# manuelbb-upb/Morbit.jl

Hardware: AMD Instinct MI355X
Metric: RBF build+solve+eval cycles/sec (higher is better)
Workload: dtype f64

## Files before the change

### include/mrbf.h

```cpp
#ifndef MRBF_H
#define MRBF_H

#include <stdint.h>

#ifdef __cplusplus
extern "C" {
#endif

typedef struct mrbf_ctx mrbf_ctx;
typedef struct mrbf_model mrbf_model;

enum {
    MRBF_CUBIC = 0,
    MRBF_INV_MULTIQUADRIC = 1,
    MRBF_MULTIQUADRIC = 2,
    MRBF_THIN_PLATE_SPLINE = 3,
    MRBF_GAUSSIAN = 4
};

enum {
    MRBF_OK = 0,
    MRBF_ENOTPD = 1,
    MRBF_ESINGULAR = 2,
    MRBF_EHIP = 3,
    MRBF_EBLAS = 4,
    MRBF_ENOMEM = 5,
    MRBF_ENODEVICE = 6,
    MRBF_ENCCL = 7
};

enum {
    MRBF_PATH_CHOL = 1,
    MRBF_PATH_PROJ_CHOL = 2,
    MRBF_PATH_LU = 3,
    MRBF_PATH_MINNORM = 4,
    MRBF_PATH_ROUND4 = 5
};

enum {
    MRBF_OPT_GRAM_MODE = 1,
    MRBF_OPT_RESIDUAL = 2,
    MRBF_OPT_FORCE_PATH = 3,
    MRBF_OPT_CHOL_IMPL = 4,
    MRBF_OPT_EVAL_IMPL = 5,
    MRBF_OPT_TIMING = 6,
    MRBF_OPT_DIAG_IMPL = 7,
    MRBF_OPT_CHOL_WINDOW = 8,
    MRBF_OPT_SPIN_MS = 9,
    MRBF_OPT_LAST_DEVICE_MS = 11,
    MRBF_OPT_SLOW_LAUNCHES = 12,
    MRBF_OPT_ARENA_BYTES = 13,
    MRBF_OPT_LIVE_HANDLES = 14,
    MRBF_OPT_SMALL_FIT_MAX_N = 15,
    MRBF_OPT_SMALL_LU = 16,
    MRBF_OPT_DEBUG_FAULT = 10
};

enum {
    MRBF_FB_CHOL_HOST_DRIVEN = 1,
    MRBF_FB_BACKSOLVE_BLOCKED = 2,
    MRBF_FB_LU = 4
};

typedef struct {
    int32_t path;
    int32_t factor_info;
    int32_t n, q;
    double rel_residual;
    double max_pitw;
    double mu;
    float ms_gram, ms_project, ms_factor, ms_solve, ms_check, ms_total;
    int32_t fallbacks;
    int32_t giveup_code;
    float ms_factor_device;
    int32_t slow_launches;
} mrbf_fit_info;

typedef struct {
    float ms_total;
    float ms_dist, ms_kernel, ms_contract;
} mrbf_eval_info;

int32_t mrbf_init(int32_t device_id, mrbf_ctx **ctx);
int32_t mrbf_shutdown(mrbf_ctx *ctx);
const char *mrbf_last_error(const mrbf_ctx *ctx);
const char *mrbf_version(void);
int32_t mrbf_set_option(mrbf_ctx *ctx, int32_t key, double value);
int32_t mrbf_get_option(const mrbf_ctx *ctx, int32_t key, double *value);
int32_t mrbf_set_stream(mrbf_ctx *ctx, void *hip_stream);
int32_t mrbf_sync(mrbf_ctx *ctx);

int32_t mrbf_gram(mrbf_ctx *ctx, int64_t n, int32_t d, const double *centres, int32_t kernel_id, double a, double b,
                  int32_t poly_deg, double *Phi_out, double *Pi_out, float *ms);

int32_t mrbf_cross_gram(mrbf_ctx *ctx, int64_t m, int64_t n, int32_t d, const double *X, const double *centres, int32_t kernel_id,
                        double a, double b, double *K_out);

int32_t mrbf_fit(mrbf_ctx *ctx, int64_t n, int32_t d, int32_t k, const double *centres, const double *values,
                 int32_t kernel_id, double a, double b, int32_t poly_deg, mrbf_model **model, double *weights_out,
                 double *poly_out, mrbf_fit_info *info);

int32_t mrbf_model_from_coeffs(mrbf_ctx *ctx, int64_t n, int32_t d, int32_t k, const double *centres,
                               const double *weights, const double *poly, int32_t kernel_id, double a, double b,
                               int32_t poly_deg, mrbf_model **model);

int32_t mrbf_eval(mrbf_ctx *ctx, const mrbf_model *model, int64_t m, const double *X, double *vals_out,
                  double *jac_out, mrbf_eval_info *info);

typedef struct {
    float ms_total;
    int32_t nsplit;
    int32_t chunks;
    int32_t reserved;
} mrbf_hess_info;
int32_t mrbf_eval_hessian(mrbf_ctx *ctx, const mrbf_model *model, int64_t m, const double *X, int32_t n_rows, const int32_t *rows,
                          double *hess_out, mrbf_hess_info *info);
int32_t mrbf_eval_hessian_limited(mrbf_ctx *ctx, const mrbf_model *model, int64_t m, const double *X, int32_t n_rows,
                                  const int32_t *rows, double *hess_out, mrbf_hess_info *info, int64_t stage_bytes);

int32_t mrbf_backtrack(mrbf_ctx *ctx, const mrbf_model *model, const double *x, const double *dir, double step0,
                       double omega, int32_t strict, double const_rhs, double shrink, double min_stepsize,
                       int32_t max_loops, double *x_plus, double *mx_plus, double *step, int32_t *n_loops);

int32_t mrbf_affine_scores(mrbf_ctx *ctx, int64_t mc, int32_t d, int32_t dz, const double *shifted, const double *Z, int32_t p_is_inf,
                           double *vals_out, int64_t *argmax, double *maxval);
int32_t mrbf_affine_select(mrbf_ctx *ctx, int64_t mc, int32_t d, const double *shifted, int32_t j0, const double *Q0, int32_t max_picks,
                           double pivot_val, int32_t p_is_inf, int64_t *picked_out, int32_t *n_picked, double *Z_out);

typedef struct {
    int64_t mc;
    int32_t j0;
    int32_t max_picks;
    double pivot_val;
    const double *shifted;
    const double *Q0;
    int64_t *picked_out;
    double *Z_out;
    int32_t n_picked;
    int32_t reserved;
} mrbf_affine_job;
int32_t mrbf_affine_select_batch(mrbf_ctx *ctx, int64_t n_starts, int32_t d, int32_t p_is_inf, mrbf_affine_job *jobs,
                                 float *ms_total);

typedef struct mrbf_round4_state mrbf_round4_state;
int32_t mrbf_round4(mrbf_ctx *ctx, int64_t n0, int32_t d, const double *start_sites, int64_t mc, const double *cand_sites,
                    int32_t kernel_id, double a, double b, int32_t poly_deg, int32_t max_points, double theta_pivot_cholesky,
                    int32_t *accepted_out, int32_t *n_accepted, mrbf_round4_state **state);
int32_t mrbf_fit_from_round4(mrbf_ctx *ctx, const mrbf_round4_state *state, int32_t k, const double *values, mrbf_model **model,
                             double *weights_out, double *poly_out, mrbf_fit_info *info);
int32_t mrbf_round4_sites(const mrbf_round4_state *state, int64_t *n0, int64_t *n_candidates, int32_t *n_accepted);
int32_t mrbf_free_round4(mrbf_ctx *ctx, mrbf_round4_state *state);

typedef struct {
    int64_t n0, mc;
    const double *start_sites;
    const double *cand_sites;
    int32_t kernel_id, poly_deg;
    double a, b;
    int32_t max_points;
    double theta_pivot_cholesky;
    int32_t *accepted_out;
    int32_t n_accepted;
    int32_t rc;
} mrbf_round4_job;
int32_t mrbf_round4_batch(mrbf_ctx *ctx, int64_t n_starts, int32_t d, mrbf_round4_job *jobs, float *ms_total);

int32_t mrbf_model_dims(const mrbf_model *model, int64_t *n, int32_t *d, int32_t *k, int32_t *q);
int32_t mrbf_free_model(mrbf_ctx *ctx, mrbf_model *model);

typedef struct {
    int64_t n, m;
    int32_t d, k, kernel_id, poly_deg;
    double a, b;
    const double *centres;
    const double *values;
    const double *X;
    double *weights_out;
    double *poly_out;
    double *vals_out;
    double *jac_out;
} mrbf_problem;

typedef struct {
    int32_t status;
    int32_t device;
    mrbf_fit_info fit;
    float ms_eval;
    double checksum_w;
    double checksum_vals;
} mrbf_result;

int32_t mrbf_batch_run(int32_t n_dev, const int32_t *device_ids, int64_t n_problems, const mrbf_problem *problems,
                       mrbf_result *results);

typedef struct {
    int64_t n;
    int32_t d, k, kernel_id, poly_deg;
    double a, b;
    const double *centres, *values;
    double *weights_out, *poly_out;
    mrbf_model *model;
    int32_t status;
    int32_t reserved;
    mrbf_fit_info info;
} mrbf_fit_job;
int32_t mrbf_fit_batch(mrbf_ctx *ctx, int64_t n_starts, mrbf_fit_job *jobs, float *ms_total);

typedef struct {
    const mrbf_model *model;
    int64_t m;
    const double *X;
    double *vals_out;
    double *jac_out;
    int32_t status;
    int32_t reserved;
} mrbf_eval_job;
int32_t mrbf_eval_batch(mrbf_ctx *ctx, int64_t n_jobs, mrbf_eval_job *jobs, float *ms_total);
int32_t mrbf_eval_batch_limited(mrbf_ctx *ctx, int64_t n_jobs, mrbf_eval_job *jobs, float *ms_total, int64_t arena_limit_bytes);

typedef struct mrbf_db mrbf_db;
int32_t mrbf_db_create(mrbf_ctx *ctx, int32_t d, int32_t k, int64_t capacity_hint, mrbf_db **db);
int32_t mrbf_db_append(mrbf_ctx *ctx, mrbf_db *db, int64_t m, const double *sites, const double *values, int64_t *first_index);
int32_t mrbf_db_set_values(mrbf_ctx *ctx, mrbf_db *db, int64_t m, const int64_t *indices, const double *values);
int32_t mrbf_db_read(mrbf_ctx *ctx, const mrbf_db *db, int64_t first, int64_t m, double *sites_out, double *values_out);
int32_t mrbf_db_dims(const mrbf_db *db, int64_t *n_sites, int32_t *d, int32_t *k);
int32_t mrbf_db_free(mrbf_ctx *ctx, mrbf_db *db);

typedef struct {
    mrbf_db *db;
    const double *lb, *ub, *x0;
    int64_t n_exclude;
    const int64_t *exclude;
    int32_t zero_first_pick;
    int32_t rc;
    int64_t *indices_out;
    double *sites_out, *shifted_out;
    double *first_row;
    int64_t mc;
    int64_t first_pick;
    const double *cand_sites_dev;
    const double *shifted_dev;
} mrbf_db_box_job;
int32_t mrbf_db_box_batch(mrbf_ctx *ctx, int64_t n_starts, int32_t d, int32_t p_is_inf, mrbf_db_box_job *jobs, float *ms_total);

typedef struct {
    mrbf_db *db;
    int64_t n_idx;
    const int64_t *indices;
    double *sites_out, *values_out;
    const double *sites_dev;
    const double *values_dev;
    int32_t rc;
    int32_t reserved;
} mrbf_db_gather_job;
int32_t mrbf_db_gather_batch(mrbf_ctx *ctx, int64_t n_starts, int32_t d, mrbf_db_gather_job *jobs, float *ms_total);

typedef struct {
    mrbf_db *db;
    int64_t m;
    const double *sites;
    const double *values;
    int64_t first_index;
    int32_t rc;
    int32_t reserved;
} mrbf_db_append_job;
int32_t mrbf_db_append_batch(mrbf_ctx *ctx, int64_t n_starts, mrbf_db_append_job *jobs, float *ms_total);
typedef struct {
    mrbf_db *db;
    int64_t m;
    const int64_t *indices;
    const double *values;
    int32_t rc;
    int32_t reserved;
} mrbf_db_set_values_job;
int32_t mrbf_db_set_values_batch(mrbf_ctx *ctx, int64_t n_starts, mrbf_db_set_values_job *jobs, float *ms_total);

enum { MRBF_R3_UPDATE = 0, MRBF_R3_IMPROVE = 1 };
enum { MRBF_R3_DONE = 0, MRBF_R3_REBUILT = 1 };
typedef struct {
    mrbf_db *db;
    const double *x, *lb, *ub;
    double pivot_val;
    const double *dirs;
    int32_t n_dirs, reversed;
    int32_t n_missing, max_new;
    int32_t ensure_fully_linear, force_rebuild, mode;
    int32_t rc;
    double *new_sites_out;
    int64_t first_index;
    int32_t n_new, fully_linear, status, n_dirs_used;
} mrbf_round3_job;
int32_t mrbf_db_round3_batch(mrbf_ctx *ctx, int64_t n_starts, int32_t d, mrbf_round3_job *jobs, float *ms_total);

int32_t mrbf_debug_env(const char *name);
int32_t mrbf_debug_mfma_layout(mrbf_ctx *ctx, double *out16x16_a_times_b, const double *A16x4, const double *B4x16);
int32_t mrbf_debug_potrf(mrbf_ctx *ctx, int64_t n, double *A_colmajor_inout, int32_t impl, int32_t *info, float *ms);
int32_t mrbf_debug_diag(mrbf_ctx *ctx, const double *A128, int32_t reps, float *ms_per_call, double *shader_cycles,
                        double *realtime_us);
int32_t mrbf_debug_mfma_peak(mrbf_ctx *ctx, int32_t blocks_per_cu, int32_t threads, int32_t iters, float *ms, double *tflops);
int32_t mrbf_debug_mfma_asm(mrbf_ctx *ctx, int32_t variant, int32_t blocks_per_cu, int32_t iters, float *ms, double *tflops,
                            double *cycles_per_mfma);
int32_t mrbf_debug_dgemm(mrbf_ctx *ctx, int32_t m, int32_t n, int32_t k, float *ms, double *tflops);
int32_t mrbf_debug_mega_tables(int32_t nt, int32_t mt, int32_t slack, int32_t slack_chain, int32_t first, int32_t win, int32_t srows,
                               int32_t half_cols, int64_t *out6);
int32_t mrbf_debug_mega_tables2(int32_t nt, int32_t mt, int32_t slack, int32_t slack_chain, int32_t first, int32_t win, int32_t srows,
                                int32_t half_cols, const int32_t *opt5, int64_t *out6);
int32_t mrbf_debug_mega_plan(int32_t nt, int32_t mt, int32_t xreal, int64_t *out39);

enum { MRBF_PS_OK = 0, MRBF_PS_CRITICAL = 1, MRBF_PS_FAILURE = 2 };
typedef struct {
    int32_t max_ideal_evals;
    int32_t max_ps_evals;
    int32_t max_polish_evals;
    int32_t reserved;
    uint64_t seed;
    double t0;
    double xtol_rel;
} mrbf_ps_options;
typedef struct {
    int32_t status;
    int32_t generations;
    int32_t evals_ideal, evals_ps, evals_polish;
    float ms_total;
    double tau;
} mrbf_ps_info;
int32_t mrbf_ps_step(mrbf_ctx *ctx, const mrbf_model *model, const double *x_n, const double *lb_eff, const double *ub_eff,
                     const double *fx_n, const double *r_or_null, const mrbf_ps_options *opts, double *x_trial, double *mx_trial,
                     double *r_out, mrbf_ps_info *info);

enum { MRBF_ROLE_NONE = -1, MRBF_ROLE_EQ = -2, MRBF_ROLE_INEQ = -3 };
typedef struct {
    int32_t n_models, n_objectives;
    const mrbf_model *const *models;
    const int32_t *roles;
    int32_t n_lin_eq, n_lin_ineq;
    const double *A_eq, *b_eq, *A_ineq, *b_ineq;
    double eq_tol;
} mrbf_ps_problem;
int32_t mrbf_ps_step_problem(mrbf_ctx *ctx, const mrbf_ps_problem *problem, const double *x_n, const double *lb_eff,
                             const double *ub_eff, const double *fx_n, const double *r_or_null, const mrbf_ps_options *opts,
                             double *x_trial, double *mx_trial, double *r_out, mrbf_ps_info *info);
int32_t mrbf_debug_ps_rank(mrbf_ctx *ctx, int32_t lam, const double *f, const double *phi, uint64_t seed, int32_t gen, int32_t impl,
                           int32_t *order_out, int32_t *gave_up);

enum { MRBF_SD_OK = 0, MRBF_SD_NO_OBJECTIVE = 1, MRBF_SD_INFEASIBLE = 2, MRBF_SD_GAVE_UP = 3 };
int32_t mrbf_sd_direction(mrbf_ctx *ctx, int64_t n_lp, int32_t d, int32_t k, int32_t m_eq, int32_t m_ineq, const double *G,
                          const double *x, const double *lb, const double *ub, const double *A_eq, const double *b_eq,
                          const double *A_ineq, const double *b_ineq, int32_t normalize, double *d_out, double *omega_out,
                          double *dual_out, int32_t *status_out, int32_t *iters_out);
typedef struct {
    int32_t status;
    int32_t iterations;
    int32_t bound_flips;
    float ms_total;
    double omega;
} mrbf_sd_info;
int32_t mrbf_sd_criticality(mrbf_ctx *ctx, const mrbf_ps_problem *problem, const double *x, const double *x_n, const double *lb,
                            const double *ub, int32_t normalize, double *d_out, double *dual_out, mrbf_sd_info *info);

enum { MRBF_NS_OK = 0, MRBF_NS_INFEASIBLE = 1, MRBF_NS_GAVE_UP = 2 };
int32_t mrbf_normal_direction(mrbf_ctx *ctx, int64_t n_lp, int32_t d, int32_t m_eq, int32_t m_ineq, const double *x, const double *lb,
                              const double *ub, const double *A_eq, const double *b_eq, const double *A_ineq, const double *b_ineq,
                              double *n_out, double *alpha_out, double *dual_out, int32_t *status_out, int32_t *iters_out);
typedef struct {
    int32_t status;
    int32_t iterations;
    int32_t bound_flips;
    float ms_total;
    double alpha;
    double delta;
} mrbf_normal_info;
int32_t mrbf_normal_step(mrbf_ctx *ctx, const mrbf_ps_problem *problem, int32_t d, const double *x, const double *lb, const double *ub,
                         double delta, double kappa_delta, double delta_max, int32_t variable_radius, double *n_out, double *dual_out,
                         mrbf_normal_info *info);

typedef struct {
    int32_t strict;
    int32_t max_loops;
    double const_rhs;
    double shrink;
    double min_stepsize;
} mrbf_sd_step_options;
typedef struct {
    int32_t branch;
    int32_t loops;
    float ms_total;
    double sigma;
    double omega;
    double step_norm;
} mrbf_sd_step_info;
int32_t mrbf_sd_step(mrbf_ctx *ctx, const mrbf_ps_problem *problem, const double *x, const double *x_n, double delta, const double *lb,
                     const double *ub, double omega, const double *d, const mrbf_sd_step_options *opts, double *x_plus, double *mx_plus,
                     mrbf_sd_step_info *info);

typedef struct {
    int32_t sd_status;
    int32_t iterations, bound_flips;
    int32_t branch, loops;
    int32_t reserved;
    double omega;
    double omega_step;
    double sigma, step_norm;
} mrbf_sd_batch_record;
int32_t mrbf_sd_iterate_batch(mrbf_ctx *ctx, int64_t n_starts, const mrbf_ps_problem *shape, const mrbf_model *const *models,
                              const double *x, const double *x_n, const double *delta, const double *lb, const double *ub,
                              int32_t normalize, const mrbf_sd_step_options *opts, double *d_out, double *x_plus, double *mx_plus,
                              mrbf_sd_batch_record *records, float *ms_total);

typedef struct {
    int32_t status;
    int32_t iterations, bound_flips;
    int32_t reserved;
    double alpha;
    double delta;
} mrbf_normal_batch_record;
int32_t mrbf_normal_step_batch(mrbf_ctx *ctx, int64_t n_starts, const mrbf_ps_problem *shape, const mrbf_model *const *models, int32_t d,
                               const double *x, const double *lb, const double *ub, const double *delta, double kappa_delta,
                               double delta_max, int32_t variable_radius, double *n_out, double *x_n_out, double *dual_out,
                               mrbf_normal_batch_record *records, float *ms_total);

int32_t mrbf_ps_step_batch(mrbf_ctx *ctx, int64_t n_starts, const mrbf_ps_problem *shape, const mrbf_model *const *models,
                           const double *x_n, const double *lb_eff, const double *ub_eff, const double *fx_n, const double *r_or_null,
                           const mrbf_ps_options *opts, const uint64_t *seeds_or_null, double *x_trial, double *mx_trial, double *r_out,
                           mrbf_ps_info *infos, float *ms_total);

enum { MRBF_DISPATCH_REFERENCE = 0, MRBF_DISPATCH_DEVICE = 1 };
enum { MRBF_FIT_FULL = 0, MRBF_FIT_FROM_ROUND4 = 1 };
enum { MRBF_ENTRY_ROUND4 = 1, MRBF_ENTRY_FIT_FROM_ROUND4 = 2, MRBF_ENTRY_PS_STEP = 3, MRBF_ENTRY_BACKTRACK = 4, MRBF_ENTRY_AFFINE = 5,
       MRBF_ENTRY_SD = 6, MRBF_ENTRY_NORMAL = 7, MRBF_ENTRY_SD_STEP = 8, MRBF_ENTRY_SD_BATCH = 9, MRBF_ENTRY_AFFINE_BATCH = 10,
       MRBF_ENTRY_FIT_BATCH = 11, MRBF_ENTRY_NORMAL_BATCH = 12, MRBF_ENTRY_ROUND4_BATCH = 13, MRBF_ENTRY_PS_BATCH = 14,
       MRBF_ENTRY_DB_BOX = 15, MRBF_ENTRY_DB_GATHER = 16, MRBF_ENTRY_DB_ROUND3 = 17, MRBF_ENTRY_DB_APPEND_BATCH = 18,
       MRBF_ENTRY_DB_SET_VALUES_BATCH = 19, MRBF_ENTRY_EVAL_BATCH = 20 };
int32_t mrbf_dispatch_ps(int32_t d, int32_t k, int32_t n_models, int32_t n_nl_constraints, int32_t n_lin_constraints, int32_t n_foreign);
int32_t mrbf_dispatch_ps_batch(int64_t n_starts, int32_t d, int32_t k, int32_t n_models, int32_t n_nl_constraints,
                               int32_t n_lin_constraints, int32_t n_foreign);
int32_t mrbf_dispatch_sd(int32_t d, int32_t k, int32_t n_models, int32_t n_nl_constraints, int32_t n_lin_constraints, int32_t n_foreign);
int32_t mrbf_dispatch_normal(int32_t d, int32_t n_models, int32_t n_nl_constraints, int32_t n_lin_constraints, int32_t n_foreign);
int32_t mrbf_dispatch_sd_step(int32_t d, int32_t k, int32_t n_models, int32_t n_nl_constraints, int32_t n_lin_constraints, int32_t n_foreign,
                              int32_t max_loops);
int32_t mrbf_dispatch_sd_batch(int64_t n_starts, int32_t d, int32_t k, int32_t n_models, int32_t n_nl_constraints,
                               int32_t n_lin_constraints, int32_t n_foreign, int32_t max_loops);
int32_t mrbf_dispatch_normal_batch(int64_t n_starts, int32_t d, int32_t n_models, int32_t n_nl_constraints, int32_t n_lin_constraints,
                                   int32_t n_foreign);
int32_t mrbf_dispatch_backtrack(int32_t n_objective_models, int32_t n_foreign, int32_t outputs_in_order);
int32_t mrbf_dispatch_affine(int64_t n_candidates, int32_t d);
int32_t mrbf_dispatch_affine_batch(int64_t n_starts, int32_t d, int32_t p_is_inf);
int32_t mrbf_dispatch_round4(int64_t n0, int32_t d, int32_t poly_deg, int64_t n_candidates);
int32_t mrbf_dispatch_fit_batch(int64_t n_starts);
int64_t mrbf_dispatch_fit_batch_max_n(int64_t n_starts, int32_t d);
int32_t mrbf_dispatch_fit_batch_lu(int64_t n_lu_starts, int64_t n_max, int32_t d);
int32_t mrbf_dispatch_round4_batch(int64_t n_starts, int32_t d);
int32_t mrbf_dispatch_db_batch(int64_t n_starts, int32_t d);
int32_t mrbf_dispatch_eval_batch(int64_t n_jobs);
int64_t mrbf_dispatch_eval_batch_min_jobs(void);
int32_t mrbf_dispatch_fit(int64_t n_training, int64_t state_n0, int32_t state_q, int32_t state_n_accepted, int32_t same_sites);
int32_t mrbf_dispatch_after(int32_t entry, int32_t rc);

int32_t mrbf_stochastic_rank(int32_t lam, const double *f, const double *phi, const double *u, double pf, int32_t *idx_out);

#ifdef __cplusplus
}
#endif
#endif
```

### morbit.jl_amd/_lib.py

```python
import ctypes
import os

import numpy as np

_HERE = os.path.dirname(os.path.abspath(__file__))
LIB_PATH = os.environ.get("MRBF_LIB") or os.path.join(_HERE, "libmrbf.so")

c_dp = ctypes.POINTER(ctypes.c_double)
c_fp = ctypes.POINTER(ctypes.c_float)
c_ip = ctypes.POINTER(ctypes.c_int32)
c_vp = ctypes.c_void_p

MRBF_OK, MRBF_ENOTPD, MRBF_ESINGULAR, MRBF_EHIP, MRBF_EBLAS, MRBF_ENOMEM, MRBF_ENODEVICE, MRBF_ENCCL = range(8)
PATH_CHOL, PATH_PROJ_CHOL, PATH_LU, PATH_MINNORM, PATH_ROUND4 = 1, 2, 3, 4, 5
OPT_GRAM_MODE, OPT_RESIDUAL, OPT_FORCE_PATH, OPT_CHOL_IMPL, OPT_EVAL_IMPL, OPT_TIMING, OPT_DIAG_IMPL, OPT_CHOL_WINDOW = 1, 2, 3, 4, 5, 6, 7, 8
OPT_SPIN_MS, OPT_DEBUG_FAULT, OPT_LAST_DEVICE_MS, OPT_SLOW_LAUNCHES = 9, 10, 11, 12
OPT_ARENA_BYTES, OPT_LIVE_HANDLES = 13, 14
OPT_SMALL_FIT_MAX_N = 15
SMALL_FIT_DEFAULT_MAX_N = 512
OPT_SMALL_LU = 16
SMALL_LU_MAX_N, SMALL_LU_MAX_D, SMALL_LU_MAX_K = 512, 128, 16
FB_CHOL_HOST_DRIVEN, FB_BACKSOLVE_BLOCKED, FB_LU = 1, 2, 4


class FitInfo(ctypes.Structure):
    _fields_ = [("path", ctypes.c_int32), ("factor_info", ctypes.c_int32), ("n", ctypes.c_int32), ("q", ctypes.c_int32),
                ("rel_residual", ctypes.c_double), ("max_pitw", ctypes.c_double), ("mu", ctypes.c_double),
                ("ms_gram", ctypes.c_float), ("ms_project", ctypes.c_float), ("ms_factor", ctypes.c_float),
                ("ms_solve", ctypes.c_float), ("ms_check", ctypes.c_float), ("ms_total", ctypes.c_float),
                ("fallbacks", ctypes.c_int32), ("giveup_code", ctypes.c_int32), ("ms_factor_device", ctypes.c_float),
                ("slow_launches", ctypes.c_int32)]

    def asdict(self):
        return {f: getattr(self, f) for f, _ in self._fields_}


class EvalInfo(ctypes.Structure):
    _fields_ = [("ms_total", ctypes.c_float), ("ms_dist", ctypes.c_float), ("ms_kernel", ctypes.c_float),
                ("ms_contract", ctypes.c_float)]

    def asdict(self):
        return {f: getattr(self, f) for f, _ in self._fields_}


class HessInfo(ctypes.Structure):
    _fields_ = [("ms_total", ctypes.c_float), ("nsplit", ctypes.c_int32), ("chunks", ctypes.c_int32), ("reserved", ctypes.c_int32)]

    def asdict(self):
        return {f: getattr(self, f) for f, _ in self._fields_}


class PsOptions(ctypes.Structure):
    _fields_ = [("max_ideal_evals", ctypes.c_int32), ("max_ps_evals", ctypes.c_int32), ("max_polish_evals", ctypes.c_int32),
                ("reserved", ctypes.c_int32), ("seed", ctypes.c_uint64), ("t0", ctypes.c_double), ("xtol_rel", ctypes.c_double)]


class PsInfo(ctypes.Structure):
    _fields_ = [("status", ctypes.c_int32), ("generations", ctypes.c_int32), ("evals_ideal", ctypes.c_int32),
                ("evals_ps", ctypes.c_int32), ("evals_polish", ctypes.c_int32), ("ms_total", ctypes.c_float), ("tau", ctypes.c_double)]

    def asdict(self):
        return {f: getattr(self, f) for f, _ in self._fields_}


PS_OK, PS_CRITICAL, PS_FAILURE = 0, 1, 2
ROLE_NONE, ROLE_EQ, ROLE_INEQ = -1, -2, -3
DISPATCH_REFERENCE, DISPATCH_DEVICE = 0, 1
FIT_FULL, FIT_FROM_ROUND4 = 0, 1
ENTRY_ROUND4, ENTRY_FIT_FROM_ROUND4, ENTRY_PS_STEP, ENTRY_BACKTRACK, ENTRY_AFFINE, ENTRY_SD, ENTRY_NORMAL, ENTRY_SD_STEP = 1, 2, 3, 4, 5, 6, 7, 8
ENTRY_SD_BATCH = 9
ENTRY_AFFINE_BATCH = 10
ENTRY_FIT_BATCH = 11
ENTRY_NORMAL_BATCH = 12
ENTRY_ROUND4_BATCH = 13
ENTRY_PS_BATCH = 14
ENTRY_DB_BOX = 15
ENTRY_DB_GATHER = 16
ENTRY_DB_ROUND3 = 17
ENTRY_DB_APPEND_BATCH = 18
ENTRY_DB_SET_VALUES_BATCH = 19
ENTRY_EVAL_BATCH = 20
R3_UPDATE, R3_IMPROVE = 0, 1
R3_DONE, R3_REBUILT = 0, 1
SD_OK, SD_NO_OBJECTIVE, SD_INFEASIBLE, SD_GAVE_UP = 0, 1, 2, 3
NS_OK, NS_INFEASIBLE, NS_GAVE_UP = 0, 1, 2
SD_BRANCH_DELTA, SD_BRANCH_ONE, SD_BRANCH_INTERSECT = 0, 1, 2


class PsProblem(ctypes.Structure):
    _fields_ = [("n_models", ctypes.c_int32), ("n_objectives", ctypes.c_int32), ("models", ctypes.POINTER(ctypes.c_void_p)),
                ("roles", ctypes.POINTER(ctypes.c_int32)), ("n_lin_eq", ctypes.c_int32), ("n_lin_ineq", ctypes.c_int32),
                ("A_eq", ctypes.c_void_p), ("b_eq", ctypes.c_void_p), ("A_ineq", ctypes.c_void_p), ("b_ineq", ctypes.c_void_p),
                ("eq_tol", ctypes.c_double)]


class SdInfo(ctypes.Structure):
    _fields_ = [("status", ctypes.c_int32), ("iterations", ctypes.c_int32), ("bound_flips", ctypes.c_int32), ("ms_total", ctypes.c_float),
                ("omega", ctypes.c_double)]

    def asdict(self):
        return {f: getattr(self, f) for f, _ in self._fields_}


class NormalInfo(ctypes.Structure):
    _fields_ = [("status", ctypes.c_int32), ("iterations", ctypes.c_int32), ("bound_flips", ctypes.c_int32), ("ms_total", ctypes.c_float),
                ("alpha", ctypes.c_double), ("delta", ctypes.c_double)]

    def asdict(self):
        return {f: getattr(self, f) for f, _ in self._fields_}


class SdStepOptions(ctypes.Structure):
    _fields_ = [("strict", ctypes.c_int32), ("max_loops", ctypes.c_int32), ("const_rhs", ctypes.c_double), ("shrink", ctypes.c_double),
                ("min_stepsize", ctypes.c_double)]


class SdStepInfo(ctypes.Structure):
    _fields_ = [("branch", ctypes.c_int32), ("loops", ctypes.c_int32), ("ms_total", ctypes.c_float), ("sigma", ctypes.c_double),
                ("omega", ctypes.c_double), ("step_norm", ctypes.c_double)]

    def asdict(self):
        return {f: getattr(self, f) for f, _ in self._fields_}


class SdBatchRecord(ctypes.Structure):
    _fields_ = [("sd_status", ctypes.c_int32), ("iterations", ctypes.c_int32), ("bound_flips", ctypes.c_int32), ("branch", ctypes.c_int32),
                ("loops", ctypes.c_int32), ("reserved", ctypes.c_int32), ("omega", ctypes.c_double), ("omega_step", ctypes.c_double),
                ("sigma", ctypes.c_double), ("step_norm", ctypes.c_double)]

    def asdict(self):
        return {f: getattr(self, f) for f, _ in self._fields_}


class NormalBatchRecord(ctypes.Structure):
    _fields_ = [("status", ctypes.c_int32), ("iterations", ctypes.c_int32), ("bound_flips", ctypes.c_int32), ("reserved", ctypes.c_int32),
                ("alpha", ctypes.c_double), ("delta", ctypes.c_double)]

    def asdict(self):
        return {f: getattr(self, f) for f, _ in self._fields_}


class AffineJob(ctypes.Structure):
    _fields_ = [("mc", ctypes.c_int64), ("j0", ctypes.c_int32), ("max_picks", ctypes.c_int32), ("pivot_val", ctypes.c_double),
                ("shifted", ctypes.c_void_p), ("Q0", ctypes.c_void_p), ("picked_out", ctypes.c_void_p), ("Z_out", ctypes.c_void_p),
                ("n_picked", ctypes.c_int32), ("reserved", ctypes.c_int32)]


class Round4Job(ctypes.Structure):
    _fields_ = [("n0", ctypes.c_int64), ("mc", ctypes.c_int64), ("start_sites", ctypes.c_void_p), ("cand_sites", ctypes.c_void_p),
                ("kernel_id", ctypes.c_int32), ("poly_deg", ctypes.c_int32), ("a", ctypes.c_double), ("b", ctypes.c_double),
                ("max_points", ctypes.c_int32), ("theta_pivot_cholesky", ctypes.c_double), ("accepted_out", ctypes.c_void_p),
                ("n_accepted", ctypes.c_int32), ("rc", ctypes.c_int32)]


class FitJob(ctypes.Structure):
    _fields_ = [("n", ctypes.c_int64), ("d", ctypes.c_int32), ("k", ctypes.c_int32), ("kernel_id", ctypes.c_int32),
                ("poly_deg", ctypes.c_int32), ("a", ctypes.c_double), ("b", ctypes.c_double), ("centres", ctypes.c_void_p),
                ("values", ctypes.c_void_p), ("weights_out", ctypes.c_void_p), ("poly_out", ctypes.c_void_p), ("model", ctypes.c_void_p),
                ("status", ctypes.c_int32), ("reserved", ctypes.c_int32), ("info", FitInfo)]


class EvalJob(ctypes.Structure):
    _fields_ = [("model", ctypes.c_void_p), ("m", ctypes.c_int64), ("X", ctypes.c_void_p), ("vals_out", ctypes.c_void_p),
                ("jac_out", ctypes.c_void_p), ("status", ctypes.c_int32), ("reserved", ctypes.c_int32)]


class DbBoxJob(ctypes.Structure):
    _fields_ = [("db", ctypes.c_void_p), ("lb", ctypes.c_void_p), ("ub", ctypes.c_void_p), ("x0", ctypes.c_void_p),
                ("n_exclude", ctypes.c_int64), ("exclude", ctypes.c_void_p), ("zero_first_pick", ctypes.c_int32), ("rc", ctypes.c_int32),
                ("indices_out", ctypes.c_void_p), ("sites_out", ctypes.c_void_p), ("shifted_out", ctypes.c_void_p),
                ("first_row", ctypes.c_void_p), ("mc", ctypes.c_int64), ("first_pick", ctypes.c_int64),
                ("cand_sites_dev", ctypes.c_void_p), ("shifted_dev", ctypes.c_void_p)]


class DbGatherJob(ctypes.Structure):
    _fields_ = [("db", ctypes.c_void_p), ("n_idx", ctypes.c_int64), ("indices", ctypes.c_void_p), ("sites_out", ctypes.c_void_p),
                ("values_out", ctypes.c_void_p), ("sites_dev", ctypes.c_void_p), ("values_dev", ctypes.c_void_p),
                ("rc", ctypes.c_int32), ("reserved", ctypes.c_int32)]


class DbAppendJob(ctypes.Structure):
    _fields_ = [("db", ctypes.c_void_p), ("m", ctypes.c_int64), ("sites", ctypes.c_void_p), ("values", ctypes.c_void_p),
                ("first_index", ctypes.c_int64), ("rc", ctypes.c_int32), ("reserved", ctypes.c_int32)]


class DbSetValuesJob(ctypes.Structure):
    _fields_ = [("db", ctypes.c_void_p), ("m", ctypes.c_int64), ("indices", ctypes.c_void_p), ("values", ctypes.c_void_p),
                ("rc", ctypes.c_int32), ("reserved", ctypes.c_int32)]


class Round3Job(ctypes.Structure):
    _fields_ = [("db", ctypes.c_void_p), ("x", ctypes.c_void_p), ("lb", ctypes.c_void_p), ("ub", ctypes.c_void_p),
                ("pivot_val", ctypes.c_double), ("dirs", ctypes.c_void_p), ("n_dirs", ctypes.c_int32), ("reversed", ctypes.c_int32),
                ("n_missing", ctypes.c_int32), ("max_new", ctypes.c_int32), ("ensure_fully_linear", ctypes.c_int32),
                ("force_rebuild", ctypes.c_int32), ("mode", ctypes.c_int32), ("rc", ctypes.c_int32), ("new_sites_out", ctypes.c_void_p),
                ("first_index", ctypes.c_int64), ("n_new", ctypes.c_int32), ("fully_linear", ctypes.c_int32), ("status", ctypes.c_int32),
                ("n_dirs_used", ctypes.c_int32)]


class Problem(ctypes.Structure):
    _fields_ = [("n", ctypes.c_int64), ("m", ctypes.c_int64), ("d", ctypes.c_int32), ("k", ctypes.c_int32),
                ("kernel_id", ctypes.c_int32), ("poly_deg", ctypes.c_int32), ("a", ctypes.c_double), ("b", ctypes.c_double),
                ("centres", c_dp), ("values", c_dp), ("X", c_dp), ("weights_out", c_dp), ("poly_out", c_dp),
                ("vals_out", c_dp), ("jac_out", c_dp)]


class Result(ctypes.Structure):
    _fields_ = [("status", ctypes.c_int32), ("device", ctypes.c_int32), ("fit", FitInfo), ("ms_eval", ctypes.c_float),
                ("checksum_w", ctypes.c_double), ("checksum_vals", ctypes.c_double)]


SIGNATURES = {
    "mrbf_init": (ctypes.c_int32, [ctypes.c_int32, ctypes.POINTER(c_vp)]),
    "mrbf_shutdown": (ctypes.c_int32, [c_vp]),
    "mrbf_last_error": (ctypes.c_char_p, [c_vp]),
    "mrbf_version": (ctypes.c_char_p, []),
    "mrbf_set_option": (ctypes.c_int32, [c_vp, ctypes.c_int32, ctypes.c_double]),
    "mrbf_get_option": (ctypes.c_int32, [c_vp, ctypes.c_int32, c_dp]),
    "mrbf_set_stream": (ctypes.c_int32, [c_vp, c_vp]),
    "mrbf_sync": (ctypes.c_int32, [c_vp]),
    "mrbf_gram": (ctypes.c_int32, [c_vp, ctypes.c_int64, ctypes.c_int32, c_vp, ctypes.c_int32, ctypes.c_double,
                                   ctypes.c_double, ctypes.c_int32, c_vp, c_vp, c_fp]),
    "mrbf_cross_gram": (ctypes.c_int32, [c_vp, ctypes.c_int64, ctypes.c_int64, ctypes.c_int32, c_vp, c_vp, ctypes.c_int32, ctypes.c_double,
                                         ctypes.c_double, c_vp]),
    "mrbf_fit": (ctypes.c_int32, [c_vp, ctypes.c_int64, ctypes.c_int32, ctypes.c_int32, c_vp, c_vp, ctypes.c_int32,
                                  ctypes.c_double, ctypes.c_double, ctypes.c_int32, ctypes.POINTER(c_vp), c_vp, c_vp,
                                  ctypes.POINTER(FitInfo)]),
    "mrbf_model_from_coeffs": (ctypes.c_int32, [c_vp, ctypes.c_int64, ctypes.c_int32, ctypes.c_int32, c_vp, c_vp, c_vp,
                                                ctypes.c_int32, ctypes.c_double, ctypes.c_double, ctypes.c_int32,
                                                ctypes.POINTER(c_vp)]),
    "mrbf_eval": (ctypes.c_int32, [c_vp, c_vp, ctypes.c_int64, c_vp, c_vp, c_vp, ctypes.POINTER(EvalInfo)]),
    "mrbf_eval_hessian": (ctypes.c_int32, [c_vp, c_vp, ctypes.c_int64, c_vp, ctypes.c_int32, c_vp, c_vp, ctypes.POINTER(HessInfo)]),
    "mrbf_eval_hessian_limited": (ctypes.c_int32, [c_vp, c_vp, ctypes.c_int64, c_vp, ctypes.c_int32, c_vp, c_vp, ctypes.POINTER(HessInfo),
                                                   ctypes.c_int64]),
    "mrbf_backtrack": (ctypes.c_int32, [c_vp, c_vp, c_vp, c_vp, ctypes.c_double, ctypes.c_double, ctypes.c_int32,
                                        ctypes.c_double, ctypes.c_double, ctypes.c_double, ctypes.c_int32, c_vp, c_vp,
                                        c_vp, c_ip]),
    "mrbf_affine_scores": (ctypes.c_int32, [c_vp, ctypes.c_int64, ctypes.c_int32, ctypes.c_int32, c_vp, c_vp, ctypes.c_int32, c_vp,
                                            ctypes.POINTER(ctypes.c_int64), c_dp]),
    "mrbf_affine_select": (ctypes.c_int32, [c_vp, ctypes.c_int64, ctypes.c_int32, c_vp, ctypes.c_int32, c_vp, ctypes.c_int32, ctypes.c_double,
                                            ctypes.c_int32, ctypes.POINTER(ctypes.c_int64), c_ip, c_vp]),
    "mrbf_affine_select_batch": (ctypes.c_int32, [c_vp, ctypes.c_int64, ctypes.c_int32, ctypes.c_int32, ctypes.POINTER(AffineJob), c_fp]),
    "mrbf_round4": (ctypes.c_int32, [c_vp, ctypes.c_int64, ctypes.c_int32, c_vp, ctypes.c_int64, c_vp, ctypes.c_int32, ctypes.c_double,
                                     ctypes.c_double, ctypes.c_int32, ctypes.c_int32, ctypes.c_double, c_vp, c_ip, ctypes.POINTER(c_vp)]),
    "mrbf_fit_from_round4": (ctypes.c_int32, [c_vp, c_vp, ctypes.c_int32, c_vp, ctypes.POINTER(c_vp), c_vp, c_vp, ctypes.POINTER(FitInfo)]),
    "mrbf_round4_sites": (ctypes.c_int32, [c_vp, ctypes.POINTER(ctypes.c_int64), ctypes.POINTER(ctypes.c_int64), c_ip]),
    "mrbf_free_round4": (ctypes.c_int32, [c_vp, c_vp]),
    "mrbf_round4_batch": (ctypes.c_int32, [c_vp, ctypes.c_int64, ctypes.c_int32, ctypes.POINTER(Round4Job), c_fp]),
    "mrbf_dispatch_round4_batch": (ctypes.c_int32, [ctypes.c_int64, ctypes.c_int32]),
    "mrbf_model_dims": (ctypes.c_int32, [c_vp, ctypes.POINTER(ctypes.c_int64), c_ip, c_ip, c_ip]),
    "mrbf_free_model": (ctypes.c_int32, [c_vp, c_vp]),
    "mrbf_batch_run": (ctypes.c_int32, [ctypes.c_int32, c_ip, ctypes.c_int64, ctypes.POINTER(Problem),
                                        ctypes.POINTER(Result)]),
    "mrbf_fit_batch": (ctypes.c_int32, [c_vp, ctypes.c_int64, ctypes.POINTER(FitJob), c_fp]),
    "mrbf_dispatch_fit_batch": (ctypes.c_int32, [ctypes.c_int64]),
    "mrbf_dispatch_fit_batch_max_n": (ctypes.c_int64, [ctypes.c_int64, ctypes.c_int32]),
    "mrbf_dispatch_fit_batch_lu": (ctypes.c_int32, [ctypes.c_int64, ctypes.c_int64, ctypes.c_int32]),
    "mrbf_eval_batch": (ctypes.c_int32, [c_vp, ctypes.c_int64, ctypes.POINTER(EvalJob), c_fp]),
    "mrbf_eval_batch_limited": (ctypes.c_int32, [c_vp, ctypes.c_int64, ctypes.POINTER(EvalJob), c_fp, ctypes.c_int64]),
    "mrbf_dispatch_eval_batch": (ctypes.c_int32, [ctypes.c_int64]),
    "mrbf_dispatch_eval_batch_min_jobs": (ctypes.c_int64, []),
    "mrbf_db_create": (ctypes.c_int32, [c_vp, ctypes.c_int32, ctypes.c_int32, ctypes.c_int64, ctypes.POINTER(c_vp)]),
    "mrbf_db_append": (ctypes.c_int32, [c_vp, c_vp, ctypes.c_int64, c_vp, c_vp, ctypes.POINTER(ctypes.c_int64)]),
    "mrbf_db_set_values": (ctypes.c_int32, [c_vp, c_vp, ctypes.c_int64, c_vp, c_vp]),
    "mrbf_db_read": (ctypes.c_int32, [c_vp, c_vp, ctypes.c_int64, ctypes.c_int64, c_vp, c_vp]),
    "mrbf_db_dims": (ctypes.c_int32, [c_vp, ctypes.POINTER(ctypes.c_int64), c_ip, c_ip]),
    "mrbf_db_free": (ctypes.c_int32, [c_vp, c_vp]),
    "mrbf_db_box_batch": (ctypes.c_int32, [c_vp, ctypes.c_int64, ctypes.c_int32, ctypes.c_int32, ctypes.POINTER(DbBoxJob), c_fp]),
    "mrbf_db_gather_batch": (ctypes.c_int32, [c_vp, ctypes.c_int64, ctypes.c_int32, ctypes.POINTER(DbGatherJob), c_fp]),
    "mrbf_db_append_batch": (ctypes.c_int32, [c_vp, ctypes.c_int64, ctypes.POINTER(DbAppendJob), c_fp]),
    "mrbf_db_set_values_batch": (ctypes.c_int32, [c_vp, ctypes.c_int64, ctypes.POINTER(DbSetValuesJob), c_fp]),
    "mrbf_db_round3_batch": (ctypes.c_int32, [c_vp, ctypes.c_int64, ctypes.c_int32, ctypes.POINTER(Round3Job), c_fp]),
    "mrbf_dispatch_db_batch": (ctypes.c_int32, [ctypes.c_int64, ctypes.c_int32]),
    "mrbf_debug_mfma_layout": (ctypes.c_int32, [c_vp, c_vp, c_vp, c_vp]),
    "mrbf_debug_potrf": (ctypes.c_int32, [c_vp, ctypes.c_int64, c_vp, ctypes.c_int32, c_ip, c_fp]),
    "mrbf_debug_env": (ctypes.c_int32, [ctypes.c_char_p]),
    "mrbf_debug_diag": (ctypes.c_int32, [c_vp, c_vp, ctypes.c_int32, c_fp, c_dp, c_dp]),
    "mrbf_debug_ps_rank": (ctypes.c_int32, [c_vp, ctypes.c_int32, c_vp, c_vp, ctypes.c_uint64, ctypes.c_int32, ctypes.c_int32, c_ip, c_ip]),
    "mrbf_debug_mfma_peak": (ctypes.c_int32, [c_vp, ctypes.c_int32, ctypes.c_int32, ctypes.c_int32, c_fp, c_dp]),
    "mrbf_debug_mfma_asm": (ctypes.c_int32, [c_vp, ctypes.c_int32, ctypes.c_int32, ctypes.c_int32, c_fp, c_dp, c_dp]),
    "mrbf_debug_dgemm": (ctypes.c_int32, [c_vp, ctypes.c_int32, ctypes.c_int32, ctypes.c_int32, c_fp, c_dp]),
    "mrbf_debug_mega_tables": (ctypes.c_int32, [ctypes.c_int32] * 8 + [c_vp]),
    "mrbf_debug_mega_tables2": (ctypes.c_int32, [ctypes.c_int32] * 8 + [c_vp, c_vp]),
    "mrbf_debug_mega_plan": (ctypes.c_int32, [ctypes.c_int32] * 3 + [c_vp]),
    "mrbf_stochastic_rank": (ctypes.c_int32, [ctypes.c_int32, c_vp, c_vp, c_vp, ctypes.c_double, c_vp]),
    "mrbf_ps_step": (ctypes.c_int32, [c_vp, c_vp, c_vp, c_vp, c_vp, c_vp, c_vp, ctypes.POINTER(PsOptions), c_vp, c_vp, c_vp,
                                      ctypes.POINTER(PsInfo)]),
    "mrbf_ps_step_problem": (ctypes.c_int32, [c_vp, ctypes.POINTER(PsProblem), c_vp, c_vp, c_vp, c_vp, c_vp, ctypes.POINTER(PsOptions),
                                              c_vp, c_vp, c_vp, ctypes.POINTER(PsInfo)]),
    "mrbf_ps_step_batch": (ctypes.c_int32, [c_vp, ctypes.c_int64, ctypes.POINTER(PsProblem), ctypes.POINTER(ctypes.c_void_p), c_vp, c_vp, c_vp,
                                            c_vp, c_vp, ctypes.POINTER(PsOptions), ctypes.POINTER(ctypes.c_uint64), c_vp, c_vp, c_vp,
                                            ctypes.POINTER(PsInfo), c_fp]),
    "mrbf_dispatch_ps_batch": (ctypes.c_int32, [ctypes.c_int64] + [ctypes.c_int32] * 6),
    "mrbf_sd_direction": (ctypes.c_int32, [c_vp, ctypes.c_int64, ctypes.c_int32, ctypes.c_int32, ctypes.c_int32, ctypes.c_int32] + [c_vp] * 8
                          + [ctypes.c_int32, c_vp, c_vp, c_vp, c_vp, c_vp]),
    "mrbf_sd_criticality": (ctypes.c_int32, [c_vp, ctypes.POINTER(PsProblem), c_vp, c_vp, c_vp, c_vp, ctypes.c_int32, c_vp, c_vp,
                                             ctypes.POINTER(SdInfo)]),
    "mrbf_normal_direction": (ctypes.c_int32, [c_vp, ctypes.c_int64, ctypes.c_int32, ctypes.c_int32, ctypes.c_int32] + [c_vp] * 12),
    "mrbf_normal_step": (ctypes.c_int32, [c_vp, ctypes.POINTER(PsProblem), ctypes.c_int32, c_vp, c_vp, c_vp, ctypes.c_double, ctypes.c_double,
                                          ctypes.c_double, ctypes.c_int32, c_vp, c_vp, ctypes.POINTER(NormalInfo)]),
    "mrbf_sd_step": (ctypes.c_int32, [c_vp, ctypes.POINTER(PsProblem), c_vp, c_vp, ctypes.c_double, c_vp, c_vp, ctypes.c_double, c_vp,
                                      ctypes.POINTER(SdStepOptions), c_vp, c_vp, ctypes.POINTER(SdStepInfo)]),
    "mrbf_sd_iterate_batch": (ctypes.c_int32, [c_vp, ctypes.c_int64, ctypes.POINTER(PsProblem), ctypes.POINTER(ctypes.c_void_p), c_vp, c_vp, c_vp,
                                               c_vp, c_vp, ctypes.c_int32, ctypes.POINTER(SdStepOptions), c_vp, c_vp, c_vp,
                                               ctypes.POINTER(SdBatchRecord), c_fp]),
    "mrbf_dispatch_sd_batch": (ctypes.c_int32, [ctypes.c_int64] + [ctypes.c_int32] * 7),
    "mrbf_normal_step_batch": (ctypes.c_int32, [c_vp, ctypes.c_int64, ctypes.POINTER(PsProblem), ctypes.POINTER(ctypes.c_void_p), ctypes.c_int32,
                                                c_vp, c_vp, c_vp, c_vp, ctypes.c_double, ctypes.c_double, ctypes.c_int32, c_vp, c_vp, c_vp,
                                                ctypes.POINTER(NormalBatchRecord), c_fp]),
    "mrbf_dispatch_normal_batch": (ctypes.c_int32, [ctypes.c_int64] + [ctypes.c_int32] * 5),
    "mrbf_dispatch_ps": (ctypes.c_int32, [ctypes.c_int32] * 6),
    "mrbf_dispatch_sd_step": (ctypes.c_int32, [ctypes.c_int32] * 7),
    "mrbf_dispatch_sd": (ctypes.c_int32, [ctypes.c_int32] * 6),
    "mrbf_dispatch_normal": (ctypes.c_int32, [ctypes.c_int32] * 5),
    "mrbf_dispatch_backtrack": (ctypes.c_int32, [ctypes.c_int32] * 3),
    "mrbf_dispatch_affine": (ctypes.c_int32, [ctypes.c_int64, ctypes.c_int32]),
    "mrbf_dispatch_affine_batch": (ctypes.c_int32, [ctypes.c_int64, ctypes.c_int32, ctypes.c_int32]),
    "mrbf_dispatch_round4": (ctypes.c_int32, [ctypes.c_int64, ctypes.c_int32, ctypes.c_int32, ctypes.c_int64]),
    "mrbf_dispatch_fit": (ctypes.c_int32, [ctypes.c_int64, ctypes.c_int64, ctypes.c_int32, ctypes.c_int32, ctypes.c_int32]),
    "mrbf_dispatch_after": (ctypes.c_int32, [ctypes.c_int32, ctypes.c_int32]),
}

_LIB = None


class MrbfError(RuntimeError):
    def __init__(self, code, msg):
        super().__init__("libmrbf error %d: %s" % (code, msg))
        self.code = code


def load():
    global _LIB
    if _LIB is None:
        if not os.path.exists(LIB_PATH):
            raise ImportError("libmrbf.so is not built (%s); run `python -c 'import __graft_entry__ as g; g.build()'` "
                              "or `make -C morbit.jl_amd/csrc`. There is no CPU fallback." % LIB_PATH)
        lib = ctypes.CDLL(LIB_PATH)
        for name, (res, args) in SIGNATURES.items():
            fn = getattr(lib, name)
            fn.restype = res
            fn.argtypes = args
        _LIB = lib
    return _LIB


def as_ptr(a):
    if a is None:
        return None
    if isinstance(a, np.ndarray):
        return ctypes.c_void_p(a.ctypes.data)
    if hasattr(a, "data_ptr"):
        return ctypes.c_void_p(a.data_ptr())
    raise TypeError("expected numpy array or tensor, got %r" % type(a))


def host_f64(a, shape=None):
    a = np.ascontiguousarray(a, dtype=np.float64)
    if shape is not None:
        a = a.reshape(shape)
    return a


class Context:

    def __init__(self, device_id=-1):
        self.lib = load()
        h = c_vp()
        rc = self.lib.mrbf_init(device_id, ctypes.byref(h))
        if rc != 0:
            raise MrbfError(rc, (self.lib.mrbf_last_error(None) or b"").decode())
        self.h = h

    def check(self, rc):
        if rc != 0:
            raise MrbfError(rc, (self.lib.mrbf_last_error(self.h) or b"").decode())

    def set_option(self, key, value):
        self.check(self.lib.mrbf_set_option(self.h, key, float(value)))

    def get_option(self, key):
        v = ctypes.c_double()
        self.check(self.lib.mrbf_get_option(self.h, key, ctypes.byref(v)))
        return v.value

    def sync(self):
        self.check(self.lib.mrbf_sync(self.h))

    def close(self):
        if getattr(self, "h", None):
            self.lib.mrbf_shutdown(self.h)
            self.h = None

    def __del__(self):
        try:
            self.close()
        except Exception:
            pass


_DEFAULT_CTX = {}


def default_context(device_id=-1):
    import threading

    key = (threading.get_ident(), device_id)
    if key not in _DEFAULT_CTX:
        _DEFAULT_CTX[key] = Context(device_id)
    return _DEFAULT_CTX[key]
```

### morbit.jl_amd/csrc/backsolve.hip

```cpp
#include "common.hpp"

namespace mrbf {

namespace bsolve {

constexpr int NB = 128, NTHR = 512;
typedef double v2d __attribute__((ext_vector_type(2)));
typedef double v4d __attribute__((ext_vector_type(4)));
typedef __attribute__((address_space(1))) unsigned gu32;
typedef __attribute__((address_space(1))) double gf64;
typedef __attribute__((address_space(1))) v2d gv2d;

template <int KB>
struct Shared {
    double xs[2][KB][NB];
    int ok;
};

__global__ __launch_bounds__(256) void premul_kernel(const double *__restrict__ L, int64_t lda, const double *__restrict__ linv_all,
                                                     double *__restrict__ Mbuf, int nb, unsigned *__restrict__ flags, int nflags,
                                                     unsigned long long *__restrict__ xb, int nxb) {
    for (int e = blockIdx.x * 256 + threadIdx.x; e < nflags; e += gridDim.x * 256) flags[e] = 0u;
    for (int e = blockIdx.x * 256 + threadIdx.x; e < nxb; e += gridDim.x * 256) xb[e] = ~0ull;
    const int slab = blockIdx.x & 3, t = (blockIdx.x >> 2) & 1, j = blockIdx.x >> 3;
    const int i = j + 1 + t;
    if (i >= nb) return;
    const double *A = L + (int64_t)i * NB + (int64_t)j * NB * lda;
    const double *B = linv_all + (size_t)j * NB * NB;
    double *M = Mbuf + ((size_t)j * 2 + t) * NB * NB;
    const int lane = threadIdx.x & 63, wave = threadIdx.x >> 6, l15 = lane & 15, l4 = lane >> 4;
    const int i0 = 32 * wave, j0 = 32 * slab;
    v4d acc[2][2];
#pragma unroll
    for (int a = 0; a < 2; ++a)
#pragma unroll
        for (int b = 0; b < 2; ++b) acc[a][b] = (v4d){0.0, 0.0, 0.0, 0.0};
    const double *pa = A + (i0 + l15) + (int64_t)(j0 + l4) * lda;
    const double *pb = B + (j0 + l4) + (int64_t)(j0 + l15) * NB;
    constexpr int UK = 8;
    double fa0[2][UK], fa1[2][UK], fb0[2][UK], fb1[2][UK];
    auto burst = [&](int buf) {
#pragma unroll
        for (int u = 0; u < UK; ++u) {
            fa0[buf][u] = pa[(int64_t)4 * u * lda];
            fa1[buf][u] = pa[(int64_t)4 * u * lda + 16];
            fb0[buf][u] = pb[4 * u];
            fb1[buf][u] = pb[4 * u + 16 * NB];
        }
        pa += (int64_t)4 * UK * lda;
        pb += 4 * UK;
    };
    auto mma = [&](int buf) {
#pragma unroll
        for (int u = 0; u < UK; ++u) {
            acc[0][0] = __builtin_amdgcn_mfma_f64_16x16x4f64(fa0[buf][u], fb0[buf][u], acc[0][0], 0, 0, 0);
            acc[0][1] = __builtin_amdgcn_mfma_f64_16x16x4f64(fa0[buf][u], fb1[buf][u], acc[0][1], 0, 0, 0);
            acc[1][0] = __builtin_amdgcn_mfma_f64_16x16x4f64(fa1[buf][u], fb0[buf][u], acc[1][0], 0, 0, 0);
            acc[1][1] = __builtin_amdgcn_mfma_f64_16x16x4f64(fa1[buf][u], fb1[buf][u], acc[1][1], 0, 0, 0);
        }
    };
    const int nburst = (NB - j0) / (4 * UK);
    burst(0);
    for (int b = 0; b < nburst; b += 2) {
        if (b + 1 < nburst) burst(1);
        mma(0);
        if (b + 1 >= nburst) break;
        if (b + 2 < nburst) burst(0);
        mma(1);
    }
#pragma unroll
    for (int a = 0; a < 2; ++a)
#pragma unroll
        for (int b = 0; b < 2; ++b)
#pragma unroll
            for (int r = 0; r < 4; ++r) M[(i0 + 16 * a + l4 + 4 * r) + (size_t)(j0 + 16 * b + l15) * NB] = acc[a][b][r];
}

__device__ __forceinline__ void load_tile(const double *__restrict__ T, int64_t ldt, v2d (&r)[2][8]) {
    const int lane = threadIdx.x & 63, w = threadIdx.x >> 6;
    const double *p = T + (int64_t)(16 * w + 2 * (lane >> 3)) * ldt + 2 * (lane & 7);
#pragma unroll
    for (int cc = 0; cc < 2; ++cc)
#pragma unroll
        for (int u = 0; u < 8; ++u) r[cc][u] = *(const gv2d *)(p + cc * ldt + 16 * u);
}

template <int N>
__device__ __forceinline__ double shl_lanes(double v) {
    const long long b = __double_as_longlong(v);
    const int lo = __builtin_amdgcn_update_dpp((int)b, (int)b, 0x100 + N, 0xf, 0xf, false);
    const int hi = __builtin_amdgcn_update_dpp((int)(b >> 32), (int)(b >> 32), 0x100 + N, 0xf, 0xf, false);
    return __longlong_as_double(((long long)hi << 32) | (unsigned)lo);
}

template <int KB>
__device__ __forceinline__ void tile_dot(const double (*xs)[NB], const v2d (&r)[2][8], double (&out)[2][KB]) {
    const int q = threadIdx.x & 7;
    double acc[2][KB];
#pragma unroll
    for (int cc = 0; cc < 2; ++cc)
#pragma unroll
        for (int l = 0; l < KB; ++l) acc[cc][l] = 0.0;
#pragma unroll
    for (int u = 0; u < 8; ++u) {
#pragma unroll
        for (int l = 0; l < KB; ++l) {
            const v2d x = *(const v2d *)&xs[l][16 * u + 2 * q];
#pragma unroll
            for (int cc = 0; cc < 2; ++cc) acc[cc][l] = fma(r[cc][u][1], x[1], fma(r[cc][u][0], x[0], acc[cc][l]));
        }
    }
#pragma unroll
    for (int cc = 0; cc < 2; ++cc)
#pragma unroll
        for (int l = 0; l < KB; ++l) {
            double v = acc[cc][l];
            v += shl_lanes<4>(v);
            v += shl_lanes<2>(v);
            v += shl_lanes<1>(v);
            out[cc][l] = v;
        }
}

template <int KB>
__device__ __forceinline__ void await_block(Shared<KB> &sh, double (*xs)[NB], const double *glob, int i, double spec, int backoff,
                                            unsigned *abortw, unsigned epoch, unsigned long long spin_ticks, int *status, int code) {
    const int tid = threadIdx.x;
    if (tid >= KB * NB) return;
    const gf64 *src = (const gf64 *)&glob[((size_t)i * KB + tid / NB) * NB + (tid % NB)];
    double v = spec;
    if (__double_as_longlong(v) == -1ll) v = __hip_atomic_load(src, __ATOMIC_RELAXED, __HIP_MEMORY_SCOPE_AGENT);
    unsigned spins = 0;
    unsigned long long t0 = 0;
    while (__double_as_longlong(v) == -1ll) {
        if ((++spins & 63u) == 0u) {
            if (__hip_atomic_load((const gu32 *)abortw, __ATOMIC_RELAXED, __HIP_MEMORY_SCOPE_AGENT) != 0u) {
                sh.ok = 0;
                break;
            }
            const unsigned long long now = wall_clock64();
            if (t0 == 0) t0 = now;
            if (now - t0 > spin_ticks) {
                __hip_atomic_store((gu32 *)abortw, epoch, __ATOMIC_RELAXED, __HIP_MEMORY_SCOPE_AGENT);
                *(__attribute__((address_space(1))) int *)status = code + (i & 0xff);
                sh.ok = 0;
                break;
            }
        }
        for (int b = 0; b < backoff; ++b) __builtin_amdgcn_s_sleep(8);
        v = __hip_atomic_load(src, __ATOMIC_RELAXED, __HIP_MEMORY_SCOPE_AGENT);
    }
    xs[tid / NB][tid % NB] = v;
}

__device__ __forceinline__ void lds_barrier() { asm volatile("s_waitcnt lgkmcnt(0)\n\ts_barrier" ::: "memory"); }

__device__ __forceinline__ void publish(double *dst, v2d v) {
    if (__double_as_longlong(v[0]) == -1ll) v[0] = __longlong_as_double(0x7ff8000000000000ll);
    if (__double_as_longlong(v[1]) == -1ll) v[1] = __longlong_as_double(0x7ff8000000000000ll);
    asm volatile("global_store_dwordx4 %0, %1, off sc1" ::"v"(dst), "v"(v) : "memory");
}

template <int KB>
__global__ __launch_bounds__(NTHR, 1) void backsolve_persistent_kernel(const double *__restrict__ L, int64_t lda, const double *__restrict__ linv_all,
                                                                        const double *__restrict__ Mbuf, double *__restrict__ Y, int64_t ldy, int k0,
                                                                        int nb, unsigned *flags, unsigned epoch, unsigned long long spin_ticks,
                                                                        int *status, int fault, double *__restrict__ xb, double *__restrict__ zb,
                                                                        long long *stamps) {
    __shared__ __attribute__((aligned(16))) Shared<KB> sh;
    const int p = (int)blockIdx.x >> 1;
    const bool finisher = blockIdx.x & 1;
    const int j = nb - 1 - p, tid = threadIdx.x;
    const int lane = tid & 63, col = 16 * (tid >> 6) + 2 * (lane >> 3), q = lane & 7;
    unsigned *abortw = flags + (size_t)nb * 32;
    const int na = nb - 1 - j, npm = na < 2 ? na : 2, npl = na - npm;
    if (tid == 0) sh.ok = 1;
    __syncthreads();
    const double fillv = __longlong_as_double(-1ll);
    if (!finisher) {
        double w[2][KB];
#pragma unroll
        for (int cc = 0; cc < 2; ++cc)
#pragma unroll
            for (int l = 0; l < KB; ++l) w[cc][l] = *(const gf64 *)&Y[(int64_t)(k0 + l) * ldy + (int64_t)j * NB + col + cc];
        const int nst = npl + 1;
        auto fetch = [&](int s, v2d(&r)[2][8]) {
            const double *src = s < npl ? L + (int64_t)(nb - 1 - s) * NB + (int64_t)j * NB * lda : linv_all + (size_t)j * NB * NB;
            load_tile(src, s < npl ? lda : (int64_t)NB, r);
        };
        auto look = [&](int s) {
            const int i = nb - 1 - (s < npl ? s : (npl > 0 ? npl - 1 : 0));
            const int e = tid < KB * NB ? tid : 0;
            return __hip_atomic_load((const gf64 *)&xb[((size_t)i * KB + e / NB) * NB + (e % NB)], __ATOMIC_RELAXED, __HIP_MEMORY_SCOPE_AGENT);
        };
        double spec = fillv, spec2 = fillv;
        auto step = [&](int s, const v2d(&r)[2][8]) -> bool {
            double(*xs)[NB] = sh.xs[s & 1];
            if (s < npl) {
                const int i = nb - 1 - s;
                const int backoff = (i - j - 3) < 24 ? (i - j - 3) : 24;
                await_block<KB>(sh, xs, xb, i, spec, backoff, abortw, epoch, spin_ticks, status, 0x700);
                if (stamps && tid == 0 && s == npl - 1) stamps[256 * 5 + j * 4 + 0] = (long long)wall_clock64();
            } else if (q == 0) {
#pragma unroll
                for (int l = 0; l < KB; ++l) *(v2d *)&xs[l][col] = (v2d){w[0][l], w[1][l]};
            }
            spec = spec2;
            spec2 = look(s + 2);
            if (s + 2 >= npl) spec2 = fillv;
            lds_barrier();
            if (!sh.ok) return false;
            double dsum[2][KB];
            tile_dot<KB>(xs, r, dsum);
#pragma unroll
            for (int cc = 0; cc < 2; ++cc)
#pragma unroll
                for (int l = 0; l < KB; ++l) w[cc][l] = s == npl ? dsum[cc][l] : w[cc][l] - dsum[cc][l];
            return true;
        };
        v2d t0[2][8], t1[2][8], t2[2][8];
        const int o = (3 - nst % 3) % 3, G = (nst + o) / 3;
        if (0 - o >= 0) fetch(0 - o, t0);
        if (1 - o >= 0) fetch(1 - o, t1);
        fetch(2 - o, t2);
        spec = look(0);
        if (npl == 0) spec = fillv;
        spec2 = look(1);
        if (npl <= 1) spec2 = fillv;
        int g = 0;
        if (G >= 2) {
            const int s = -o;
            if (s >= 0 && !step(s, t0)) return;
            fetch(s + 3, t0);
            if (s + 1 >= 0 && !step(s + 1, t1)) return;
            fetch(s + 4, t1);
            if (!step(s + 2, t2)) return;
            fetch(s + 5, t2);
            g = 1;
        }
        for (; g < G - 1; ++g) {
            const int s = 3 * g - o;
            if (!step(s, t0)) return;
            fetch(s + 3, t0);
            if (!step(s + 1, t1)) return;
            fetch(s + 4, t1);
            if (!step(s + 2, t2)) return;
            fetch(s + 5, t2);
        }
        {
            const int s = 3 * (G - 1) - o;
            if (s >= 0 && !step(s, t0)) return;
            if (s + 1 >= 0 && !step(s + 1, t1)) return;
            if (!step(s + 2, t2)) return;
        }
        if (stamps && tid == 0) stamps[256 * 5 + j * 4 + 1] = (long long)wall_clock64();
        if (q == 0) {
#pragma unroll
            for (int l = 0; l < KB; ++l) publish(&zb[((size_t)j * KB + l) * NB + col], (v2d){w[0][l], w[1][l]});
        }
        return;
    }
    v2d tm2[2][8], tm1[2][8];
    if (npm == 2) load_tile(Mbuf + ((size_t)j * 2 + 1) * NB * NB, NB, tm2);
    if (npm >= 1) load_tile(Mbuf + (size_t)j * 2 * NB * NB, NB, tm1);
    double acc[2][KB];
#pragma unroll
    for (int cc = 0; cc < 2; ++cc)
#pragma unroll
        for (int l = 0; l < KB; ++l) acc[cc][l] = 0.0;
    if (npm == 2) {
        await_block<KB>(sh, sh.xs[0], xb, j + 2, fillv, 1, abortw, epoch, spin_ticks, status, 0x700);
        lds_barrier();
        if (!sh.ok) return;
        if (stamps && tid == 0) stamps[256 * 5 + j * 4 + 3] = (long long)wall_clock64();
        tile_dot<KB>(sh.xs[0], tm2, acc);
    }
    v2d zj[KB];
    if (q == 0) {
        unsigned spins = 0;
        unsigned long long t0 = 0;
#pragma unroll
        for (int l = 0; l < KB; ++l) {
            const double *src = &zb[((size_t)j * KB + l) * NB + col];
            while (true) {
                v2d v;
                asm volatile("global_load_dwordx4 %0, %1, off sc1\n\ts_waitcnt vmcnt(0)" : "=v"(v) : "v"(src) : "memory");
                if (__double_as_longlong(v[0]) != -1ll && __double_as_longlong(v[1]) != -1ll) {
                    zj[l] = v;
                    break;
                }
                if ((++spins & 63u) == 0u) {
                    if (__hip_atomic_load((const gu32 *)abortw, __ATOMIC_RELAXED, __HIP_MEMORY_SCOPE_AGENT) != 0u) {
                        sh.ok = 0;
                        break;
                    }
                    const unsigned long long now = wall_clock64();
                    if (t0 == 0) t0 = now;
                    if (now - t0 > spin_ticks) {
                        __hip_atomic_store((gu32 *)abortw, epoch, __ATOMIC_RELAXED, __HIP_MEMORY_SCOPE_AGENT);
                        *(__attribute__((address_space(1))) int *)status = 0x600 + (j & 0xff);
                        sh.ok = 0;
                        break;
                    }
                }
                __builtin_amdgcn_s_sleep(2);
            }
            if (!sh.ok) break;
        }
    }
    if (stamps && tid == 0) stamps[256 * 5 + j * 4 + 2] = (long long)wall_clock64();
    double last[2][KB];
#pragma unroll
    for (int cc = 0; cc < 2; ++cc)
#pragma unroll
        for (int l = 0; l < KB; ++l) last[cc][l] = 0.0;
    if (npm >= 1) {
        if (stamps && tid == 0) stamps[256 * 4 + j] = (long long)wall_clock64();
        await_block<KB>(sh, sh.xs[1], xb, j + 1, fillv, 0, abortw, epoch, spin_ticks, status, 0x700);
        if (stamps && tid == 0) stamps[j * 4 + 0] = (long long)wall_clock64();
        lds_barrier();
        if (!sh.ok) return;
        if (stamps && tid == 0) stamps[j * 4 + 1] = (long long)wall_clock64();
        tile_dot<KB>(sh.xs[1], tm1, last);
    } else {
        lds_barrier();
        if (!sh.ok) return;
    }
    if ((fault & 1) && j == nb / 2) return;
    if (stamps && tid == 0) stamps[j * 4 + 2] = (long long)wall_clock64();
    if (q == 0) {
#pragma unroll
        for (int l = 0; l < KB; ++l) {
            const v2d v = (v2d){(zj[l][0] - acc[0][l]) - last[0][l], (zj[l][1] - acc[1][l]) - last[1][l]};
            publish(&xb[((size_t)j * KB + l) * NB + col], v);
            *(v2d *)&Y[(int64_t)(k0 + l) * ldy + (int64_t)j * NB + col] = v;
        }
    }
}

}

int backsolve_blocked(mrbf_ctx *ctx, int64_t npad, const double *L, int64_t lda, const double *linv_all, double *Y, int64_t ldy, int k);

int backsolve_persistent(mrbf_ctx *ctx, int64_t npad, const double *L, int64_t lda, const double *linv_all, double *Y, int64_t ldy, int k,
                         int *status) {
    using namespace bsolve;
    const int nb = (int)(npad / NB);
    static const int force_old = mrbf_env("MRBF_BACKSOLVE_LAUNCHES") ? atoi(mrbf_env("MRBF_BACKSOLVE_LAUNCHES")) : 0;
    const int ncu = ctx->ncu;
    if (force_old || nb < 3 || nb > ncu || (lda & 1) || (reinterpret_cast<uintptr_t>(L) & 15))
        return backsolve_blocked(ctx, npad, L, lda, linv_all, Y, ldy, k);
    unsigned *flags;
    MRBF_TRY(get_buf(ctx, S_BSOLVE_FLAGS, (size_t)(nb + 1) * 32, &flags));
    const unsigned long long spin_ticks = (unsigned long long)std::max(1, ctx->spin_ms) * 100000ull;
    const int fault = (ctx->debug_fault & 2) ? 1 : 0;
    double *xb, *Mbuf;
    MRBF_TRY(get_buf(ctx, S_BSOLVE_X, (size_t)2 * nb * 4 * NB, &xb));
    MRBF_TRY(get_buf(ctx, S_BSOLVE_M, (size_t)nb * 2 * NB * NB, &Mbuf));
    hipLaunchKernelGGL(premul_kernel, dim3((unsigned)(8 * (nb - 1))), dim3(256), 0, ctx->stream, L, lda, linv_all, Mbuf, nb, flags, (nb + 1) * 32,
                       reinterpret_cast<unsigned long long *>(xb), 2 * nb * 4 * NB);
    static const bool want_stamps = mrbf_env("MRBF_BSOLVE_STAMPS") && atoi(mrbf_env("MRBF_BSOLVE_STAMPS")) != 0;
    long long *stamps = nullptr;
    if (want_stamps) {
        static long long *dbg = nullptr;
        if (!dbg) MRBF_HIP(ctx, hipMalloc(&dbg, (size_t)256 * 9 * sizeof(long long)));
        stamps = dbg;
    }
    unsigned epoch = 0;
    for (int k0 = 0; k0 < k; k0 += 4) {
        const int kb = std::min(4, k - k0);
        ++epoch;
        if (k0 > 0) MRBF_HIP(ctx, hipMemsetAsync(xb, 0xff, (size_t)2 * nb * 4 * NB * sizeof(double), ctx->stream));
#define MRBF_BSP(KBV)                                                                                                          \
    hipLaunchKernelGGL((backsolve_persistent_kernel<KBV>), dim3((unsigned)(2 * nb)), dim3(NTHR), 0, ctx->stream, L, lda, linv_all, Mbuf, Y, ldy, k0, nb, \
                       flags, epoch, spin_ticks, status, fault, xb, xb + (size_t)nb * 4 * NB, stamps)
        if (kb == 1) MRBF_BSP(1); else if (kb == 2) MRBF_BSP(2); else if (kb == 3) MRBF_BSP(3); else MRBF_BSP(4);
#undef MRBF_BSP
    }
    MRBF_HIP(ctx, hipGetLastError());
    if (want_stamps) {
        std::vector<long long> h((size_t)256 * 9);
        MRBF_HIP(ctx, hipMemcpyAsync(h.data(), stamps, h.size() * sizeof(long long), hipMemcpyDeviceToHost, ctx->stream));
        MRBF_HIP(ctx, hipStreamSynchronize(ctx->stream));
        double seen = 0, bar = 0, dot = 0, hop = 0, late = 0;
        int cnt = 0;
        for (int j = 1; j + 2 < nb; ++j) {
            seen += (double)(h[j * 4 + 0] - h[(j + 1) * 4 + 2]);
            bar += (double)(h[j * 4 + 1] - h[j * 4 + 0]);
            dot += (double)(h[j * 4 + 2] - h[j * 4 + 1]);
            hop += (double)(h[j * 4 + 2] - h[(j + 1) * 4 + 2]);
            late += (double)(h[256 * 4 + j] - h[(j + 1) * 4 + 2]);
            ++cnt;
        }
        double a3 = 0, zt = 0, zs = 0, x2 = 0;
        int c2 = 0;
        for (int j = 2; j + 4 < nb; ++j) {
            const long long *S = &h[256 * 5 + j * 4];
            a3 += (double)(S[0] - h[(j + 3) * 4 + 2]);
            zt += (double)(S[1] - S[0]);
            zs += (double)(S[2] - S[1]);
            x2 += (double)(S[3] - h[(j + 2) * 4 + 2]);
            ++c2;
        }
        fprintf(stderr, "[backsolve stamps] streamer: x_{j+3} seen %.2f us after its publication, z_j published %.2f us later, finisher has z_j %.2f us "
                "later; finisher past x_{j+2} %.2f us after that block's publication\n", a3 / c2 / 100.0, zt / c2 / 100.0, zs / c2 / 100.0, x2 / c2 / 100.0);
        fprintf(stderr, "[backsolve stamps] nb %d: publish -> seen %.2f us, seen -> barrier %.2f us, barrier -> publish %.2f us, step %.2f us; "
                "the finisher starts polling %.2f us after the publication\n", nb, seen / cnt / 100.0, bar / cnt / 100.0, dot / cnt / 100.0,
                hop / cnt / 100.0, late / cnt / 100.0);
    }
    return 0;
}

}
```

### morbit.jl_amd/csrc/chol.hip

```cpp
#include <chrono>

#include "common.hpp"

namespace mrbf {

int debug_diag(mrbf_ctx *ctx, const double *A128_dev, int reps, float *ms_per_call, unsigned long long *stamps_host);
int launch_pad_identity(mrbf_ctx *ctx, double *A, int64_t n, int64_t npad, int64_t ld);

int potrf_lower(mrbf_ctx *ctx, int impl, int64_t n, double *A, int64_t lda, int *info_host) {
    int *dinfo;
    MRBF_TRY(get_buf(ctx, S_INFO, (size_t)4, &dinfo));
    const int64_t npad = round_up(n, 128);
    if (impl == 0) impl = (lda >= npad) ? ((npad >= ctx->mega.min && npad <= ctx->mega.max) ? 3 : 2) : 1;
    if (impl == 2 || impl == 3) {
        if (lda < npad) return fail(ctx, MRBF_EHIP, "built-in Cholesky needs lda >= round_up(n,128)");
        MRBF_TRY(launch_pad_identity(ctx, A, n, npad, lda));
        PotrfOpts opt;
        opt.impl = impl;
        opt.any_size = true;
        MRBF_TRY(potrf_blocked_tall(ctx, npad, npad, A, lda, dinfo, nullptr, opt));
    } else {
        MRBF_BLAS(ctx, rocsolver_dpotrf(ctx->blas, rocblas_fill_lower, (int)n, A, (int)lda, dinfo));
    }
    MRBF_HIP(ctx, hipMemcpyAsync(info_host, dinfo, sizeof(int), hipMemcpyDeviceToHost, ctx->stream));
    MRBF_HIP(ctx, hipStreamSynchronize(ctx->stream));
    MRBF_TRY(mega_collect_stat(ctx));
    return 0;
}

}

using namespace mrbf;

extern "C" int32_t mrbf_debug_potrf(mrbf_ctx *ctx, int64_t n, double *A, int32_t impl, int32_t *info, float *ms) {
    if (!ctx) return -1;
    if (n <= 0) return -2;
    if (!A) return -3;
    (void)hipSetDevice(ctx->device);
    const int64_t npad = round_up(n, 128);
    double *dA;
    MRBF_TRY(get_buf(ctx, S_PHI, (size_t)npad * npad, &dA));
    const hipMemcpyKind in = is_device_ptr(A) ? hipMemcpyDeviceToDevice : hipMemcpyHostToDevice;
    const hipMemcpyKind out = is_device_ptr(A) ? hipMemcpyDeviceToDevice : hipMemcpyDeviceToHost;
    MRBF_HIP(ctx, hipMemcpy2DAsync(dA, (size_t)npad * sizeof(double), A, (size_t)n * sizeof(double), (size_t)n * sizeof(double),
                                   (size_t)n, in, ctx->stream));
    int hinfo = 0;
    static const double host_trace_ms = mrbf_env("MRBF_MEGA_HOSTTRACE") ? atof(mrbf_env("MRBF_MEGA_HOSTTRACE")) : 0.0;
    auto now_ms = []() { return std::chrono::duration<double, std::milli>(std::chrono::steady_clock::now().time_since_epoch()).count(); };
    const double h0 = now_ms();
    MRBF_HIP(ctx, hipEventRecord(ctx->ev[0], ctx->stream));
    const double h1 = now_ms();
    MRBF_TRY(potrf_lower(ctx, impl, n, dA, npad, &hinfo));
    const double h2 = now_ms();
    MRBF_HIP(ctx, hipEventRecord(ctx->ev[1], ctx->stream));
    MRBF_HIP(ctx, hipEventSynchronize(ctx->ev[1]));
    const double h3 = now_ms();
    if (host_trace_ms > 0.0 && h3 - h0 > host_trace_ms)
        fprintf(stderr, "mrbf_debug_potrf host trace (n %lld): record ev0 %.3f ms | potrf_lower incl. sync %.3f | record ev1 + sync %.3f\n", (long long)n,
                h1 - h0, h2 - h1, h3 - h2);
    if (ms) MRBF_HIP(ctx, hipEventElapsedTime(ms, ctx->ev[0], ctx->ev[1]));
    if (info) *info = hinfo;
    MRBF_HIP(ctx, hipMemcpy2DAsync(A, (size_t)n * sizeof(double), dA, (size_t)npad * sizeof(double), (size_t)n * sizeof(double),
                                   (size_t)n, out, ctx->stream));
    MRBF_HIP(ctx, hipStreamSynchronize(ctx->stream));
    return MRBF_OK;
}

extern "C" int32_t mrbf_debug_diag(mrbf_ctx *ctx, const double *A128, int32_t reps, float *ms_per_call, double *shader_cycles,
                                   double *realtime_us) {
    if (!ctx) return -1;
    if (!A128) return -2;
    (void)hipSetDevice(ctx->device);
    const double *dA;
    MRBF_TRY(stage_in(ctx, S_STAGE_A, A128, 128 * 128, &dA));
    unsigned long long st[6] = {0, 0, 0, 0, 0, 0};
    float ms = 0;
    MRBF_TRY(debug_diag(ctx, dA, reps, &ms, st));
    if (ms_per_call) *ms_per_call = ms;
    if (shader_cycles) *shader_cycles = (double)st[0];
    if (realtime_us) *realtime_us = (double)st[1] / 100.0;
    if (mrbf_env("MRBF_DIAG_VERBOSE"))
        fprintf(stderr, "diag segments (cycles over 128 columns, wave 0): barrier %llu read %llu critical %llu rest %llu\n", st[2], st[3],
                st[4], st[5]);
    return MRBF_OK;
}
```

### morbit.jl_amd/csrc/chol_blocked.hip

```cpp
#include "common.hpp"
#include "mega_gemm.hpp"

namespace mrbf {

typedef double v4d __attribute__((ext_vector_type(4)));
typedef double v2d __attribute__((ext_vector_type(2)));

constexpr int CNB = 128;

enum { UPD_LOWER_SUB = 0, UPD_OVERWRITE = 1, UPD_FULL_SUB = 2, UPD_COLUMN_SUB = 3 };
int launch_diag(mrbf_ctx *ctx, hipStream_t st, double *Ajj, int64_t lda, double *Linv, int *dinfo, int col0);

template <int TM, int MODE>
__global__ __launch_bounds__(256, 2) void chol_update_kernel(const double *__restrict__ A, int64_t lda,
                                                             const double *__restrict__ B, int64_t ldb,
                                                             double *__restrict__ C, int64_t ldc, int K,
                                                             const int *__restrict__ info, int mt_sq = 0, int ntiles_total = 0,
                                                             const double *__restrict__ cvec = nullptr, double cs = 0.0, int64_t cn = 0) {
    constexpr int NJ = (TM == 128) ? 4 : 2;
    __shared__ __attribute__((aligned(16))) double smem[mega::NSTG * mega::STG];
    if (info && *info != 0) return;
    if (MODE == UPD_OVERWRITE || MODE == UPD_COLUMN_SUB) __builtin_amdgcn_s_setprio(2);
    const int tid = threadIdx.x, lane = tid & 63, wave = tid >> 6;
    const int l15 = lane & 15, l4 = lane >> 4;
    const int tile_end = (MODE == UPD_LOWER_SUB && ntiles_total > 0) ? ntiles_total : (int)blockIdx.x + 1;
    for (int bid = blockIdx.x; bid < tile_end; bid += gridDim.x) {
    int ti, tj;
    if (MODE == UPD_LOWER_SUB) {
        const int ntri = mt_sq * (mt_sq + 1) / 2;
        if (bid < ntri || mt_sq == 0) {
            int t = (int)((sqrt(8.0 * (double)bid + 1.0) - 1.0) * 0.5);
            while ((t + 1) * (t + 2) / 2 <= bid) ++t;
            while (t * (t + 1) / 2 > bid) --t;
            ti = t;
            tj = bid - t * (t + 1) / 2;
        } else {
            ti = mt_sq + (bid - ntri) / mt_sq;
            tj = (bid - ntri) % mt_sq;
        }
    } else {
        ti = blockIdx.x;
        tj = blockIdx.y;
    }
    const int64_t I0 = (int64_t)ti * TM, J0 = (int64_t)tj * 128;
    const int ioff = (TM == 128) ? (wave >> 1) * 64 : 0;
    const int joff = (TM == 128) ? (wave & 1) * 64 : wave * 32;

    v4d acc[NJ][4];
#pragma unroll
    for (int j = 0; j < NJ; ++j)
#pragma unroll
        for (int i = 0; i < 4; ++i) acc[j][i] = (v4d){0.0, 0.0, 0.0, 0.0};

    asm volatile("s_waitcnt vmcnt(0)" ::: "memory");
    constexpr bool NEG_START = (MODE == UPD_LOWER_SUB);
    if (NEG_START) {
#pragma unroll
        for (int j = 0; j < NJ; ++j)
#pragma unroll
            for (int r = 0; r < 4; ++r) {
                const int64_t gj = J0 + joff + j * 16 + l4 + 4 * r;
#pragma unroll
                for (int i = 0; i < 4; ++i) acc[j][i][r] = -C[(I0 + ioff + i * 16 + l15) + gj * ldc];
            }
    }
    mega::gemm_acc<TM>(A + I0, lda, B + J0, ldb, K, acc, smem);
    double cvi[4] = {0.0, 0.0, 0.0, 0.0}, cei[4] = {0.0, 0.0, 0.0, 0.0};
    if (MODE == UPD_LOWER_SUB && cvec) {
#pragma unroll
        for (int i = 0; i < 4; ++i) {
            const int64_t gi = I0 + ioff + i * 16 + l15;
            cvi[i] = cs * cvec[gi];
            cei[i] = gi < cn ? cs : 0.0;
        }
    }
#pragma unroll
    for (int j = 0; j < NJ; ++j) {
        double cv[4][4];
        double cvj[4] = {0.0, 0.0, 0.0, 0.0}, cej[4] = {0.0, 0.0, 0.0, 0.0};
        if (MODE == UPD_LOWER_SUB && cvec) {
#pragma unroll
            for (int r = 0; r < 4; ++r) {
                const int64_t gj = J0 + joff + j * 16 + l4 + 4 * r;
                cvj[r] = cvec[gj];
                cej[r] = gj < cn ? 1.0 : 0.0;
            }
        }
        if (MODE != UPD_OVERWRITE && !NEG_START) {
#pragma unroll
            for (int r = 0; r < 4; ++r) {
                const int64_t gj = J0 + joff + j * 16 + l4 + 4 * r;
#pragma unroll
                for (int i = 0; i < 4; ++i) cv[r][i] = C[(I0 + ioff + i * 16 + l15) + gj * ldc];
            }
        }
#pragma unroll
        for (int r = 0; r < 4; ++r) {
            const int64_t gj = J0 + joff + j * 16 + l4 + 4 * r;
#pragma unroll
            for (int i = 0; i < 4; ++i) {
                const int64_t gi = I0 + ioff + i * 16 + l15;
                double *dst = C + gi + gj * ldc;
                if (MODE == UPD_OVERWRITE) {
                    *dst = acc[j][i][r];
                } else if (MODE == UPD_FULL_SUB) {
                    *dst = cv[r][i] - acc[j][i][r];
                } else if (MODE == UPD_COLUMN_SUB) {
                    if (gi >= gj) *dst = cv[r][i] - acc[j][i][r];
                } else {
                    double x = -acc[j][i][r];
                    if (cvec) x -= fma(cei[i], cvj[r], cvi[i] * cej[r]);
                    if (ti != tj || gi >= gj) *dst = x;
                }
            }
        }
    }
    if (bid + (int)gridDim.x < tile_end) __syncthreads();
    }
}

struct __attribute__((aligned(16))) DiagShared {
    double col[2][2 * CNB];
    double rinv[2];
    int sbad;
    unsigned long long seg[4];
    int stamp;
};

__device__ __forceinline__ double fast_rsqrt(double x) {
    double y = __builtin_amdgcn_rsq(x);
    const double h = 0.5 * x;
#pragma unroll
    for (int it = 0; it < 3; ++it) y = y * fma(-h, y * y, 1.5);
    return y;
}

template <int KV, bool STAMP>
__device__ __forceinline__ void diag_phase(double (&a)[8][8], DiagShared &sh, int ti, int tj, int half, int &buf, int &bad) {
    constexpr int KN = (KV < 7) ? KV + 1 : 7;
    double piv = 0.0;
    if (half == 0) piv = __shfl(a[KV][KV], tj, 16);
#pragma unroll 1
    for (int kk = 0; kk < 16; ++kk) {
        const int k = KV * 16 + kk;
        const bool st = STAMP && threadIdx.x < 64;
        unsigned long long s0 = 0, s1 = 0, s2 = 0, s3 = 0;
        if (st) s0 = __builtin_amdgcn_s_memtime();
        __syncthreads();
        if (st) s1 = __builtin_amdgcn_s_memtime();
        double lj[8];
#pragma unroll
        for (int v = KV; v < 8; ++v) lj[v] = sh.col[buf][tj + 16 * v];
        if (half == 0) {
            double li[8];
#pragma unroll
            for (int u = KV; u < 8; ++u) li[u] = sh.col[buf][ti + 16 * u];
            if (st) {
                asm volatile("s_waitcnt lgkmcnt(0)" ::: "memory");
                s2 = __builtin_amdgcn_s_memtime();
            }
            if (kk < 15) {
                if (tj > kk) piv = fma(-lj[KV], lj[KV], piv);
                if (tj == kk + 1) {
                    const int kn = k + 1;
                    double rinv = 0.0;
                    if (piv > 0.0) {
                        rinv = fast_rsqrt(piv);
                    } else if (bad == 0) {
                        bad = kn + 1;
                    }
                    if (ti == 0) sh.rinv[buf ^ 1] = rinv;
                    double w[8];
#pragma unroll
                    for (int u = 0; u < 8; ++u) {
                        const int i = ti + 16 * u;
                        double val = 0.0;
                        if (u >= KV && i >= kn) {
                            val = fma(-li[u], lj[KV], a[u][KV]) * rinv;
                            a[u][KV] = val;
                        }
                        w[u] = val;
                    }
#pragma unroll
                    for (int u = 0; u < 8; ++u) sh.col[buf ^ 1][ti + 16 * u] = w[u];
                }
            } else if (KV < 7) {
                if (tj == 0) {
                    const int kn = k + 1;
                    const double pv = __shfl(fma(-li[KN], lj[KN], a[KN][KN]), 0, 16);
                    double rinv = 0.0;
                    if (pv > 0.0) {
                        rinv = fast_rsqrt(pv);
                    } else if (bad == 0) {
                        bad = kn + 1;
                    }
                    if (ti == 0) sh.rinv[buf ^ 1] = rinv;
                    double w[8];
#pragma unroll
                    for (int u = 0; u < 8; ++u) {
                        double val = 0.0;
                        if (u >= KN) {
                            val = fma(-li[u], lj[KN], a[u][KN]) * rinv;
                            a[u][KN] = val;
                        }
                        w[u] = val;
                    }
#pragma unroll
                    for (int u = 0; u < 8; ++u) sh.col[buf ^ 1][ti + 16 * u] = w[u];
                }
            }
            if (st) {
                asm volatile("s_waitcnt lgkmcnt(0)" ::: "memory");
                s3 = __builtin_amdgcn_s_memtime();
            }
            const bool own_next = (kk < 15) ? (tj == kk + 1) : (KV < 7 && tj == 0);
            const bool lowtri = ti >= tj;
#pragma unroll
            for (int v = KV; v < 8; ++v) {
                double ljv = lj[v];
                if (v == KV) ljv = (tj > kk && !(own_next && kk < 15)) ? ljv : 0.0;
                if (v == KN && KV < 7) ljv = (own_next && kk == 15) ? 0.0 : ljv;
                a[v][v] = fma(lowtri ? -li[v] : 0.0, ljv, a[v][v]);
#pragma unroll
                for (int u = v + 1; u < 8; ++u) a[u][v] = fma(-li[u], ljv, a[u][v]);
            }
            if (st && threadIdx.x == 0) {
                asm volatile("" ::"v"(a[7][7]));
                const unsigned long long s4 = __builtin_amdgcn_s_memtime();
                sh.seg[0] += s1 - s0;
                sh.seg[1] += s2 - s1;
                sh.seg[2] += s3 - s2;
                sh.seg[3] += s4 - s3;
            }
        } else {
            const double rinv = sh.rinv[buf];
            const double ljk = (tj > kk) ? lj[KV] : 0.0;
#pragma unroll
            for (int u = 0; u <= KV; ++u) {
                const double erk = sh.col[buf][CNB + ti + 16 * u] * rinv;
                if (tj == kk) a[u][KV] = erk;
                a[u][KV] = fma(-erk, ljk, a[u][KV]);
#pragma unroll
                for (int v = KV + 1; v < 8; ++v) a[u][v] = fma(-erk, lj[v], a[u][v]);
            }
            if (kk < 15) {
                if (tj == kk + 1) {
#pragma unroll
                    for (int u = 0; u < 8; ++u) sh.col[buf ^ 1][CNB + ti + 16 * u] = (u <= KV) ? a[u][KV] : 0.0;
                }
            } else if (KV < 7) {
                if (tj == 0) {
#pragma unroll
                    for (int u = 0; u < 8; ++u) sh.col[buf ^ 1][CNB + ti + 16 * u] = (u <= KN) ? a[u][KN] : 0.0;
                }
            }
        }
        buf ^= 1;
    }
}

template <bool STAMP>
__global__ __launch_bounds__(512) void chol_diag_kernel(double *__restrict__ A, int64_t lda, double *__restrict__ Linv,
                                                        int *__restrict__ info, int col0,
                                                        unsigned long long *__restrict__ stamps) {
    __shared__ DiagShared sh;
    if (*info != 0) return;
    unsigned long long t0 = 0, r0 = 0;
    if (STAMP) {
        if (threadIdx.x == 0) sh.seg[0] = sh.seg[1] = sh.seg[2] = sh.seg[3] = 0;
        __syncthreads();
        t0 = __builtin_amdgcn_s_memtime();
        r0 = __builtin_amdgcn_s_memrealtime();
    }
    const int tid = threadIdx.x, ti = tid & 15, tj = (tid >> 4) & 15, half = tid >> 8;
    double a[8][8];
#pragma unroll
    for (int v = 0; v < 8; ++v)
#pragma unroll
        for (int u = 0; u < 8; ++u) {
            const int i = ti + 16 * u, j = tj + 16 * v;
            if (half == 0)
                a[u][v] = (i >= j) ? A[i + (int64_t)j * lda] : 0.0;
            else
                a[u][v] = (i == j) ? 1.0 : 0.0;
        }
    int buf = 0, bad = 0;
    if (tj == 0) {
        if (half == 0) {
            const double pv = __shfl(a[0][0], 0, 16);
            double rinv = 0.0;
            if (pv > 0.0) {
                rinv = fast_rsqrt(pv);
            } else {
                bad = 1;
            }
            if (ti == 0) sh.rinv[0] = rinv;
#pragma unroll
            for (int u = 0; u < 8; ++u) {
                a[u][0] *= rinv;
                sh.col[0][ti + 16 * u] = a[u][0];
            }
        } else {
#pragma unroll
            for (int u = 0; u < 8; ++u) sh.col[0][CNB + ti + 16 * u] = (u == 0) ? a[0][0] : 0.0;
        }
    }
    diag_phase<0, STAMP>(a, sh, ti, tj, half, buf, bad);
    diag_phase<1, STAMP>(a, sh, ti, tj, half, buf, bad);
    diag_phase<2, STAMP>(a, sh, ti, tj, half, buf, bad);
    diag_phase<3, STAMP>(a, sh, ti, tj, half, buf, bad);
    diag_phase<4, STAMP>(a, sh, ti, tj, half, buf, bad);
    diag_phase<5, STAMP>(a, sh, ti, tj, half, buf, bad);
    diag_phase<6, STAMP>(a, sh, ti, tj, half, buf, bad);
    diag_phase<7, STAMP>(a, sh, ti, tj, half, buf, bad);
    if (tid == 0) sh.sbad = 0x7fffffff;
    __syncthreads();
    if (bad) atomicMin(&sh.sbad, bad);
    __syncthreads();
    if (sh.sbad != 0x7fffffff) {
        if (tid == 0) *info = col0 + sh.sbad;
        return;
    }
#pragma unroll
    for (int v = 0; v < 8; ++v)
#pragma unroll
        for (int u = 0; u < 8; ++u) {
            const int i = ti + 16 * u, j = tj + 16 * v;
            if (half == 0) {
                if (i >= j) A[i + (int64_t)j * lda] = a[u][v];
            } else {
                Linv[j + i * CNB] = (j >= i) ? a[u][v] : 0.0;
            }
        }
    if (STAMP && threadIdx.x == 0) {
        stamps[0] = __builtin_amdgcn_s_memtime() - t0;
        stamps[1] = __builtin_amdgcn_s_memrealtime() - r0;
        for (int q = 0; q < 4; ++q) stamps[2 + q] = sh.seg[q];
    }
}

__global__ void pad_identity_kernel(double *__restrict__ A, int64_t n, int64_t npad, int64_t ld) {
    const int64_t idx = (int64_t)blockIdx.x * blockDim.x + threadIdx.x;
    const int64_t pw = npad - n;
    if (idx >= npad * pw) return;
    const int64_t j = n + idx / npad, i = idx % npad;
    A[i + j * ld] = (i == j) ? 1.0 : 0.0;
    if (i < n) A[j + i * ld] = 0.0;
}

int launch_pad_identity(mrbf_ctx *ctx, double *A, int64_t n, int64_t npad, int64_t ld) {
    if (npad == n) return 0;
    const int64_t cnt = npad * (npad - n);
    hipLaunchKernelGGL(pad_identity_kernel, dim3((unsigned)((cnt + 255) / 256)), dim3(256), 0, ctx->stream, A, n, npad, ld);
    MRBF_HIP(ctx, hipGetLastError());
    return 0;
}

int debug_diag(mrbf_ctx *ctx, const double *A128_dev, int reps, float *ms_per_call, unsigned long long *stamps_host) {
    const bool with_stamps = reps > 0;
    if (reps < 0) reps = -reps;
    double *W, *Linv;
    int *dinfo;
    unsigned long long *st;
    MRBF_TRY(get_buf(ctx, S_PHI, (size_t)CNB * CNB * reps, &W));
    MRBF_TRY(get_buf(ctx, S_CHOL_WS, (size_t)CNB * CNB, &Linv));
    MRBF_TRY(get_buf(ctx, S_INFO, (size_t)4, &dinfo));
    MRBF_TRY(get_buf(ctx, S_MISC, (size_t)8, (double **)&st));
    for (int r = 0; r < reps; ++r)
        MRBF_HIP(ctx, hipMemcpyAsync(W + (size_t)r * CNB * CNB, A128_dev, sizeof(double) * CNB * CNB, hipMemcpyDeviceToDevice, ctx->stream));
    MRBF_HIP(ctx, hipMemsetAsync(dinfo, 0, sizeof(int), ctx->stream));
    MRBF_HIP(ctx, hipEventRecord(ctx->ev[0], ctx->stream));
    for (int r = 0; r < reps; ++r)
        if (ctx->diag_impl != 1)
            launch_diag(ctx, ctx->stream, W + (size_t)r * CNB * CNB, (int64_t)CNB, Linv, dinfo, 0);
        else if (with_stamps)
            hipLaunchKernelGGL(chol_diag_kernel<true>, dim3(1), dim3(512), 0, ctx->stream, W + (size_t)r * CNB * CNB, (int64_t)CNB, Linv,
                               dinfo, 0, st);
        else
            hipLaunchKernelGGL(chol_diag_kernel<false>, dim3(1), dim3(512), 0, ctx->stream, W + (size_t)r * CNB * CNB, (int64_t)CNB, Linv,
                               dinfo, 0, (unsigned long long *)nullptr);
    MRBF_HIP(ctx, hipEventRecord(ctx->ev[1], ctx->stream));
    MRBF_HIP(ctx, hipEventSynchronize(ctx->ev[1]));
    float t;
    MRBF_HIP(ctx, hipEventElapsedTime(&t, ctx->ev[0], ctx->ev[1]));
    *ms_per_call = t / reps;
    MRBF_HIP(ctx, hipMemcpy(stamps_host, st, 6 * sizeof(unsigned long long), hipMemcpyDeviceToHost));
    return 0;
}

int launch_update_lower(mrbf_ctx *ctx, const double *A, int64_t lda, const double *B, int64_t ldb, double *C, int64_t ldc, int64_t nt,
                        int K, const double *cvec, double cs, int64_t cn) {
    if (nt <= 0 || K <= 0) return 0;
    hipLaunchKernelGGL((chol_update_kernel<128, UPD_LOWER_SUB>), dim3((unsigned)(nt * (nt + 1) / 2)), dim3(256), 0, ctx->stream, A,
                       lda, B, ldb, C, ldc, K, (const int *)nullptr, (int)nt, 0, cvec, cs, cn);
    MRBF_HIP(ctx, hipGetLastError());
    return 0;
}

int potrf_blocked_tall(mrbf_ctx *ctx, int64_t ncols, int64_t mrows, double *A, int64_t lda, int *dinfo, double *linv_all, PotrfOpts opt) {
    if (ncols % CNB != 0 || mrows % CNB != 0 || mrows < ncols || (lda & 1) || (reinterpret_cast<uintptr_t>(A) & 15))
        return fail(ctx, MRBF_EHIP, "potrf_blocked needs 128-padded, 16-byte aligned storage (ncols=%lld mrows=%lld lda=%lld)",
                    (long long)ncols, (long long)mrows, (long long)lda);
    const int impl = opt.impl != 0 ? opt.impl : ctx->chol_impl;
    if ((impl == 3 || (impl == 0 && ncols <= ctx->mega.max)) && (opt.any_size || ncols >= ctx->mega.min))
        return potrf_mega_tall(ctx, ncols, mrows, A, lda, dinfo, linv_all, opt);
    double *Lone = nullptr;
    if (!linv_all) MRBF_TRY(get_buf(ctx, S_CHOL_WS, (size_t)CNB * CNB, &Lone));
    hipStream_t S = ctx->stream, M = ctx->bulk_stream, P = ctx->panel_stream;
    hipEvent_t evStart = ctx->evx[0], evT = ctx->evx[1], evU2 = ctx->evx[2], evEnd = ctx->evx[3];
    const bool single = ncols <= 4 * CNB;
    if (single) M = P = S;
    MRBF_HIP(ctx, hipMemsetAsync(dinfo, 0, sizeof(int), S));
    if (!single) {
        MRBF_HIP(ctx, hipEventRecord(evStart, S));
        MRBF_HIP(ctx, hipStreamWaitEvent(P, evStart, 0));
        MRBF_HIP(ctx, hipStreamWaitEvent(M, evStart, 0));
    }
    const int nb = (int)(ncols / CNB);
    bool have_u2 = false;
    int w0 = 0, W = 1;
    for (int j = 0; j < nb; ++j) {
        const int64_t c = (int64_t)j * CNB;
        if (j == w0) {
            const int64_t rem = ncols - c;
            W = (rem > 4800) ? 4 : (rem > 2400 ? 2 : 1);
            if (ctx->chol_window > 0) W = ctx->chol_window;
        }
        const bool last_in_window = (j == w0 + W - 1) || (j == nb - 1);
        const int kpan = (int)((j - w0 + 1) * CNB);
        const int64_t cw = (int64_t)w0 * CNB;
        double *Ajj = A + c + c * lda;
        double *Linv = linv_all ? linv_all + (size_t)j * CNB * CNB : Lone;
        if (ctx->diag_impl == 1)
            hipLaunchKernelGGL(chol_diag_kernel<false>, dim3(1), dim3(512), 0, P, Ajj, lda, Linv, dinfo, (int)c,
                               (unsigned long long *)nullptr);
        else
            launch_diag(ctx, P, Ajj, lda, Linv, dinfo, (int)c);
        const int64_t m = mrows - c - CNB;
        if (m <= 0) break;
        double *A21 = A + (c + CNB) + c * lda;
        hipLaunchKernelGGL((chol_update_kernel<64, UPD_OVERWRITE>), dim3((unsigned)(m / 64), 1), dim3(256), 0, P, A21, lda, Linv,
                           (int64_t)CNB, A21, lda, CNB, dinfo);
        if (c + CNB >= ncols) break;
        if (!single) MRBF_HIP(ctx, hipEventRecord(evT, P));
        if (have_u2 && !single) {
            MRBF_HIP(ctx, hipStreamWaitEvent(P, evU2, 0));
            have_u2 = false;
        }
        const double *Pw = A + (c + CNB) + cw * lda;
        double *A22 = A + (c + CNB) + (c + CNB) * lda;
        hipLaunchKernelGGL((chol_update_kernel<64, UPD_COLUMN_SUB>), dim3((unsigned)(m / 64), 1), dim3(256), 0, P, Pw, lda, Pw, lda,
                           A22, lda, kpan, dinfo);
        if (last_in_window) {
            const int64_t mt2 = (ncols - c - 2 * CNB) / CNB;
            if (mt2 > 0) {
                if (!single) MRBF_HIP(ctx, hipStreamWaitEvent(M, evT, 0));
                const int64_t mx = (mrows - ncols) / CNB;
                const int64_t rem_next = ncols - c - CNB;
                int Wn = (rem_next > 4800) ? 4 : (rem_next > 2400 ? 2 : 1);
                if (ctx->chol_window > 0) Wn = ctx->chol_window;
                const int64_t na = std::min<int64_t>(Wn, mt2);
                const double *P2 = A + (c + 2 * CNB) + cw * lda;
                double *C2 = A + (c + 2 * CNB) + (c + 2 * CNB) * lda;
                hipLaunchKernelGGL((chol_update_kernel<128, UPD_LOWER_SUB>),
                                   dim3((unsigned)(na * (na + 1) / 2 + (mt2 - na + mx) * na)), dim3(256), 0, M, P2, lda, P2, lda, C2, lda,
                                   kpan, dinfo, (int)na);
                if (!single) MRBF_HIP(ctx, hipEventRecord(evU2, M));
                have_u2 = true;
                const int64_t mb2 = mt2 - na;
                if (mb2 > 0) {
                    const double *P3 = P2 + na * CNB;
                    double *C3 = C2 + na * CNB + na * CNB * lda;
                    const int64_t nt3 = mb2 * (mb2 + 1) / 2 + mx * mb2;
                    const int64_t g3 = (ctx->bulk_grid > 0 && nt3 > ctx->bulk_grid) ? ctx->bulk_grid : nt3;
                    hipLaunchKernelGGL((chol_update_kernel<128, UPD_LOWER_SUB>), dim3((unsigned)g3), dim3(256), 0, M, P3, lda, P3, lda,
                                       C3, lda, kpan, dinfo, (int)mb2, (int)nt3);
                }
            }
            w0 = j + 1;
        }
    }
    MRBF_HIP(ctx, hipGetLastError());
    if (!single) {
        MRBF_HIP(ctx, hipEventRecord(evEnd, P));
        MRBF_HIP(ctx, hipStreamWaitEvent(S, evEnd, 0));
        MRBF_HIP(ctx, hipEventRecord(evStart, M));
        MRBF_HIP(ctx, hipStreamWaitEvent(S, evStart, 0));
    }
    return 0;
}

constexpr int BS_LD = 65;
template <int KB>
__device__ __forceinline__ void tile_tdot(const double *__restrict__ Tl, int64_t ldt, const double *xs ,
                                          double *res , double *stage ,
                                          double *part ) {
    const int tid = threadIdx.x, c = tid & 127, g = tid >> 7;
    double acc[KB];
#pragma unroll
    for (int l = 0; l < KB; ++l) acc[l] = 0.0;
    for (int h = 0; h < 2; ++h) {
        double v[32];
#pragma unroll
        for (int p = 0; p < 32; ++p) v[p] = Tl[(int64_t)(p * 4 + (tid >> 6)) * ldt + 64 * h + (tid & 63)];
        __syncthreads();
#pragma unroll
        for (int p = 0; p < 32; ++p) stage[(p * 4 + (tid >> 6)) * BS_LD + (tid & 63)] = v[p];
        __syncthreads();
#pragma unroll 8
        for (int r = 0; r < 32; ++r) {
            const double t = stage[c * BS_LD + 32 * g + r];
#pragma unroll
            for (int l = 0; l < KB; ++l) acc[l] = fma(t, xs[l * CNB + 64 * h + 32 * g + r], acc[l]);
        }
    }
#pragma unroll
    for (int l = 0; l < KB; ++l) part[l * 256 + tid] = acc[l];
    __syncthreads();
    if (g == 0) {
#pragma unroll
        for (int l = 0; l < KB; ++l) res[l * CNB + c] = part[l * 256 + c] + part[l * 256 + 128 + c];
    }
}

template <int KB>
__global__ __launch_bounds__(256) void chol_backsolve_kernel(const double *__restrict__ L, int64_t lda, const double *__restrict__ linv_all,
                                                             double *__restrict__ Y, int64_t ldy, int k0, int i ,
                                                             int prologue) {
    __shared__ double xs[KB * CNB];
    __shared__ double res[KB * CNB];
    __shared__ double part[KB * 256];
    __shared__ double stage[CNB * BS_LD];
    const int tid = threadIdx.x;
    const int j = blockIdx.x;
    if (!prologue) {
        for (int t = tid; t < KB * CNB; t += 256) xs[t] = Y[(int64_t)(k0 + t / CNB) * ldy + (int64_t)i * CNB + (t % CNB)];
        __syncthreads();
        tile_tdot<KB>(L + (int64_t)i * CNB + (int64_t)j * CNB * lda, lda, xs, res, stage, part);
        __syncthreads();
        for (int t = tid; t < KB * CNB; t += 256) {
            double *yp = Y + (int64_t)(k0 + t / CNB) * ldy + (int64_t)j * CNB + (t % CNB);
            const double v = *yp - res[t];
            *yp = v;
            xs[t] = v;
        }
        if (j != i - 1) return;
        __syncthreads();
    } else {
        for (int t = tid; t < KB * CNB; t += 256) xs[t] = Y[(int64_t)(k0 + t / CNB) * ldy + (int64_t)i * CNB + (t % CNB)];
        __syncthreads();
    }
    const int jb = prologue ? i : i - 1;
    tile_tdot<KB>(linv_all + (size_t)jb * CNB * CNB, CNB, xs, res, stage, part);
    __syncthreads();
    for (int t = tid; t < KB * CNB; t += 256) Y[(int64_t)(k0 + t / CNB) * ldy + (int64_t)jb * CNB + (t % CNB)] = res[t];
}

int backsolve_blocked(mrbf_ctx *ctx, int64_t npad, const double *L, int64_t lda, const double *linv_all, double *Y, int64_t ldy, int k) {
    const int nb = (int)(npad / CNB);
    for (int k0 = 0; k0 < k; k0 += 4) {
        const int kb = std::min(4, k - k0);
#define MRBF_BS(KBV, grid, ii, pro)                                                                                         \
    hipLaunchKernelGGL((chol_backsolve_kernel<KBV>), dim3((unsigned)(grid)), dim3(256), 0, ctx->stream, L, lda, linv_all, Y, ldy, \
                       k0, ii, pro)
        for (int i = nb - 1; i >= 0; --i) {
            const bool pro = (i == nb - 1);
            if (pro) {
                if (kb == 1) MRBF_BS(1, 1, i, 1); else if (kb == 2) MRBF_BS(2, 1, i, 1); else if (kb == 3) MRBF_BS(3, 1, i, 1); else MRBF_BS(4, 1, i, 1);
            }
            if (i > 0) {
                if (kb == 1) MRBF_BS(1, i, i, 0); else if (kb == 2) MRBF_BS(2, i, i, 0); else if (kb == 3) MRBF_BS(3, i, i, 0); else MRBF_BS(4, i, i, 0);
            }
        }
#undef MRBF_BS
    }
    MRBF_HIP(ctx, hipGetLastError());
    return 0;
}

}
```

### morbit.jl_amd/csrc/solve.hip

```cpp
#include "common.hpp"
#include "small.hpp"

namespace mrbf {

__global__ void fit_publish_kernel(const int *__restrict__ dinfo, const double *__restrict__ scal, const unsigned long long *__restrict__ dstat,
                                   int *__restrict__ hflags, double *__restrict__ hscal, unsigned long long *__restrict__ hstat) {
    const int t = threadIdx.x;
    if (t < 4) hflags[t] = dinfo[t];
    if (t >= 4 && t < 6 && scal) hscal[t - 4] = scal[t - 4];
    if (t == 6 && dstat && hstat) hstat[0] = dstat[0];
}

__global__ void fill_saddle_kernel(const double *__restrict__ Pi, int64_t n, int q, double *__restrict__ S, int64_t N) {
    const int64_t idx = (int64_t)blockIdx.x * blockDim.x + threadIdx.x;
    const int64_t tot = n * q;
    if (idx < tot) {
        const int64_t i = idx % n;
        const int t = (int)(idx / n);
        const double v = Pi[idx];
        S[i + (n + t) * N] = v;
        S[(n + t) + i * N] = v;
    } else if (idx < tot + (int64_t)q * q) {
        const int64_t r = idx - tot;
        S[(n + r % q) + (n + r / q) * N] = 0.0;
    }
}

__global__ void rhs_from_values_kernel(const double *__restrict__ Y, int64_t n, int k, double *__restrict__ B, int64_t N) {
    const int64_t idx = (int64_t)blockIdx.x * blockDim.x + threadIdx.x;
    if (idx >= N * k) return;
    const int64_t i = idx % N;
    const int l = (int)(idx / N);
    B[idx] = (i < n) ? Y[i * k + l] : 0.0;
}

__global__ void scatter_solution_kernel(const double *__restrict__ B, int64_t ldB, int64_t n, int64_t npad, int k, int q,
                                        int64_t lam_row0, double *__restrict__ W, double *__restrict__ Wc,
                                        double *__restrict__ lam, const double *__restrict__ lamsrc, int64_t ldlam) {
    const int64_t idx = (int64_t)blockIdx.x * blockDim.x + threadIdx.x;
    if (idx < npad * k) {
        const int64_t i = idx % npad;
        const int l = (int)(idx / npad);
        const double v = (i < n) ? B[i + l * ldB] : 0.0;
        Wc[idx] = v;
        if (i < n) W[i * k + l] = v;
    } else if (idx < npad * k + (int64_t)q * k) {
        const int64_t r = idx - npad * k;
        const int t = (int)(r % q), l = (int)(r / q);
        lam[(int64_t)t * k + l] = lamsrc[lam_row0 + t + l * ldlam];
    }
}

__global__ void copy_upper_kernel(const double *__restrict__ A, int64_t lda, int q, double *__restrict__ R) {
    const int idx = blockIdx.x * blockDim.x + threadIdx.x;
    if (idx >= q * q) return;
    const int i = idx % q, j = idx / q;
    R[idx] = (i <= j) ? A[i + (int64_t)j * lda] : 0.0;
}

__global__ void trace_kernel(const double *__restrict__ G, int q, double *__restrict__ out) {
    __shared__ double red[256];
    double s = 0.0;
    for (int i = threadIdx.x; i < q; i += 256) s += G[i + (int64_t)i * q];
    red[threadIdx.x] = s;
    __syncthreads();
    for (int w = 128; w > 0; w >>= 1) {
        if ((int)threadIdx.x < w) red[threadIdx.x] += red[threadIdx.x + w];
        __syncthreads();
    }
    if (threadIdx.x == 0) out[0] = red[0];
}

__global__ void max_abs_kernel(const double *__restrict__ v, int64_t cnt, double *__restrict__ out) {
    __shared__ double red[256];
    double s = 0.0;
    for (int64_t i = threadIdx.x; i < cnt; i += 256) s = fmax(s, fabs(v[i]));
    red[threadIdx.x] = s;
    __syncthreads();
    for (int w = 128; w > 0; w >>= 1) {
        if ((int)threadIdx.x < w) red[threadIdx.x] = fmax(red[threadIdx.x], red[threadIdx.x + w]);
        __syncthreads();
    }
    if (threadIdx.x == 0) out[0] = red[0];
}

__global__ void residual_kernel(const double *__restrict__ a, const double *__restrict__ b, int64_t cnt,
                                double *__restrict__ out) {
    __shared__ double r0[256], r1[256];
    double s0 = 0.0, s1 = 0.0;
    for (int64_t i = threadIdx.x; i < cnt; i += 256) {
        const double df = a[i] - b[i];
        s0 = fma(df, df, s0);
        s1 = fma(b[i], b[i], s1);
    }
    r0[threadIdx.x] = s0;
    r1[threadIdx.x] = s1;
    __syncthreads();
    for (int w = 128; w > 0; w >>= 1) {
        if ((int)threadIdx.x < w) {
            r0[threadIdx.x] += r0[threadIdx.x + w];
            r1[threadIdx.x] += r1[threadIdx.x + w];
        }
        __syncthreads();
    }
    if (threadIdx.x == 0) {
        out[0] = r0[0];
        out[1] = r1[0];
    }
}

static inline unsigned nblk(int64_t cnt) { return (unsigned)((cnt + 255) / 256); }

void model_block_release(mrbf_ctx *ctx, void *p, size_t bytes, bool slab) {
    if (!ctx) {
        (void)hipFree(p);
        return;
    }
    model_pool_release(ctx->model_pool, p, bytes, slab, [](void *q) { (void)hipFree(q); });
}

void destroy_model(mrbf_ctx *ctx, mrbf_model *M) {
    if (!M) return;
    if (ctx && (M->block || M->slab)) --ctx->live_models;
    if (M->block) model_block_release(ctx, M->block, M->block_bytes);
    if (M->slab && slab_drop(M->slab)) {
        model_block_release(ctx, M->slab->p, M->slab->bytes, true);
        delete M->slab;
    }
    delete M;
}

void model_set_dims(mrbf_model *M, int64_t n, int d, int k, int kid, double a, double b, int deg) {
    M->n = n;
    M->d = d;
    M->k = k;
    M->deg = deg;
    M->q = poly_dim(d, deg);
    M->npad = round_up(n, 128);
    M->dpad = (d <= 64) ? 64 : (d <= 128 ? 128 : (d <= 256 ? 256 : (int)round_up(d, 16)));
    M->kp = make_kp(kid, a, b);
}

size_t model_block_layout(const mrbf_model *M, size_t off[7]) {
    const size_t cnt[7] = {(size_t)M->n * M->d, (size_t)M->npad * M->dpad, (size_t)M->npad, (size_t)M->dpad, (size_t)M->n * M->k,
                           (size_t)M->npad * M->k, (size_t)std::max(M->q, 1) * M->k};
    size_t at = 0;
    for (int i = 0; i < 7; ++i) {
        off[i] = at;
        at += (std::max<size_t>(cnt[i], 2) * sizeof(double) + 255) & ~size_t(255);
    }
    return at;
}

void model_carve(mrbf_model *M, char *base, const size_t off[7]) {
    M->C = (double *)(base + off[0]);
    M->Xc = (double *)(base + off[1]);
    M->sq = (double *)(base + off[2]);
    M->mean = (double *)(base + off[3]);
    M->W = (double *)(base + off[4]);
    M->Wc = (double *)(base + off[5]);
    M->lam = (double *)(base + off[6]);
}

int model_block_acquire(mrbf_ctx *ctx, size_t total, void **p, size_t *bytes) {
    hipError_t e = hipSuccess;
    auto alloc = [&](size_t b) -> void * {
        void *q = nullptr;
        e = hipMalloc(&q, b);
        return e == hipSuccess ? q : nullptr;
    };
    if (!model_pool_acquire(ctx->model_pool, total, p, bytes, alloc, [](void *q) { (void)hipFree(q); }))
        return fail(ctx, MRBF_ENOMEM, "model allocation failed: %s", hipGetErrorString(e));
    return 0;
}

int build_model_shell(mrbf_ctx *ctx, int64_t n, int d, int k, const double *Cdev, int kid, double a, double b, int deg,
                      mrbf_model **out) {
    mrbf_model *M = new mrbf_model();
    model_set_dims(M, n, d, k, kid, a, b, deg);
    size_t off[7];
    const size_t total = model_block_layout(M, off);
    const int rc_block = model_block_acquire(ctx, total, &M->block, &M->block_bytes);
    if (rc_block != 0) {
        delete M;
        return rc_block;
    }
    ++ctx->live_models;
    M->owner = ctx;
    model_carve(M, (char *)M->block, off);
    auto init = [&]() -> int {
        if (Cdev != M->C)
            MRBF_HIP(ctx, hipMemcpyAsync(M->C, Cdev, (size_t)n * d * sizeof(double), hipMemcpyDeviceToDevice, ctx->stream));
        MRBF_TRY(launch_center_pad(ctx, M->C, n, d, nullptr, M->mean, M->Xc, M->npad, M->dpad, M->sq));
        return 0;
    };
    const int rc = init();
    if (rc != 0) {
        destroy_model(ctx, M);
        return rc;
    }
    *out = M;
    return 0;
}

static int read_info(mrbf_ctx *ctx, const int *dinfo, int *hinfo) {
    MRBF_HIP(ctx, hipMemcpyAsync(hinfo, dinfo, sizeof(int), hipMemcpyDeviceToHost, ctx->stream));
    MRBF_HIP(ctx, hipStreamSynchronize(ctx->stream));
    return 0;
}

void fill_small_prob(const mrbf_ctx *ctx, const mrbf_model *M, const double *Y, double *ws, int *flags, double *scal, int *cl, smallfit::Prob *P);
static int fit_lu(mrbf_ctx *ctx, mrbf_model *M, const double *Y, mrbf_fit_info *info) {
    const int64_t n = M->n, N = n + M->q;
    const int k = M->k, q = M->q;
    double *S, *B, *Pi = nullptr;
    int *ipiv, *dinfo;
    MRBF_TRY(get_buf(ctx, S_PHI, (size_t)N * N, &S));
    MRBF_TRY(get_buf(ctx, S_RHS, (size_t)N * k, &B));
    MRBF_TRY(get_buf(ctx, S_IPIV, (size_t)N, &ipiv));
    MRBF_TRY(get_buf(ctx, S_INFO, (size_t)4, &dinfo));
    hipLaunchKernelGGL(rhs_from_values_kernel, dim3(nblk(N * k)), dim3(256), 0, ctx->stream, Y, n, k, B, N);
    MRBF_HIP(ctx, hipEventRecord(ctx->ev[0], ctx->stream));
    MRBF_TRY(launch_gram(ctx, ctx->gram_mode, M->C, M->Xc, M->sq, n, M->npad, M->d, M->dpad, M->kp, S, N));
    MRBF_HIP(ctx, hipEventRecord(ctx->ev[1], ctx->stream));
    if (q > 0) {
        MRBF_TRY(get_buf(ctx, S_PI, (size_t)n * q, &Pi));
        MRBF_TRY(launch_poly_matrix(ctx, M->C, n, M->d, q, Pi, n));
        hipLaunchKernelGGL(fill_saddle_kernel, dim3(nblk(n * q + (int64_t)q * q)), dim3(256), 0, ctx->stream, Pi, n, q, S, N);
    }
    MRBF_HIP(ctx, hipGetLastError());
    MRBF_HIP(ctx, hipEventRecord(ctx->ev[5], ctx->stream));
    MRBF_BLAS(ctx, rocsolver_dgetrf(ctx->blas, (int)N, (int)N, S, (int)N, ipiv, dinfo));
    MRBF_HIP(ctx, hipEventRecord(ctx->ev[2], ctx->stream));
    int hinfo = 0;
    MRBF_TRY(read_info(ctx, dinfo, &hinfo));
    info->factor_info = hinfo;
    info->path = MRBF_PATH_LU;
    if (hinfo != 0) return fail(ctx, MRBF_ESINGULAR, "saddle matrix is singular (getrf info = %d, N = %lld)", hinfo, (long long)N);
    MRBF_BLAS(ctx, rocsolver_dgetrs(ctx->blas, rocblas_operation_none, (int)N, k, S, (int)N, ipiv, B, (int)N));
    hipLaunchKernelGGL(scatter_solution_kernel, dim3(nblk(M->npad * k + (int64_t)q * k)), dim3(256), 0, ctx->stream, B, N, n,
                       M->npad, k, q, n, M->W, M->Wc, M->lam, B, N);
    MRBF_HIP(ctx, hipGetLastError());
    MRBF_HIP(ctx, hipEventRecord(ctx->ev[3], ctx->stream));
    MRBF_HIP(ctx, hipEventSynchronize(ctx->ev[3]));
    MRBF_HIP(ctx, hipEventElapsedTime(&info->ms_gram, ctx->ev[0], ctx->ev[1]));
    MRBF_HIP(ctx, hipEventElapsedTime(&info->ms_project, ctx->ev[1], ctx->ev[5]));
    MRBF_HIP(ctx, hipEventElapsedTime(&info->ms_factor, ctx->ev[5], ctx->ev[2]));
    MRBF_HIP(ctx, hipEventElapsedTime(&info->ms_solve, ctx->ev[2], ctx->ev[3]));
    return 0;
}

static int fit_small_lu(mrbf_ctx *ctx, mrbf_model *M, const double *Y, mrbf_fit_info *info) {
    smallfit::Prob P;
    double *ws, *scal;
    int *flags;
    MRBF_TRY(get_buf(ctx, S_SMALL_LU, small_lu_scratch_doubles(M->n, M->q), &ws));
    MRBF_TRY(get_buf(ctx, S_SMALL_FLAGS, (size_t)4, &flags));
    MRBF_TRY(get_buf(ctx, S_MISC, (size_t)8, &scal));
    fill_small_prob(ctx, M, Y, ws, flags, scal, nullptr, &P);
    int hflags_local[4] = {0, 0, 0, 0};
    int *hflags = ctx->hpin ? reinterpret_cast<int *>(ctx->hpin + HPIN_SMALL_FLAGS) : hflags_local;
    MRBF_HIP(ctx, hipEventRecord(ctx->ev[0], ctx->stream));
    MRBF_TRY(launch_small_lu(ctx, &P, 1, nullptr));
    MRBF_HIP(ctx, hipEventRecord(ctx->ev[1], ctx->stream));
    MRBF_HIP(ctx, hipMemcpyAsync(hflags, flags, 4 * sizeof(int), hipMemcpyDeviceToHost, ctx->stream));
    MRBF_HIP(ctx, hipStreamSynchronize(ctx->stream));
    info->factor_info = hflags[0];
    info->path = MRBF_PATH_LU;
    if (hflags[0] != 0)
        return fail(ctx, MRBF_ESINGULAR, "saddle matrix is singular (getrf info = %d, N = %lld)", hflags[0], (long long)(M->n + M->q));
    MRBF_HIP(ctx, hipEventElapsedTime(&info->ms_factor, ctx->ev[0], ctx->ev[1]));
    return 0;
}

__global__ void scale_rows_pinv_kernel(double *__restrict__ T, int N, int k, const double *__restrict__ sv) {
    const int idx = blockIdx.x * blockDim.x + threadIdx.x;
    if (idx >= N * k) return;
    const int i = idx % N;
    const double s = sv[i], cut = (double)N * 2.220446049250313e-16 * sv[0];
    T[idx] = (s > cut) ? T[idx] / s : 0.0;
}

static int fit_minnorm(mrbf_ctx *ctx, mrbf_model *M, const double *Y, mrbf_fit_info *info) {
    const int64_t n = M->n, N = n + M->q;
    const int k = M->k, q = M->q;
    const double one = 1.0, zero = 0.0;
    double *S, *B, *Pi, *U, *VT, *sv, *E, *T;
    int *dinfo;
    MRBF_TRY(get_buf(ctx, S_PHI, (size_t)N * N, &S));
    MRBF_TRY(get_buf(ctx, S_RHS, (size_t)N * k, &B));
    MRBF_TRY(get_buf(ctx, S_PI, (size_t)n * q, &Pi));
    MRBF_TRY(get_buf(ctx, S_Q1, (size_t)N * N, &U));
    MRBF_TRY(get_buf(ctx, S_W1, (size_t)N * N, &VT));
    MRBF_TRY(get_buf(ctx, S_TAU, (size_t)2 * N, &sv));
    MRBF_TRY(get_buf(ctx, S_T1, (size_t)N * k, &T));
    MRBF_TRY(get_buf(ctx, S_INFO, (size_t)4, &dinfo));
    E = sv + N;
    hipLaunchKernelGGL(rhs_from_values_kernel, dim3(nblk(N * k)), dim3(256), 0, ctx->stream, Y, n, k, B, N);
    MRBF_HIP(ctx, hipEventRecord(ctx->ev[0], ctx->stream));
    MRBF_TRY(launch_gram(ctx, ctx->gram_mode, M->C, M->Xc, M->sq, n, M->npad, M->d, M->dpad, M->kp, S, N));
    MRBF_HIP(ctx, hipEventRecord(ctx->ev[1], ctx->stream));
    MRBF_TRY(launch_poly_matrix(ctx, M->C, n, M->d, q, Pi, n));
    hipLaunchKernelGGL(fill_saddle_kernel, dim3(nblk(n * q + (int64_t)q * q)), dim3(256), 0, ctx->stream, Pi, n, q, S, N);
    MRBF_HIP(ctx, hipGetLastError());
    MRBF_BLAS(ctx, rocsolver_dgesvd(ctx->blas, rocblas_svect_all, rocblas_svect_all, (int)N, (int)N, S, (int)N, sv, U, (int)N, VT,
                                    (int)N, E, rocblas_outofplace, dinfo));
    MRBF_HIP(ctx, hipEventRecord(ctx->ev[2], ctx->stream));
    int hinfo = 0;
    MRBF_TRY(read_info(ctx, dinfo, &hinfo));
    info->factor_info = hinfo;
    info->path = MRBF_PATH_MINNORM;
    if (hinfo != 0) return fail(ctx, MRBF_ESINGULAR, "SVD of the saddle matrix did not converge (info = %d)", hinfo);
    MRBF_BLAS(ctx, rocblas_dgemm(ctx->blas, rocblas_operation_transpose, rocblas_operation_none, (int)N, k, (int)N, &one, U, (int)N,
                                 B, (int)N, &zero, T, (int)N));
    hipLaunchKernelGGL(scale_rows_pinv_kernel, dim3(nblk(N * k)), dim3(256), 0, ctx->stream, T, (int)N, k, sv);
    MRBF_BLAS(ctx, rocblas_dgemm(ctx->blas, rocblas_operation_transpose, rocblas_operation_none, (int)N, k, (int)N, &one, VT, (int)N,
                                 T, (int)N, &zero, B, (int)N));
    hipLaunchKernelGGL(scatter_solution_kernel, dim3(nblk(M->npad * k + (int64_t)q * k)), dim3(256), 0, ctx->stream, B, N, n,
                       M->npad, k, q, n, M->W, M->Wc, M->lam, B, N);
    MRBF_HIP(ctx, hipGetLastError());
    MRBF_HIP(ctx, hipEventRecord(ctx->ev[3], ctx->stream));
    MRBF_HIP(ctx, hipEventSynchronize(ctx->ev[3]));
    MRBF_HIP(ctx, hipEventElapsedTime(&info->ms_gram, ctx->ev[0], ctx->ev[1]));
    MRBF_HIP(ctx, hipEventElapsedTime(&info->ms_factor, ctx->ev[1], ctx->ev[2]));
    MRBF_HIP(ctx, hipEventElapsedTime(&info->ms_solve, ctx->ev[2], ctx->ev[3]));
    return 0;
}

int backsolve_blocked(mrbf_ctx *ctx, int64_t npad, const double *L, int64_t lda, const double *linv_all, double *Y, int64_t ldy, int k);
int backsolve_persistent(mrbf_ctx *ctx, int64_t npad, const double *L, int64_t lda, const double *linv_all, double *Y, int64_t ldy, int k,
                         int *status);
int launch_update_lower(mrbf_ctx *ctx, const double *A, int64_t lda, const double *B, int64_t ldb, double *C, int64_t ldc, int64_t nt, int K,
                        const double *cvec, double cs, int64_t cn);
int launch_pad_identity(mrbf_ctx *ctx, double *A, int64_t n, int64_t npad, int64_t ld);
int tsmm_tn(mrbf_ctx *ctx, int64_t n, int p, int r, double alpha, const double *A, int64_t lda, const double *B, int64_t ldb, double beta,
            double *C, int64_t ldc);
int symm_panel(mrbf_ctx *ctx, int64_t n, int64_t npad, int q, const double *Phi, int64_t ld, const double *Q, int64_t ldq, double *W,
               int64_t ldwo, bool const_first, double cval);

__global__ void set_rhs_rows_kernel(double *__restrict__ A, int64_t ld, int64_t npad, int xt, const double *__restrict__ B, int k) {
    const int64_t idx = (int64_t)blockIdx.x * blockDim.x + threadIdx.x;
    if (idx >= npad * xt) return;
    const int l = (int)(idx % xt);
    const int64_t i = idx / xt;
    A[(npad + l) + i * ld] = (l < k) ? B[i + (int64_t)l * npad] : 0.0;
}
__global__ void get_rhs_rows_kernel(const double *__restrict__ A, int64_t ld, int64_t npad, double *__restrict__ B, int k) {
    const int64_t idx = (int64_t)blockIdx.x * blockDim.x + threadIdx.x;
    if (idx >= npad * k) return;
    const int l = (int)(idx % k);
    const int64_t i = idx / k;
    B[i + (int64_t)l * npad] = A[(npad + l) + i * ld];
}
__global__ void xc_to_tall_kernel(const double *__restrict__ Xc, int64_t n, int d, int dpad, double *__restrict__ Tall, int64_t lt,
                                  int64_t dq) {
    const int64_t idx = (int64_t)blockIdx.x * blockDim.x + threadIdx.x;
    if (idx >= n * d) return;
    const int64_t i = idx / d;
    const int t = (int)(idx % d);
    Tall[(dq + i) + (int64_t)t * lt] = Xc[i * dpad + t];
}
__global__ void build_q1_kernel(const double *__restrict__ Tall, int64_t lt, int64_t dq, int64_t n, int64_t npad, int q,
                                double *__restrict__ Q1) {
    const int64_t idx = (int64_t)blockIdx.x * blockDim.x + threadIdx.x;
    if (idx >= npad * q) return;
    const int64_t i = idx % npad;
    const int t = (int)(idx / npad);
    double v = 0.0;
    if (i < n) v = (t == 0) ? 1.0 / sqrt((double)n) : Tall[(dq + i) + (int64_t)(t - 1) * lt];
    Q1[idx] = v;
}
__global__ void shift_from_trace_kernel(double *__restrict__ scal, double nphi0, double nmq, int *__restrict__ flags) {
    const double mu = (nphi0 - scal[0]) / nmq;
    const bool ok = mu > 0.0 && mu < 1e300;
    scal[1] = ok ? mu : 1.0;
    flags[2] = ok ? 0 : 1;
}

__global__ void build_panels_kernel(const double *__restrict__ Q1, const double *__restrict__ W, const double *__restrict__ scal,
                                    int64_t n, int64_t npad, int q, int K2, int skip, double *__restrict__ PA, double *__restrict__ PB,
                                    double *__restrict__ v0) {
    const int64_t idx = (int64_t)blockIdx.x * blockDim.x + threadIdx.x;
    if (idx >= npad * K2) return;
    const double mu = scal[1];
    const int64_t i = idx % npad;
    const int t = (int)(idx / npad);
    const int qq = q - skip;
    double a = 0.0, b = 0.0;
    if (i < n && t < 2 * qq) {
        const int tt = t % qq + skip;
        const double qv = Q1[i + (int64_t)tt * npad];
        const double vv = fma(-0.5 * mu, qv, W[i + (int64_t)tt * npad]);
        a = (t < qq) ? qv : vv;
        b = (t < qq) ? vv : qv;
    }
    PA[idx] = a;
    PB[idx] = b;
    if (skip && t == 0) v0[i] = (i < n) ? fma(-0.5 * mu, Q1[i], W[i]) : 0.0;
}
__global__ __launch_bounds__(64) void finish_lambda_kernel(double *__restrict__ T1, int q, int k, double sqrtn, const double *__restrict__ mean) {
    __shared__ double part[64];
    const int l = blockIdx.x, tid = threadIdx.x;
    if (l >= k) return;
    double acc = 0.0;
    for (int t = 1 + tid; t < q; t += 64) acc = fma(mean[t - 1], T1[t + (int64_t)l * q], acc);
    part[tid] = acc;
    __syncthreads();
    if (tid == 0) {
        double dsum = 0.0;
        for (int u = 0; u < 64; ++u) dsum += part[u];
        T1[(int64_t)l * q] = T1[(int64_t)l * q] / sqrtn - dsum;
    }
}

__global__ __launch_bounds__(256) void sub_qt_kernel(double *__restrict__ B, int64_t ldb, const double *__restrict__ Q, int64_t ldq,
                                                     const double *__restrict__ T, int64_t n, int q, int k) {
    __shared__ double part[4][64];
    const int r = threadIdx.x & 63, g = threadIdx.x >> 6;
    const int64_t row = (int64_t)blockIdx.x * 64 + r;
    for (int l = 0; l < k; ++l) {
        double s0 = 0.0, s1 = 0.0;
        if (row < n) {
            int t = g;
            for (; t + 4 < q; t += 8) {
                s0 = fma(Q[row + (int64_t)t * ldq], T[t + (int64_t)l * q], s0);
                s1 = fma(Q[row + (int64_t)(t + 4) * ldq], T[t + 4 + (int64_t)l * q], s1);
            }
            if (t < q) s0 = fma(Q[row + (int64_t)t * ldq], T[t + (int64_t)l * q], s0);
        }
        __syncthreads();
        part[g][r] = s0 + s1;
        __syncthreads();
        if (g == 0 && row < n) B[row + (int64_t)l * ldb] -= (part[0][r] + part[1][r]) + (part[2][r] + part[3][r]);
    }
}

__global__ __launch_bounds__(256) void apply_linv_t_kernel(const double *__restrict__ inv, int d, double *__restrict__ X, int64_t ldx, int k) {
    __shared__ double bs[128];
    const int j = threadIdx.x & 127, half = threadIdx.x >> 7;
    __shared__ double part[2][128];
    for (int l = 0; l < k; ++l) {
        __syncthreads();
        if (threadIdx.x < 128) bs[threadIdx.x] = threadIdx.x < d ? X[threadIdx.x + (int64_t)l * ldx] : 0.0;
        __syncthreads();
        double v = 0.0;
        if (j < d) {
            const double *col = inv + (int64_t)j * 128;
            for (int i = j + half; i < d; i += 2) v = fma(col[i], bs[i], v);
        }
        part[half][j] = v;
        __syncthreads();
        if (half == 0 && j < d) X[j + (int64_t)l * ldx] = part[0][j] + part[1][j];
    }
}

__global__ __launch_bounds__(256) void trsm_lt_small_kernel(const double *__restrict__ L, int64_t ldl, int d, double *__restrict__ X,
                                                            int64_t ldx, int k) {
    __shared__ double xs[256];
    const int j = threadIdx.x;
    for (int l = 0; l < k; ++l) {
        double v = j < d ? X[j + (int64_t)l * ldx] : 0.0;
        for (int c = d - 1; c >= 0; --c) {
            if (j == c) {
                v /= L[c + (int64_t)c * ldl];
                xs[c] = v;
            }
            __syncthreads();
            if (j < c) v -= L[c + (int64_t)j * ldl] * xs[c];
            __syncthreads();
        }
        if (j < d) X[j + (int64_t)l * ldx] = v;
    }
}

__global__ __launch_bounds__(256) void tail_dots_kernel(const double *__restrict__ Bw, int64_t ldb, const double *__restrict__ Q1,
                                                        const double *__restrict__ Wm, int64_t ldq, int64_t n, int q, int k,
                                                        double *__restrict__ part) {
    __shared__ double ws[64 * 16];
    __shared__ double red[4][2][64];
    const int tid = threadIdx.x, g = tid >> 6, lane = tid & 63;
    const int64_t R0 = (int64_t)blockIdx.x * 64;
    for (int e = tid; e < 64 * k; e += 256) {
        const int i = e & 63, l = e >> 6;
        ws[e] = R0 + i < n ? Bw[R0 + i + (int64_t)l * ldb] : 0.0;
    }
    __syncthreads();
    for (int a0 = 0; a0 < q; a0 += 64) {
        const int a = a0 + lane;
        double qv[16], wv[16];
#pragma unroll
        for (int u = 0; u < 16; ++u) {
            const int64_t r = R0 + 16 * g + u;
            const bool ok = a < q && r < n;
            qv[u] = ok ? Q1[r + (int64_t)a * ldq] : 0.0;
            wv[u] = ok ? Wm[r + (int64_t)a * ldq] : 0.0;
        }
        for (int l = 0; l < k; ++l) {
            double s0 = 0.0, s1 = 0.0;
#pragma unroll
            for (int u = 0; u < 16; ++u) {
                const double w = ws[l * 64 + 16 * g + u];
                s0 = fma(qv[u], w, s0);
                s1 = fma(wv[u], w, s1);
            }
            __syncthreads();
            red[g][0][lane] = s0;
            red[g][1][lane] = s1;
            __syncthreads();
            if (g == 0 && a < q) {
                double *o = part + ((size_t)blockIdx.x * 2 * k + l) * q + a;
                o[0] = (red[0][0][lane] + red[1][0][lane]) + (red[2][0][lane] + red[3][0][lane]);
                o[(size_t)k * q] = (red[0][1][lane] + red[1][1][lane]) + (red[2][1][lane] + red[3][1][lane]);
            }
        }
    }
}

__global__ __launch_bounds__(1024) void tail_coeff_kernel(const double *__restrict__ part, int nch, int q, int k, int d, const double *__restrict__ T1,
                                                         const double *__restrict__ G, double cg, const double *__restrict__ LxInv,
                                                         double sqrtn, const double *__restrict__ mean, double *__restrict__ T2,
                                                         double *__restrict__ lam_out) {
    __shared__ double t2[129 * 16], zz[129 * 16], xx[129 * 16];
    const int tid = threadIdx.x, nthr = blockDim.x;
    for (int e = tid; e < 2 * k * q; e += nthr) {
        double sv = 0.0;
        for (int c0 = 0; c0 < nch; c0 += 32) {
            double v[32];
#pragma unroll
            for (int u = 0; u < 32; ++u) v[u] = c0 + u < nch ? part[(size_t)(c0 + u) * 2 * k * q + e] : 0.0;
#pragma unroll
            for (int u = 0; u < 32; ++u) sv += v[u];
        }
        if (e < k * q)
            t2[e] = sv;
        else
            zz[e - k * q] = sv;
    }
    __syncthreads();
    for (int e = tid; e < k * q; e += nthr) {
        const int l = e / q, a = e % q;
        double corr = 0.0;
        for (int b0 = 0; b0 < q; b0 += 16) {
            double gv[16];
#pragma unroll
            for (int u = 0; u < 16; ++u) gv[u] = b0 + u < q ? G[b0 + u + (int64_t)a * q] : 0.0;
#pragma unroll
            for (int u = 0; u < 16; ++u) corr = fma(gv[u], b0 + u < q ? t2[l * q + b0 + u] : 0.0, corr);
        }
        zz[e] = T1[a + (int64_t)l * q] - zz[e] + cg * corr;
        T2[a + (int64_t)l * q] = t2[e];
    }
    __syncthreads();
    for (int e = tid; e < k * d; e += nthr) {
        const int l = e / d, j = e % d;
        double acc = 0.0;
        for (int i0 = j; i0 < d; i0 += 16) {
            double iv[16];
#pragma unroll
            for (int u = 0; u < 16; ++u) iv[u] = i0 + u < d ? LxInv[i0 + u + (int64_t)j * 128] : 0.0;
#pragma unroll
            for (int u = 0; u < 16; ++u) acc = fma(iv[u], i0 + u < d ? zz[l * q + 1 + i0 + u] : 0.0, acc);
        }
        xx[l * q + 1 + j] = acc;
    }
    __syncthreads();
    if (tid < k) {
        const int l = tid;
        double dsum = 0.0;
        for (int t0 = 1; t0 < q; t0 += 16) {
            double mv[16];
#pragma unroll
            for (int u = 0; u < 16; ++u) mv[u] = t0 + u < q ? mean[t0 + u - 1] : 0.0;
#pragma unroll
            for (int u = 0; u < 16; ++u) dsum = fma(mv[u], t0 + u < q ? xx[l * q + t0 + u] : 0.0, dsum);
        }
        xx[l * q] = zz[l * q] / sqrtn - dsum;
    }
    __syncthreads();
    for (int e = tid; e < k * q; e += nthr) lam_out[(e % q) + (int64_t)(e / q) * q] = xx[e];
}

__global__ __launch_bounds__(256) void tail_apply_kernel(const double *__restrict__ Bw, int64_t ldb, const double *__restrict__ Q1, int64_t ldq,
                                                         const double *__restrict__ T2, const double *__restrict__ lamsrc, int64_t n,
                                                         int64_t npad, int q, int k, double *__restrict__ W, double *__restrict__ Wc,
                                                         double *__restrict__ lam) {
    __shared__ double part4[4][64];
    const int tid = threadIdx.x, r = tid & 63, g = tid >> 6;
    const int64_t row = (int64_t)blockIdx.x * 64 + r;
    for (int l = 0; l < k; ++l) {
        double s0 = 0.0, s1 = 0.0;
        if (row < n) {
            int t = g;
            for (; t + 4 < q; t += 8) {
                s0 = fma(Q1[row + (int64_t)t * ldq], T2[t + (int64_t)l * q], s0);
                s1 = fma(Q1[row + (int64_t)(t + 4) * ldq], T2[t + 4 + (int64_t)l * q], s1);
            }
            if (t < q) s0 = fma(Q1[row + (int64_t)t * ldq], T2[t + (int64_t)l * q], s0);
        }
        __syncthreads();
        part4[g][r] = s0 + s1;
        __syncthreads();
        if (g == 0 && row < npad) {
            const double v = row < n ? Bw[row + (int64_t)l * ldb] - ((part4[0][r] + part4[1][r]) + (part4[2][r] + part4[3][r])) : 0.0;
            Wc[row + (int64_t)l * npad] = v;
            if (row < n) W[row * k + l] = v;
        }
    }
    if (blockIdx.x == 0)
        for (int e = tid; e < q * k; e += 256) lam[(int64_t)(e % q) * k + e / q] = lamsrc[(e % q) + (int64_t)(e / q) * q];
}

static int fit_chol(mrbf_ctx *ctx, mrbf_model *M, const double *Y, mrbf_fit_info *info, int *not_pd, int *gave_up, int impl = 0) {
    const int64_t n = M->n, npad = M->npad;
    const int k = M->k, q = M->q, d = M->d;
    const double one = 1.0, mhalf = -0.5;
    *not_pd = 0;
    *gave_up = 0;
    if (impl == 0) impl = ctx->chol_impl;
    const bool builtin = impl != 1;
    PotrfOpts popt;
    popt.impl = impl;
    const int xt = builtin ? (int)round_up(k, 128) : 0;
    const int64_t ld = npad + xt;
    double *Phi, *B;
    int *dinfo;
    MRBF_TRY(get_buf(ctx, S_PHI, (size_t)ld * npad, &Phi));
    MRBF_TRY(get_buf(ctx, S_RHS, (size_t)npad * k, &B));
    MRBF_TRY(get_buf(ctx, S_INFO, (size_t)4, &dinfo));
    MRBF_HIP(ctx, hipMemsetAsync(dinfo, 0, 4 * sizeof(int), ctx->stream));
    const bool tailq = q > 1 && tail_basis_applies(M) && M->k == k;
    if (!tailq) hipLaunchKernelGGL(rhs_from_values_kernel, dim3(nblk(npad * k)), dim3(256), 0, ctx->stream, Y, n, k, B, npad);
    double *Q1 = nullptr, *Wm = nullptr, *G = nullptr, *T1 = nullptr, *scal = nullptr, *Tall = nullptr, *LxInv = nullptr;
    int64_t lt = 0, dq = 0;
    info->mu = 0.0;
    hipStream_t main_stream = ctx->stream;
    const bool side = q > 0 && ctx->panel_stream && ctx->panel_stream != main_stream && n >= 2048;
    const bool fused = q > 0 && gram_w_applies(ctx, M) && (q == 1 || round_up(d, 128) == 128);
    if (q > 0) {
        MRBF_TRY(get_buf(ctx, S_Q1, (size_t)npad * q, &Q1));
        MRBF_TRY(get_buf(ctx, S_W1, (size_t)npad * q, &Wm));
        MRBF_TRY(get_buf(ctx, S_G, (size_t)q * q, &G));
        MRBF_TRY(get_buf(ctx, S_T1, (size_t)q * k, &T1));
        MRBF_TRY(get_buf(ctx, S_MISC, (size_t)8, &scal));
        if (side) {
            MRBF_HIP(ctx, hipEventRecord(ctx->evx[0], main_stream));
            MRBF_HIP(ctx, hipStreamWaitEvent(ctx->panel_stream, ctx->evx[0], 0));
            ctx->stream = ctx->panel_stream;
        }
        struct RestoreStream {
            mrbf_ctx *c;
            hipStream_t s;
            ~RestoreStream() { c->stream = s; }
        } restore{ctx, main_stream};
        if (tailq) {
            double *scratch;
            MRBF_TRY(get_buf(ctx, S_PI, tail_basis_scratch_doubles(), &scratch));
            MRBF_TRY(get_buf(ctx, S_QR_INV, (size_t)128 * 128, &LxInv));
            MRBF_TRY(launch_tail_basis(ctx, M, Y, scratch, LxInv, T1, Q1, B, builtin ? Phi : nullptr, ld, xt, dinfo));
        } else if (q > 1) {
            dq = round_up(d, 128);
            lt = dq + npad;
            MRBF_TRY(get_buf(ctx, S_PI, (size_t)lt * dq, &Tall));
            MRBF_HIP(ctx, hipMemsetAsync(Tall, 0, (size_t)lt * dq * sizeof(double), ctx->stream));
            hipLaunchKernelGGL(xc_to_tall_kernel, dim3(nblk(n * d)), dim3(256), 0, ctx->stream, M->Xc, n, d, M->dpad, Tall, lt, dq);
            MRBF_TRY(tsmm_tn(ctx, n, d, d, 1.0, Tall + dq, lt, Tall + dq, lt, 0.0, Tall, lt));
            MRBF_TRY(launch_pad_identity(ctx, Tall, d, dq, lt));
            if (dq == 128) MRBF_TRY(get_buf(ctx, S_QR_INV, (size_t)128 * 128, &LxInv));
            MRBF_TRY(potrf_blocked_tall(ctx, dq, lt, Tall, lt, dinfo + 1, LxInv, popt));
        }
        if (!tailq) hipLaunchKernelGGL(build_q1_kernel, dim3(nblk(npad * q)), dim3(256), 0, ctx->stream, Tall, lt, dq, n, npad, q, Q1);
        if (!fused) MRBF_HIP(ctx, hipMemsetAsync(Wm, 0, (size_t)npad * q * sizeof(double), ctx->stream));
        if (!tailq) {
            MRBF_TRY(tsmm_tn(ctx, n, q, k, 1.0, Q1, npad, B, npad, 0.0, T1, q));
            hipLaunchKernelGGL(sub_qt_kernel, dim3((unsigned)((n + 63) / 64)), dim3(256), 0, ctx->stream, B, npad, Q1, npad, T1, n, q, k);
            if (builtin) hipLaunchKernelGGL(set_rhs_rows_kernel, dim3(nblk(npad * xt)), dim3(256), 0, ctx->stream, Phi, ld, npad, xt, B, k);
        }
        if (side) MRBF_HIP(ctx, hipEventRecord(ctx->evx[1], ctx->stream));
    }
    ctx->stream = main_stream;
    MRBF_HIP(ctx, hipEventRecord(ctx->ev[0], ctx->stream));
    double *Wpart = nullptr, *rspart = nullptr;
    int nseg = 0;
    if (fused)
        MRBF_TRY(launch_gram_w(ctx, M, Phi, ld, &Wpart, &rspart, &nseg));
    else
        MRBF_TRY(launch_gram(ctx, ctx->gram_mode, M->C, M->Xc, M->sq, n, M->npad, M->d, M->dpad, M->kp, Phi, ld));
    MRBF_HIP(ctx, hipEventRecord(ctx->ev[1], ctx->stream));
    if (side) MRBF_HIP(ctx, hipStreamWaitEvent(ctx->stream, ctx->evx[1], 0));
    if (fused) {
        const int skip = (q > 1 && round_up(2 * (q - 1), 16) < round_up(2 * q, 16)) ? 1 : 0;
        const int K2 = (int)round_up(2 * (q - skip), 16);
        double *PA, *PB, *v0 = nullptr;
        MRBF_TRY(get_buf(ctx, S_STAGE_C, (size_t)npad * K2, &PA));
        MRBF_TRY(get_buf(ctx, S_STAGE_D, (size_t)npad * K2, &PB));
        if (skip) MRBF_TRY(get_buf(ctx, S_V0, (size_t)npad, &v0));
        MRBF_TRY(launch_projection_small(ctx, M, Wpart, rspart, nseg, LxInv, Q1, Wm, G, scal, dinfo, K2, skip, PA, PB, v0));
        MRBF_TRY(launch_update_lower(ctx, PA, npad, PB, npad, Phi, ld, npad / 128, K2, v0, 1.0 / std::sqrt((double)n), n));
    } else if (q > 0) {
        MRBF_TRY(symm_panel(ctx, n, npad, q, Phi, ld, Q1, npad, Wm, npad, true, 1.0 / std::sqrt((double)n)));
        MRBF_TRY(tsmm_tn(ctx, n, q, q, 1.0, Q1, npad, Wm, npad, 0.0, G, q));
        hipLaunchKernelGGL(trace_kernel, dim3(1), dim3(256), 0, ctx->stream, G, q, scal);
        MRBF_BLAS(ctx, rocblas_dgemm(ctx->blas, rocblas_operation_none, rocblas_operation_none, (int)n, q, q, &mhalf, Q1, (int)npad,
                                     G, q, &one, Wm, (int)npad));
        hipLaunchKernelGGL(shift_from_trace_kernel, dim3(1), dim3(1), 0, ctx->stream, scal, (double)n * M->kp.phi0,
                           (double)std::max<int64_t>(n - q, 1), dinfo);
        const int skip = (q > 1 && round_up(2 * (q - 1), 16) < round_up(2 * q, 16)) ? 1 : 0;
        const int K2 = (int)round_up(2 * (q - skip), 16);
        double *PA, *PB, *v0 = nullptr;
        MRBF_TRY(get_buf(ctx, S_STAGE_C, (size_t)npad * K2, &PA));
        MRBF_TRY(get_buf(ctx, S_STAGE_D, (size_t)npad * K2, &PB));
        if (skip) MRBF_TRY(get_buf(ctx, S_V0, (size_t)npad, &v0));
        hipLaunchKernelGGL(build_panels_kernel, dim3(nblk(npad * K2)), dim3(256), 0, ctx->stream, Q1, Wm, scal, n, npad, q, K2, skip, PA, PB, v0);
        MRBF_TRY(launch_update_lower(ctx, PA, npad, PB, npad, Phi, ld, npad / 128, K2, v0, 1.0 / std::sqrt((double)n), n));
    }
    MRBF_HIP(ctx, hipEventRecord(ctx->ev[2], ctx->stream));
    int hinfo = 0;
    double *linv_all = nullptr;
    if (builtin) {
        MRBF_TRY(get_buf(ctx, S_CHOL_WS, (size_t)npad * 128, &linv_all));
        MRBF_TRY(launch_pad_identity(ctx, Phi, n, npad, ld));
        if (q == 0) hipLaunchKernelGGL(set_rhs_rows_kernel, dim3(nblk(npad * xt)), dim3(256), 0, ctx->stream, Phi, ld, npad, xt, B, k);
        popt.xreal = k;
        popt.info_clean = true;
        MRBF_TRY(potrf_blocked_tall(ctx, npad, npad + xt, Phi, ld, dinfo, linv_all, popt));
        MRBF_HIP(ctx, hipEventRecord(ctx->ev[3], ctx->stream));
    } else {
        int *dpot;
        MRBF_TRY(get_buf(ctx, S_IPIV, (size_t)4, &dpot));
        MRBF_BLAS(ctx, rocsolver_dpotrf(ctx->blas, rocblas_fill_lower, (int)n, Phi, (int)ld, dpot));
        MRBF_HIP(ctx, hipMemcpyAsync(dinfo, dpot, sizeof(int), hipMemcpyDeviceToDevice, ctx->stream));
        MRBF_HIP(ctx, hipEventRecord(ctx->ev[3], ctx->stream));
    }
    double *T1w = nullptr;
    if (q > 0) MRBF_TRY(get_buf(ctx, S_T1W, (size_t)q * k, &T1w));
    auto solve_tail = [&](bool persistent) -> int {
        if (builtin) {
            hipLaunchKernelGGL(get_rhs_rows_kernel, dim3(nblk(npad * k)), dim3(256), 0, ctx->stream, Phi, ld, npad, B, k);
            if (persistent)
                MRBF_TRY(backsolve_persistent(ctx, npad, Phi, ld, linv_all, B, npad, k, dinfo + 3));
            else
                MRBF_TRY(backsolve_blocked(ctx, npad, Phi, ld, linv_all, B, npad, k));
        } else {
            MRBF_BLAS(ctx, rocsolver_dpotrs(ctx->blas, rocblas_fill_lower, (int)n, k, Phi, (int)ld, B, (int)npad));
        }
        static const int tail3 = mrbf_env("MRBF_TAIL3") ? atoi(mrbf_env("MRBF_TAIL3")) : 1;
        if (tail3 && q > 0 && q <= 129 && k <= 16 && (q == 1 || LxInv)) {
            const int nch = (int)(npad / 64);
            double *T2, *part;
            MRBF_TRY(get_buf(ctx, S_T2, (size_t)q * k, &T2));
            MRBF_TRY(get_buf(ctx, S_TAIL_PART, (size_t)nch * 2 * k * q, &part));
            hipLaunchKernelGGL(tail_dots_kernel, dim3((unsigned)nch), dim3(256), 0, ctx->stream, B, npad, Q1, Wm, npad, n, q, k, part);
            hipLaunchKernelGGL(tail_coeff_kernel, dim3(1), dim3(1024), 0, ctx->stream, part, nch, q, k, q > 1 ? d : 0, T1, G, fused ? 1.0 : 0.5, LxInv,
                               std::sqrt((double)n), M->mean, T2, T1w);
            hipLaunchKernelGGL(tail_apply_kernel, dim3((unsigned)nch), dim3(256), 0, ctx->stream, B, npad, Q1, npad, T2, T1w, n, M->npad, q, k, M->W,
                               M->Wc, M->lam);
            MRBF_HIP(ctx, hipGetLastError());
            return 0;
        }
        if (q > 0) {
            double *T2;
            MRBF_TRY(get_buf(ctx, S_T2, (size_t)q * k, &T2));
            MRBF_HIP(ctx, hipMemcpyAsync(T1w, T1, (size_t)q * k * sizeof(double), hipMemcpyDeviceToDevice, ctx->stream));
            MRBF_TRY(tsmm_tn(ctx, n, q, k, 1.0, Q1, npad, B, npad, 0.0, T2, q));
            hipLaunchKernelGGL(sub_qt_kernel, dim3((unsigned)((n + 63) / 64)), dim3(256), 0, ctx->stream, B, npad, Q1, npad, T2, n, q, k);
            MRBF_TRY(tsmm_tn(ctx, n, q, k, -1.0, Wm, npad, B, npad, 1.0, T1w, q));
            if (q > 1) {
                if (LxInv)
                    hipLaunchKernelGGL(apply_linv_t_kernel, dim3(1), dim3(256), 0, ctx->stream, LxInv, d, T1w + 1, (int64_t)q, k);
                else if (d <= 256)
                    hipLaunchKernelGGL(trsm_lt_small_kernel, dim3(1), dim3(256), 0, ctx->stream, Tall, lt, d, T1w + 1, (int64_t)q, k);
                else
                    MRBF_BLAS(ctx, rocblas_dtrsm(ctx->blas, rocblas_side_left, rocblas_fill_lower, rocblas_operation_transpose,
                                                 rocblas_diagonal_non_unit, d, k, &one, Tall, (int)lt, T1w + 1, q));
            }
            hipLaunchKernelGGL(finish_lambda_kernel, dim3((unsigned)k), dim3(64), 0, ctx->stream, T1w, q, k, std::sqrt((double)n), M->mean);
        }
        hipLaunchKernelGGL(scatter_solution_kernel, dim3(nblk(M->npad * k + (int64_t)q * k)), dim3(256), 0, ctx->stream, B, npad, n,
                           M->npad, k, q, (int64_t)0, M->W, M->Wc, M->lam, T1w ? T1w : B, (int64_t)q);
        MRBF_HIP(ctx, hipGetLastError());
        return 0;
    };
    MRBF_TRY(solve_tail(true));
    MRBF_HIP(ctx, hipEventRecord(ctx->ev[4], ctx->stream));
    {
        int hflags_local[4] = {0, 0, 0, 0};
        double hscal_local[2] = {0.0, 0.0};
        int *hflags = ctx->hpin ? reinterpret_cast<int *>(ctx->hpin + HPIN_FIT_FLAGS) : hflags_local;
        double *hscal = ctx->hpin ? reinterpret_cast<double *>(ctx->hpin + HPIN_FIT_SCAL) : hscal_local;
        hscal[0] = hscal[1] = 0.0;
        static const int publish = mrbf_env("MRBF_FIT_PUBLISH") ? atoi(mrbf_env("MRBF_FIT_PUBLISH")) : 1;
        if (ctx->hpin && publish) {
            unsigned long long *hstat = nullptr;
            const unsigned long long *dstat = nullptr;
            if (ctx->mega_stat_pending && ctx->mega_stat_dev) {
                ctx->hpin[HPIN_MEGA_STAT] = ~0ull;
                hstat = &ctx->hpin[HPIN_MEGA_STAT];
                dstat = ctx->mega_stat_dev;
                ctx->mega_stat_pending = 2;
            }
            hipLaunchKernelGGL(fit_publish_kernel, dim3(1), dim3(64), 0, ctx->stream, (const int *)dinfo, q > 0 ? (const double *)scal : nullptr, dstat,
                               hflags, hscal, hstat);
        } else {
        MRBF_HIP(ctx, hipMemcpyAsync(hflags, dinfo, 4 * sizeof(int), hipMemcpyDeviceToHost, ctx->stream));
        if (q > 0) MRBF_HIP(ctx, hipMemcpyAsync(hscal, scal, 2 * sizeof(double), hipMemcpyDeviceToHost, ctx->stream));
        MRBF_TRY(mega_stat_enqueue(ctx));
        }
        MRBF_HIP(ctx, hipStreamSynchronize(ctx->stream));
        MRBF_TRY(mega_stat_finish(ctx));
        info->ms_factor_device = ctx->last_device_ms;
        hinfo = hflags[0];
        if (hinfo < 0) {
            *gave_up = 1;
            info->giveup_code = -hinfo;
            return 0;
        }
        info->factor_info = hinfo;
        if (q > 0) info->mu = hscal[1];
        if (hflags[1] < 0) {
            *gave_up = 1;
            info->giveup_code = -hflags[1];
            return 0;
        }
        if (hflags[1] != 0) {
            *not_pd = 1;
            info->factor_info = -2;
            return 0;
        }
        if (hflags[2] != 0) {
            *not_pd = 1;
            info->factor_info = -1;
            return 0;
        }
        if (hinfo != 0) {
            *not_pd = 1;
            return 0;
        }
        if (hflags[3] != 0) {
            info->fallbacks |= MRBF_FB_BACKSOLVE_BLOCKED;
            info->giveup_code = hflags[3];
            MRBF_TRY(solve_tail(false));
            MRBF_HIP(ctx, hipEventRecord(ctx->ev[4], ctx->stream));
        }
    }
    MRBF_HIP(ctx, hipEventSynchronize(ctx->ev[4]));
    MRBF_HIP(ctx, hipEventElapsedTime(&info->ms_gram, ctx->ev[0], ctx->ev[1]));
    MRBF_HIP(ctx, hipEventElapsedTime(&info->ms_project, ctx->ev[1], ctx->ev[2]));
    MRBF_HIP(ctx, hipEventElapsedTime(&info->ms_factor, ctx->ev[2], ctx->ev[3]));
    MRBF_HIP(ctx, hipEventElapsedTime(&info->ms_solve, ctx->ev[3], ctx->ev[4]));
    info->path = q > 0 ? MRBF_PATH_PROJ_CHOL : MRBF_PATH_CHOL;
    return 0;
}

void fill_small_prob(const mrbf_ctx *ctx, const mrbf_model *M, const double *Y, double *ws, int *flags, double *scal, int *cl, smallfit::Prob *P) {
    P->n = (int)M->n;
    P->d = M->d;
    P->k = M->k;
    P->q = M->q;
    P->deg = M->deg;
    P->n16 = (int)round_up(M->n, 16);
    P->npad = (int)M->npad;
    P->dpad = M->dpad;
    P->q16 = (int)round_up(std::max(M->q, 1), 16);
    P->kp = M->kp;
    P->C = M->C;
    P->Y = Y;
    P->Xc = M->Xc;
    P->sq = M->sq;
    P->mean = M->mean;
    P->W = M->W;
    P->Wc = M->Wc;
    P->lam = M->lam;
    P->ws = ws;
    P->flags = flags;
    P->scal = scal;
    P->stamps = nullptr;
    P->cl = cl;
    P->spin_ticks = (unsigned long long)std::max(1, ctx->spin_ms) * 100000ull;
    P->fault = (ctx->debug_fault & 4) ? 1 : 0;
    P->mean_given = 0;
}
int small_fit_verdict(const mrbf_model *M, const int *hflags, const double *hscal, mrbf_fit_info *info) {
    info->path = M->q > 0 ? MRBF_PATH_PROJ_CHOL : MRBF_PATH_CHOL;
    info->mu = M->q > 0 ? hscal[1] : 0.0;
    info->factor_info = hflags[0];
    if (hflags[1] != 0) {
        info->factor_info = -2;
        return 1;
    }
    if (hflags[2] != 0) {
        info->factor_info = -1;
        return 1;
    }
    return hflags[0] != 0 ? 1 : 0;
}
static int fit_check_enqueue(mrbf_ctx *ctx, mrbf_model *M, const double *Y, double *h, hipEvent_t e0, hipEvent_t e1);
static int fit_check_finish(mrbf_ctx *ctx, const mrbf_model *M, const double *h, mrbf_fit_info *info, hipEvent_t e0, hipEvent_t e1);
static int fit_small(mrbf_ctx *ctx, mrbf_model *M, const double *Y, mrbf_fit_info *info, int *not_pd, int force_nc, int *nc_used,
                     bool *checked = nullptr) {
    *not_pd = 0;
    if (checked) *checked = false;
    smallfit::Prob P;
    const smallfit::Carve cv = smallfit::carve((int)M->npad, (int)round_up(std::max(M->q, 1), 16));
    double *ws, *scal;
    int *flags;
    MRBF_TRY(get_buf(ctx, S_SMALL_WS, cv.total, &ws));
    MRBF_TRY(get_buf(ctx, S_SMALL_FLAGS, (size_t)4, &flags));
    MRBF_TRY(get_buf(ctx, S_MISC, (size_t)8, &scal));
    int *cl;
    MRBF_TRY(get_buf(ctx, S_SMALL_CL, (size_t)smallfit::CL_WORDS, &cl));
    fill_small_prob(ctx, M, Y, ws, flags, scal, cl, &P);
    static const int want_stamps = mrbf_env("MRBF_SMALL_STAMPS") ? atoi(mrbf_env("MRBF_SMALL_STAMPS")) : 0;
    long long *dstamps = nullptr;
    if (want_stamps) {
        MRBF_TRY(get_buf(ctx, S_SMALL_DESC, (size_t)16, &dstamps));
        P.stamps = dstamps;
    }
    int hflags_local[4] = {0, 0, 0, 0};
    double hscal_local[2] = {0.0, 0.0}, hchk_local[3] = {0, 0, 0};
    int *hflags = ctx->hpin ? reinterpret_cast<int *>(ctx->hpin + HPIN_SMALL_FLAGS) : hflags_local;
    double *hscal = ctx->hpin ? reinterpret_cast<double *>(ctx->hpin + HPIN_SMALL_SCAL) : hscal_local;
    double *hchk = ctx->hpin ? reinterpret_cast<double *>(ctx->hpin + HPIN_SMALL_CHK) : hchk_local;
    int nc = force_nc > 0 ? force_nc : small_fit_cluster(ctx, 1);
    for (int attempt = 0; attempt < 2; ++attempt) {
        MRBF_HIP(ctx, hipMemsetAsync(cl, 0, smallfit::CL_WORDS * sizeof(int), ctx->stream));
        MRBF_HIP(ctx, hipEventRecord(ctx->ev[0], ctx->stream));
        MRBF_TRY(launch_small_fit(ctx, &P, 1, nullptr, nc));
        MRBF_HIP(ctx, hipEventRecord(ctx->ev[1], ctx->stream));
        MRBF_HIP(ctx, hipMemcpyAsync(hflags, flags, 4 * sizeof(int), hipMemcpyDeviceToHost, ctx->stream));
        MRBF_HIP(ctx, hipMemcpyAsync(hscal, scal, 2 * sizeof(double), hipMemcpyDeviceToHost, ctx->stream));
        hchk[0] = hchk[1] = hchk[2] = 0.0;
        const bool with_check = checked && ctx->residual;
        if (with_check) MRBF_TRY(fit_check_enqueue(ctx, M, Y, hchk, ctx->ev[2], ctx->ev[3]));
        MRBF_HIP(ctx, hipStreamSynchronize(ctx->stream));
        if (with_check && hflags[3] == 0 && hflags[0] == 0 && hflags[1] == 0 && hflags[2] == 0) {
            MRBF_TRY(fit_check_finish(ctx, M, hchk, info, ctx->ev[2], ctx->ev[3]));
            *checked = true;
        }
        if (nc == 1) break;
        if (hflags[3] == 0) {
            ctx->small_timeouts = 0;
            break;
        }
        if (hflags[3] == 2 || ++ctx->small_timeouts >= 3) ctx->small_nc = 1;
        nc = 1;
    }
    *nc_used = nc;
    MRBF_HIP(ctx, hipEventElapsedTime(&info->ms_factor, ctx->ev[0], ctx->ev[1]));
    if (want_stamps) {
        long long hs[16];
        MRBF_HIP(ctx, hipMemcpy(hs, dstamps, sizeof(hs), hipMemcpyDeviceToHost));
        static const char *names[] = {"centre", "gram", "Q1", "W,G,mu,V", "K update", "rhs", "potrf", "solves", "tail"};
        fprintf(stderr, "small fit n=%lld d=%d q=%d (%d workgroup%s): %.3f ms |", (long long)M->n, M->d, M->q, nc, nc == 1 ? "" : "s", info->ms_factor);
        for (int i = 0; i < 9; ++i) fprintf(stderr, " %s %.1f us |", names[i], (hs[i + 1] - hs[i]) * 0.01);
        fprintf(stderr, " [gram: product %.1f us, radial function %.1f us, padding %.1f us]\n", (hs[11] - hs[1]) * 0.01, (hs[12] - hs[11]) * 0.01,
                (hs[2] - hs[12]) * 0.01);
    }
    *not_pd = small_fit_verdict(M, hflags, hscal, info);
    return 0;
}

static int fit_check_enqueue(mrbf_ctx *ctx, mrbf_model *M, const double *Y, double *h, hipEvent_t e0, hipEvent_t e1) {
    const int64_t n = M->n;
    const int k = M->k, q = M->q;
    double *V, *scal;
    MRBF_TRY(get_buf(ctx, S_STAGE_D, (size_t)n * k, &V));
    MRBF_TRY(get_buf(ctx, S_CHECK_SCAL, (size_t)8, &scal));
    MRBF_HIP(ctx, hipEventRecord(e0, ctx->stream));
    EvalHints hints;
    hints.check_call = true;
    MRBF_TRY(eval_model(ctx, M, n, M->C, V, nullptr, nullptr, hints));
    hipLaunchKernelGGL(residual_kernel, dim3(1), dim3(256), 0, ctx->stream, V, Y, n * k, scal);
    if (q > 0) {
        double *Pi, *T;
        MRBF_TRY(get_buf(ctx, S_PI, (size_t)n * q, &Pi));
        MRBF_TRY(get_buf(ctx, S_T2, (size_t)q * k, &T));
        MRBF_TRY(launch_poly_matrix(ctx, M->C, n, M->d, q, Pi, n));
        MRBF_TRY(tsmm_tn(ctx, n, q, k, 1.0, Pi, n, M->Wc, M->npad, 0.0, T, q));
        hipLaunchKernelGGL(max_abs_kernel, dim3(1), dim3(256), 0, ctx->stream, T, (int64_t)q * k, scal + 2);
    }
    MRBF_HIP(ctx, hipGetLastError());
    MRBF_HIP(ctx, hipMemcpyAsync(h, scal, 3 * sizeof(double), hipMemcpyDeviceToHost, ctx->stream));
    MRBF_HIP(ctx, hipEventRecord(e1, ctx->stream));
    return 0;
}
static int fit_check_finish(mrbf_ctx *ctx, const mrbf_model *M, const double *h, mrbf_fit_info *info, hipEvent_t e0, hipEvent_t e1) {
    info->rel_residual = std::sqrt(h[0]) / std::max(std::sqrt(h[1]), 1e-300);
    info->max_pitw = M->q > 0 ? h[2] : 0.0;
    MRBF_HIP(ctx, hipEventElapsedTime(&info->ms_check, e0, e1));
    return 0;
}
int fit_check(mrbf_ctx *ctx, mrbf_model *M, const double *Y, mrbf_fit_info *info) {
    double h_local[3] = {0, 0, 0};
    double *h = ctx->hpin ? reinterpret_cast<double *>(ctx->hpin + HPIN_RESIDUAL) : h_local;
    h[0] = h[1] = h[2] = 0.0;
    MRBF_TRY(fit_check_enqueue(ctx, M, Y, h, ctx->ev[0], ctx->ev[1]));
    MRBF_HIP(ctx, hipStreamSynchronize(ctx->stream));
    return fit_check_finish(ctx, M, h, info, ctx->ev[0], ctx->ev[1]);
}

int fit_model(mrbf_ctx *ctx, mrbf_model *M, const double *Y, mrbf_fit_info *info) {
    mrbf_fit_info local;
    if (!info) info = &local;
    std::memset(info, 0, sizeof(*info));
    info->n = (int32_t)M->n;
    info->q = M->q;
    info->rel_residual = NAN;
    info->max_pitw = NAN;
    const int order = cpd_order(M->kp.kid, M->kp.a, M->kp.b);
    int path = ctx->force_path;
    int small_nc_used = 0;
    bool checked = false;
    if (path == 0) path = (order <= M->deg + 1 && M->n > M->q) ? (M->q > 0 ? MRBF_PATH_PROJ_CHOL : MRBF_PATH_CHOL) : MRBF_PATH_LU;
    if (M->n < M->q) path = MRBF_PATH_MINNORM;
    if (path == MRBF_PATH_CHOL && M->q > 0) path = MRBF_PATH_PROJ_CHOL;
    if (path == MRBF_PATH_PROJ_CHOL && M->q == 0) path = MRBF_PATH_CHOL;
    if (path == MRBF_PATH_MINNORM) {
        MRBF_TRY(fit_minnorm(ctx, M, Y, info));
    } else if (path != MRBF_PATH_LU && !kp_nonsmooth(M->kp) && small_fit_applies(ctx, M->n, M->d, M->k, M->q, path)) {
        int not_pd = 0;
        MRBF_TRY(fit_small(ctx, M, Y, info, &not_pd, 0, &small_nc_used, &checked));
        if (not_pd) {
            info->fallbacks |= MRBF_FB_LU;
            if (ctx->force_path != 0)
                return fail(ctx, MRBF_ENOTPD, "Cholesky path forced but the matrix is not positive definite (info = %d)",
                            info->factor_info);
            path = MRBF_PATH_LU;
        }
    } else if (path != MRBF_PATH_LU) {
        int not_pd = 0, gave_up = 0;
        MRBF_TRY(fit_chol(ctx, M, Y, info, &not_pd, &gave_up));
        if (gave_up) {
            info->fallbacks |= MRBF_FB_CHOL_HOST_DRIVEN;
            MRBF_TRY(fit_chol(ctx, M, Y, info, &not_pd, &gave_up, 2));
            if (gave_up) return fail(ctx, MRBF_EHIP, "host-driven Cholesky reported a give-up code (0x%x)", info->giveup_code);
        }
        if (not_pd) {
            info->fallbacks |= MRBF_FB_LU;
            if (ctx->force_path != 0)
                return fail(ctx, MRBF_ENOTPD, "Cholesky path forced but the matrix is not positive definite (info = %d)",
                            info->factor_info);
            path = MRBF_PATH_LU;
        }
    }
    if (path == MRBF_PATH_LU) {
        if (small_lu_applies(ctx, M->n, M->d, M->k, M->q, M->kp))
            MRBF_TRY(fit_small_lu(ctx, M, Y, info));
        else
            MRBF_TRY(fit_lu(ctx, M, Y, info));
    }
    if (ctx->residual && !(checked && path != MRBF_PATH_LU)) MRBF_TRY(fit_check(ctx, M, Y, info));
    if (ctx->residual && small_nc_used > 1 && path != MRBF_PATH_LU && !(info->rel_residual < 1e-6)) {
        const double res_cluster = info->rel_residual;
        std::vector<double> wc((size_t)M->n * M->k);
        MRBF_HIP(ctx, hipMemcpy(wc.data(), M->W, wc.size() * sizeof(double), hipMemcpyDeviceToHost));
        int not_pd = 0, nc1 = 1;
        mrbf_fit_info again = *info;
        MRBF_TRY(fit_small(ctx, M, Y, &again, &not_pd, 1, &nc1));
        if (!not_pd) {
            MRBF_TRY(fit_check(ctx, M, Y, &again));
            std::vector<double> w1(wc.size());
            MRBF_HIP(ctx, hipMemcpy(w1.data(), M->W, w1.size() * sizeof(double), hipMemcpyDeviceToHost));
            if (std::memcmp(w1.data(), wc.data(), w1.size() * sizeof(double)) != 0 && (again.rel_residual < res_cluster || !(res_cluster == res_cluster)))
                ctx->small_nc = 1;
            *info = again;
        }
    }
    info->ms_total = info->ms_gram + info->ms_project + info->ms_factor + info->ms_solve;
    info->slow_launches = ctx->slow_launches;
    return 0;
}

}
```

Baseline: 174.3.

## Split tail update tiles, fold RHS copy into premul, fuse fit publish

The lower-triangular update launch now splits the leftover tiles of its last wave into half-height 64-row pieces, so the final round fills more compute slots (2 per CU by default). The persistent backsolve's premul kernel now also copies the RHS rows, which removes a separate get_rhs_rows launch. The fit-result publish to pinned host memory is moved into tail_apply_kernel, which removes one more small launch. All three are gated by the MRBF_FIT_GAPS bits, default 14, which turns them on. Risks are extra per-tile index math in the update kernel and a bit more work inside premul.

```diff
diff --git a/include/mrbf.h b/include/mrbf.h
--- a/include/mrbf.h
+++ b/include/mrbf.h
@@ -297,6 +297,9 @@
 int32_t mrbf_debug_potrf(mrbf_ctx *ctx, int64_t n, double *A_colmajor_inout, int32_t impl, int32_t *info, float *ms);
 int32_t mrbf_debug_diag(mrbf_ctx *ctx, const double *A128, int32_t reps, float *ms_per_call, double *shader_cycles,
                         double *realtime_us);
+int32_t mrbf_debug_update_lower(mrbf_ctx *ctx, int32_t nt, int32_t K, int32_t slots, const double *A_dev, const double *B_dev,
+                                double *C_dev, int64_t ldc, const double *cvec_dev, double cs, int64_t cn);
+int32_t mrbf_debug_update_split(int32_t nt, int32_t slots, int64_t *out4, int32_t *pieces);
 int32_t mrbf_debug_mfma_peak(mrbf_ctx *ctx, int32_t blocks_per_cu, int32_t threads, int32_t iters, float *ms, double *tflops);
 int32_t mrbf_debug_mfma_asm(mrbf_ctx *ctx, int32_t variant, int32_t blocks_per_cu, int32_t iters, float *ms, double *tflops,
                             double *cycles_per_mfma);
diff --git a/morbit.jl_amd/_lib.py b/morbit.jl_amd/_lib.py
--- a/morbit.jl_amd/_lib.py
+++ b/morbit.jl_amd/_lib.py
@@ -283,6 +283,9 @@
     "mrbf_debug_mega_tables": (ctypes.c_int32, [ctypes.c_int32] * 8 + [c_vp]),
     "mrbf_debug_mega_tables2": (ctypes.c_int32, [ctypes.c_int32] * 8 + [c_vp, c_vp]),
     "mrbf_debug_mega_plan": (ctypes.c_int32, [ctypes.c_int32] * 3 + [c_vp]),
+    "mrbf_debug_update_lower": (ctypes.c_int32, [c_vp] + [ctypes.c_int32] * 3 + [c_vp, c_vp, c_vp, ctypes.c_int64, c_vp, ctypes.c_double,
+                                                 ctypes.c_int64]),
+    "mrbf_debug_update_split": (ctypes.c_int32, [ctypes.c_int32] * 2 + [c_vp, c_vp]),
     "mrbf_stochastic_rank": (ctypes.c_int32, [ctypes.c_int32, c_vp, c_vp, c_vp, ctypes.c_double, c_vp]),
     "mrbf_ps_step": (ctypes.c_int32, [c_vp, c_vp, c_vp, c_vp, c_vp, c_vp, c_vp, ctypes.POINTER(PsOptions), c_vp, c_vp, c_vp,
                                       ctypes.POINTER(PsInfo)]),
diff --git a/morbit.jl_amd/csrc/backsolve.hip b/morbit.jl_amd/csrc/backsolve.hip
--- a/morbit.jl_amd/csrc/backsolve.hip
+++ b/morbit.jl_amd/csrc/backsolve.hip
@@ -19,9 +19,16 @@
 
 __global__ __launch_bounds__(256) void premul_kernel(const double *__restrict__ L, int64_t lda, const double *__restrict__ linv_all,
                                                      double *__restrict__ Mbuf, int nb, unsigned *__restrict__ flags, int nflags,
-                                                     unsigned long long *__restrict__ xb, int nxb) {
+                                                     unsigned long long *__restrict__ xb, int nxb, double *__restrict__ Y, int64_t ldy,
+                                                     int krhs) {
     for (int e = blockIdx.x * 256 + threadIdx.x; e < nflags; e += gridDim.x * 256) flags[e] = 0u;
     for (int e = blockIdx.x * 256 + threadIdx.x; e < nxb; e += gridDim.x * 256) xb[e] = ~0ull;
+    const int64_t nrow = (int64_t)nb * NB;
+    for (int64_t e = (int64_t)blockIdx.x * 256 + threadIdx.x; e < nrow * krhs; e += (int64_t)gridDim.x * 256) {
+        const int l = (int)(e % krhs);
+        const int64_t i = e / krhs;
+        Y[i + (int64_t)l * ldy] = L[(nrow + l) + i * lda];
+    }
     const int slab = blockIdx.x & 3, t = (blockIdx.x >> 2) & 1, j = blockIdx.x >> 3;
     const int i = j + 1 + t;
     if (i >= nb) return;
@@ -341,15 +348,17 @@
 }
 
 int backsolve_blocked(mrbf_ctx *ctx, int64_t npad, const double *L, int64_t lda, const double *linv_all, double *Y, int64_t ldy, int k);
+int launch_get_rhs_rows(mrbf_ctx *ctx, const double *A, int64_t ld, int64_t npad, double *B, int k);
 
 int backsolve_persistent(mrbf_ctx *ctx, int64_t npad, const double *L, int64_t lda, const double *linv_all, double *Y, int64_t ldy, int k,
-                         int *status) {
+                         int *status, bool fold_rhs_copy) {
     using namespace bsolve;
     const int nb = (int)(npad / NB);
     static const int force_old = mrbf_env("MRBF_BACKSOLVE_LAUNCHES") ? atoi(mrbf_env("MRBF_BACKSOLVE_LAUNCHES")) : 0;
     const int ncu = ctx->ncu;
-    if (force_old || nb < 3 || nb > ncu || (lda & 1) || (reinterpret_cast<uintptr_t>(L) & 15))
-        return backsolve_blocked(ctx, npad, L, lda, linv_all, Y, ldy, k);
+    const bool persistent = !(force_old || nb < 3 || nb > ncu || (lda & 1) || (reinterpret_cast<uintptr_t>(L) & 15));
+    if (!persistent || !fold_rhs_copy) MRBF_TRY(launch_get_rhs_rows(ctx, L, lda, npad, Y, k));
+    if (!persistent) return backsolve_blocked(ctx, npad, L, lda, linv_all, Y, ldy, k);
     unsigned *flags;
     MRBF_TRY(get_buf(ctx, S_BSOLVE_FLAGS, (size_t)(nb + 1) * 32, &flags));
     const unsigned long long spin_ticks = (unsigned long long)std::max(1, ctx->spin_ms) * 100000ull;
@@ -358,7 +367,7 @@
     MRBF_TRY(get_buf(ctx, S_BSOLVE_X, (size_t)2 * nb * 4 * NB, &xb));
     MRBF_TRY(get_buf(ctx, S_BSOLVE_M, (size_t)nb * 2 * NB * NB, &Mbuf));
     hipLaunchKernelGGL(premul_kernel, dim3((unsigned)(8 * (nb - 1))), dim3(256), 0, ctx->stream, L, lda, linv_all, Mbuf, nb, flags, (nb + 1) * 32,
-                       reinterpret_cast<unsigned long long *>(xb), 2 * nb * 4 * NB);
+                       reinterpret_cast<unsigned long long *>(xb), 2 * nb * 4 * NB, Y, ldy, fold_rhs_copy ? k : 0);
     static const bool want_stamps = mrbf_env("MRBF_BSOLVE_STAMPS") && atoi(mrbf_env("MRBF_BSOLVE_STAMPS")) != 0;
     long long *stamps = nullptr;
     if (want_stamps) {
diff --git a/morbit.jl_amd/csrc/chol.hip b/morbit.jl_amd/csrc/chol.hip
--- a/morbit.jl_amd/csrc/chol.hip
+++ b/morbit.jl_amd/csrc/chol.hip
@@ -1,8 +1,13 @@
 #include <chrono>
+#include <vector>
 
 #include "common.hpp"
+#include "update_split.hpp"
 
 namespace mrbf {
+
+int launch_update_lower(mrbf_ctx *ctx, const double *A, int64_t lda, const double *B, int64_t ldb, double *C, int64_t ldc, int64_t nt, int K,
+                        const double *cvec, double cs, int64_t cn, int slots);
 
 int debug_diag(mrbf_ctx *ctx, const double *A128_dev, int reps, float *ms_per_call, unsigned long long *stamps_host);
 int launch_pad_identity(mrbf_ctx *ctx, double *A, int64_t n, int64_t npad, int64_t ld);
@@ -66,6 +71,60 @@
     return MRBF_OK;
 }
 
+extern "C" int32_t mrbf_debug_update_lower(mrbf_ctx *ctx, int32_t nt, int32_t K, int32_t slots, const double *A_dev, const double *B_dev,
+                                           double *C_dev, int64_t ldc, const double *cvec_dev, double cs, int64_t cn) {
+    if (!ctx) return -1;
+    if (nt < 1 || nt > 1024) return -2;
+    if (K < 16 || K % 16 != 0) return -3;
+    if (slots < 0) return -4;
+    const int64_t m = (int64_t)nt * 128;
+    if (!A_dev || !is_device_ptr(A_dev) || (reinterpret_cast<uintptr_t>(A_dev) & 15)) return -5;
+    if (!B_dev || !is_device_ptr(B_dev) || (reinterpret_cast<uintptr_t>(B_dev) & 15)) return -6;
+    if (!C_dev || !is_device_ptr(C_dev)) return -7;
+    if (ldc < m) return -8;
+    if (cvec_dev && !is_device_ptr(cvec_dev)) return -9;
+    if (cn < 0 || cn > m) return -11;
+    (void)hipSetDevice(ctx->device);
+    MRBF_TRY(launch_update_lower(ctx, A_dev, m, B_dev, m, C_dev, ldc, nt, K, cvec_dev, cs, cn, slots));
+    MRBF_HIP(ctx, hipStreamSynchronize(ctx->stream));
+    return MRBF_OK;
+}
+
+extern "C" int32_t mrbf_debug_update_split(int32_t nt, int32_t slots, int64_t *out4, int32_t *pieces) {
+    if (nt < 1 || nt > 1024) return -1;
+    if (slots < 1) return -2;
+    if (!out4) return -3;
+    const int64_t ntiles = (int64_t)nt * (nt + 1) / 2;
+    const updsplit::Split sp = updsplit::split(ntiles, slots);
+    std::vector<unsigned char> seen((size_t)nt * nt * 2, 0);
+    int64_t bad = 0;
+    if (sp.nfull < 0 || sp.nfull > sp.npieces) ++bad;
+    for (int p = 0; p < sp.npieces; ++p) {
+        const updsplit::Piece pc = updsplit::piece(p, sp.nfull, nt);
+        if (pieces) {
+            pieces[4 * p + 0] = pc.ti;
+            pieces[4 * p + 1] = pc.tj;
+            pieces[4 * p + 2] = pc.r0;
+            pieces[4 * p + 3] = pc.rows;
+        }
+        const bool shape = (pc.rows == 128 && pc.r0 == 0) || (pc.rows == 64 && (pc.r0 == 0 || pc.r0 == 64));
+        if (!shape || pc.ti < 0 || pc.ti >= nt || pc.tj < 0 || pc.tj > pc.ti) {
+            ++bad;
+            continue;
+        }
+        for (int h = pc.r0 / 64; h < (pc.r0 + pc.rows) / 64; ++h) ++seen[((size_t)pc.ti * nt + pc.tj) * 2 + h];
+    }
+    for (int ti = 0; ti < nt; ++ti)
+        for (int tj = 0; tj < nt; ++tj)
+            for (int h = 0; h < 2; ++h)
+                if (seen[((size_t)ti * nt + tj) * 2 + h] != (tj <= ti ? 1 : 0)) ++bad;
+    out4[0] = sp.nfull;
+    out4[1] = sp.npieces;
+    out4[2] = updsplit::half_rounds(slots, sp);
+    out4[3] = bad;
+    return MRBF_OK;
+}
+
 extern "C" int32_t mrbf_debug_diag(mrbf_ctx *ctx, const double *A128, int32_t reps, float *ms_per_call, double *shader_cycles,
                                    double *realtime_us) {
     if (!ctx) return -1;
diff --git a/morbit.jl_amd/csrc/chol_blocked.hip b/morbit.jl_amd/csrc/chol_blocked.hip
--- a/morbit.jl_amd/csrc/chol_blocked.hip
+++ b/morbit.jl_amd/csrc/chol_blocked.hip
@@ -1,5 +1,6 @@
 #include "common.hpp"
 #include "mega_gemm.hpp"
+#include "update_split.hpp"
 
 namespace mrbf {
 
@@ -12,37 +13,12 @@
 int launch_diag(mrbf_ctx *ctx, hipStream_t st, double *Ajj, int64_t lda, double *Linv, int *dinfo, int col0);
 
 template <int TM, int MODE>
-__global__ __launch_bounds__(256, 2) void chol_update_kernel(const double *__restrict__ A, int64_t lda,
-                                                             const double *__restrict__ B, int64_t ldb,
-                                                             double *__restrict__ C, int64_t ldc, int K,
-                                                             const int *__restrict__ info, int mt_sq = 0, int ntiles_total = 0,
-                                                             const double *__restrict__ cvec = nullptr, double cs = 0.0, int64_t cn = 0) {
+__device__ __forceinline__ void update_piece(const double *__restrict__ A, int64_t lda, const double *__restrict__ B, int64_t ldb,
+                                             double *__restrict__ C, int64_t ldc, int K, int64_t I0, int64_t J0, bool diag,
+                                             const double *__restrict__ cvec, double cs, int64_t cn, double *smem) {
     constexpr int NJ = (TM == 128) ? 4 : 2;
-    __shared__ __attribute__((aligned(16))) double smem[mega::NSTG * mega::STG];
-    if (info && *info != 0) return;
-    if (MODE == UPD_OVERWRITE || MODE == UPD_COLUMN_SUB) __builtin_amdgcn_s_setprio(2);
     const int tid = threadIdx.x, lane = tid & 63, wave = tid >> 6;
     const int l15 = lane & 15, l4 = lane >> 4;
-    const int tile_end = (MODE == UPD_LOWER_SUB && ntiles_total > 0) ? ntiles_total : (int)blockIdx.x + 1;
-    for (int bid = blockIdx.x; bid < tile_end; bid += gridDim.x) {
-    int ti, tj;
-    if (MODE == UPD_LOWER_SUB) {
-        const int ntri = mt_sq * (mt_sq + 1) / 2;
-        if (bid < ntri || mt_sq == 0) {
-            int t = (int)((sqrt(8.0 * (double)bid + 1.0) - 1.0) * 0.5);
-            while ((t + 1) * (t + 2) / 2 <= bid) ++t;
-            while (t * (t + 1) / 2 > bid) --t;
-            ti = t;
-            tj = bid - t * (t + 1) / 2;
-        } else {
-            ti = mt_sq + (bid - ntri) / mt_sq;
-            tj = (bid - ntri) % mt_sq;
-        }
-    } else {
-        ti = blockIdx.x;
-        tj = blockIdx.y;
-    }
-    const int64_t I0 = (int64_t)ti * TM, J0 = (int64_t)tj * 128;
     const int ioff = (TM == 128) ? (wave >> 1) * 64 : 0;
     const int joff = (TM == 128) ? (wave & 1) * 64 : wave * 32;
 
@@ -110,12 +86,36 @@
                 } else {
                     double x = -acc[j][i][r];
                     if (cvec) x -= fma(cei[i], cvj[r], cvi[i] * cej[r]);
-                    if (ti != tj || gi >= gj) *dst = x;
+                    if (!diag || gi >= gj) *dst = x;
                 }
             }
         }
     }
-    if (bid + (int)gridDim.x < tile_end) __syncthreads();
+}
+
+template <int TM, int MODE>
+__global__ __launch_bounds__(256, 2) void chol_update_kernel(const double *__restrict__ A, int64_t lda,
+                                                             const double *__restrict__ B, int64_t ldb,
+                                                             double *__restrict__ C, int64_t ldc, int K,
+                                                             const int *__restrict__ info, int mt_sq = 0, int ntiles_total = 0,
+                                                             const double *__restrict__ cvec = nullptr, double cs = 0.0, int64_t cn = 0,
+                                                             int nfull = 0x7fffffff) {
+    __shared__ __attribute__((aligned(16))) double smem[mega::NSTG * mega::STG];
+    if (info && *info != 0) return;
+    if (MODE == UPD_OVERWRITE || MODE == UPD_COLUMN_SUB) __builtin_amdgcn_s_setprio(2);
+    const int tile_end = (MODE == UPD_LOWER_SUB && ntiles_total > 0) ? ntiles_total : (int)blockIdx.x + 1;
+    for (int bid = blockIdx.x; bid < tile_end; bid += gridDim.x) {
+        if constexpr (MODE == UPD_LOWER_SUB) {
+            const updsplit::Piece pc = updsplit::piece(bid, nfull, mt_sq);
+            if (TM == 128 && pc.rows == 64)
+                update_piece<64, MODE>(A, lda, B, ldb, C, ldc, K, (int64_t)pc.ti * 128 + pc.r0, (int64_t)pc.tj * 128, pc.ti == pc.tj, cvec, cs,
+                                       cn, smem);
+            else
+                update_piece<TM, MODE>(A, lda, B, ldb, C, ldc, K, (int64_t)pc.ti * TM, (int64_t)pc.tj * 128, pc.ti == pc.tj, cvec, cs, cn, smem);
+        } else {
+            update_piece<TM, MODE>(A, lda, B, ldb, C, ldc, K, (int64_t)blockIdx.x * TM, (int64_t)blockIdx.y * 128, false, cvec, cs, cn, smem);
+        }
+        if (bid + (int)gridDim.x < tile_end) __syncthreads();
     }
 }
 
@@ -389,10 +389,11 @@
 }
 
 int launch_update_lower(mrbf_ctx *ctx, const double *A, int64_t lda, const double *B, int64_t ldb, double *C, int64_t ldc, int64_t nt,
-                        int K, const double *cvec, double cs, int64_t cn) {
+                        int K, const double *cvec, double cs, int64_t cn, int slots) {
     if (nt <= 0 || K <= 0) return 0;
-    hipLaunchKernelGGL((chol_update_kernel<128, UPD_LOWER_SUB>), dim3((unsigned)(nt * (nt + 1) / 2)), dim3(256), 0, ctx->stream, A,
-                       lda, B, ldb, C, ldc, K, (const int *)nullptr, (int)nt, 0, cvec, cs, cn);
+    const updsplit::Split sp = updsplit::split(nt * (nt + 1) / 2, slots > 0 ? slots : 2 * ctx->ncu);
+    hipLaunchKernelGGL((chol_update_kernel<128, UPD_LOWER_SUB>), dim3((unsigned)sp.npieces), dim3(256), 0, ctx->stream, A, lda, B, ldb, C,
+                       ldc, K, (const int *)nullptr, (int)nt, 0, cvec, cs, cn, sp.nfull);
     MRBF_HIP(ctx, hipGetLastError());
     return 0;
 }
diff --git a/morbit.jl_amd/csrc/solve.hip b/morbit.jl_amd/csrc/solve.hip
--- a/morbit.jl_amd/csrc/solve.hip
+++ b/morbit.jl_amd/csrc/solve.hip
@@ -3,13 +3,20 @@
 
 namespace mrbf {
 
-__global__ void fit_publish_kernel(const int *__restrict__ dinfo, const double *__restrict__ scal, const unsigned long long *__restrict__ dstat,
-                                   int *__restrict__ hflags, double *__restrict__ hscal, unsigned long long *__restrict__ hstat) {
-    const int t = threadIdx.x;
-    if (t < 4) hflags[t] = dinfo[t];
-    if (t >= 4 && t < 6 && scal) hscal[t - 4] = scal[t - 4];
-    if (t == 6 && dstat && hstat) hstat[0] = dstat[0];
-}
+struct FitPublish {
+    const int *dinfo = nullptr;
+    const double *scal = nullptr;
+    const unsigned long long *dstat = nullptr;
+    int *hflags = nullptr;
+    double *hscal = nullptr;
+    unsigned long long *hstat = nullptr;
+};
+__device__ __forceinline__ void fit_publish(const FitPublish &p, int t) {
+    if (t < 4) p.hflags[t] = p.dinfo[t];
+    if (t >= 4 && t < 6 && p.scal) p.hscal[t - 4] = p.scal[t - 4];
+    if (t == 6 && p.dstat && p.hstat) p.hstat[0] = p.dstat[0];
+}
+__global__ void fit_publish_kernel(FitPublish p) { fit_publish(p, threadIdx.x); }
 
 __global__ void fill_saddle_kernel(const double *__restrict__ Pi, int64_t n, int q, double *__restrict__ S, int64_t N) {
     const int64_t idx = (int64_t)blockIdx.x * blockDim.x + threadIdx.x;
@@ -329,9 +336,9 @@
 
 int backsolve_blocked(mrbf_ctx *ctx, int64_t npad, const double *L, int64_t lda, const double *linv_all, double *Y, int64_t ldy, int k);
 int backsolve_persistent(mrbf_ctx *ctx, int64_t npad, const double *L, int64_t lda, const double *linv_all, double *Y, int64_t ldy, int k,
-                         int *status);
+                         int *status, bool fold_rhs_copy);
 int launch_update_lower(mrbf_ctx *ctx, const double *A, int64_t lda, const double *B, int64_t ldb, double *C, int64_t ldc, int64_t nt, int K,
-                        const double *cvec, double cs, int64_t cn);
+                        const double *cvec, double cs, int64_t cn, int slots = 0);
 int launch_pad_identity(mrbf_ctx *ctx, double *A, int64_t n, int64_t npad, int64_t ld);
 int tsmm_tn(mrbf_ctx *ctx, int64_t n, int p, int r, double alpha, const double *A, int64_t lda, const double *B, int64_t ldb, double beta,
             double *C, int64_t ldc);
@@ -351,6 +358,11 @@
     const int l = (int)(idx % k);
     const int64_t i = idx / k;
     B[i + (int64_t)l * npad] = A[(npad + l) + i * ld];
+}
+int launch_get_rhs_rows(mrbf_ctx *ctx, const double *A, int64_t ld, int64_t npad, double *B, int k) {
+    hipLaunchKernelGGL(get_rhs_rows_kernel, dim3(nblk(npad * k)), dim3(256), 0, ctx->stream, A, ld, npad, B, k);
+    MRBF_HIP(ctx, hipGetLastError());
+    return 0;
 }
 __global__ void xc_to_tall_kernel(const double *__restrict__ Xc, int64_t n, int d, int dpad, double *__restrict__ Tall, int64_t lt,
                                   int64_t dq) {
@@ -583,8 +595,9 @@
 __global__ __launch_bounds__(256) void tail_apply_kernel(const double *__restrict__ Bw, int64_t ldb, const double *__restrict__ Q1, int64_t ldq,
                                                          const double *__restrict__ T2, const double *__restrict__ lamsrc, int64_t n,
                                                          int64_t npad, int q, int k, double *__restrict__ W, double *__restrict__ Wc,
-                                                         double *__restrict__ lam) {
+                                                         double *__restrict__ lam, FitPublish pub) {
     __shared__ double part4[4][64];
+    if (blockIdx.x == gridDim.x - 1 && pub.hflags) fit_publish(pub, threadIdx.x);
     const int tid = threadIdx.x, r = tid & 63, g = tid >> 6;
     const int64_t row = (int64_t)blockIdx.x * 64 + r;
     for (int l = 0; l < k; ++l) {
@@ -618,6 +631,8 @@
     *gave_up = 0;
     if (impl == 0) impl = ctx->chol_impl;
     const bool builtin = impl != 1;
+    static const int gaps = mrbf_env("MRBF_FIT_GAPS") ? atoi(mrbf_env("MRBF_FIT_GAPS")) : 14;
+    const int upd_slots = (gaps & 2) ? 0 : 0x7fffffff;
     PotrfOpts popt;
     popt.impl = impl;
     const int xt = builtin ? (int)round_up(k, 128) : 0;
@@ -695,7 +710,7 @@
         MRBF_TRY(get_buf(ctx, S_STAGE_D, (size_t)npad * K2, &PB));
         if (skip) MRBF_TRY(get_buf(ctx, S_V0, (size_t)npad, &v0));
         MRBF_TRY(launch_projection_small(ctx, M, Wpart, rspart, nseg, LxInv, Q1, Wm, G, scal, dinfo, K2, skip, PA, PB, v0));
-        MRBF_TRY(launch_update_lower(ctx, PA, npad, PB, npad, Phi, ld, npad / 128, K2, v0, 1.0 / std::sqrt((double)n), n));
+        MRBF_TRY(launch_update_lower(ctx, PA, npad, PB, npad, Phi, ld, npad / 128, K2, v0, 1.0 / std::sqrt((double)n), n, upd_slots));
     } else if (q > 0) {
         MRBF_TRY(symm_panel(ctx, n, npad, q, Phi, ld, Q1, npad, Wm, npad, true, 1.0 / std::sqrt((double)n)));
         MRBF_TRY(tsmm_tn(ctx, n, q, q, 1.0, Q1, npad, Wm, npad, 0.0, G, q));
@@ -711,7 +726,7 @@
         MRBF_TRY(get_buf(ctx, S_STAGE_D, (size_t)npad * K2, &PB));
         if (skip) MRBF_TRY(get_buf(ctx, S_V0, (size_t)npad, &v0));
         hipLaunchKernelGGL(build_panels_kernel, dim3(nblk(npad * K2)), dim3(256), 0, ctx->stream, Q1, Wm, scal, n, npad, q, K2, skip, PA, PB, v0);
-        MRBF_TRY(launch_update_lower(ctx, PA, npad, PB, npad, Phi, ld, npad / 128, K2, v0, 1.0 / std::sqrt((double)n), n));
+        MRBF_TRY(launch_update_lower(ctx, PA, npad, PB, npad, Phi, ld, npad / 128, K2, v0, 1.0 / std::sqrt((double)n), n, upd_slots));
     }
     MRBF_HIP(ctx, hipEventRecord(ctx->ev[2], ctx->stream));
     int hinfo = 0;
@@ -733,13 +748,14 @@
     }
     double *T1w = nullptr;
     if (q > 0) MRBF_TRY(get_buf(ctx, S_T1W, (size_t)q * k, &T1w));
-    auto solve_tail = [&](bool persistent) -> int {
+    auto solve_tail = [&](bool persistent, const FitPublish &pub, bool *published) -> int {
         if (builtin) {
-            hipLaunchKernelGGL(get_rhs_rows_kernel, dim3(nblk(npad * k)), dim3(256), 0, ctx->stream, Phi, ld, npad, B, k);
-            if (persistent)
-                MRBF_TRY(backsolve_persistent(ctx, npad, Phi, ld, linv_all, B, npad, k, dinfo + 3));
-            else
+            if (persistent) {
+                MRBF_TRY(backsolve_persistent(ctx, npad, Phi, ld, linv_all, B, npad, k, dinfo + 3, (gaps & 4) != 0));
+            } else {
+                MRBF_TRY(launch_get_rhs_rows(ctx, Phi, ld, npad, B, k));
                 MRBF_TRY(backsolve_blocked(ctx, npad, Phi, ld, linv_all, B, npad, k));
+            }
         } else {
             MRBF_BLAS(ctx, rocsolver_dpotrs(ctx->blas, rocblas_fill_lower, (int)n, k, Phi, (int)ld, B, (int)npad));
         }
@@ -753,8 +769,9 @@
             hipLaunchKernelGGL(tail_coeff_kernel, dim3(1), dim3(1024), 0, ctx->stream, part, nch, q, k, q > 1 ? d : 0, T1, G, fused ? 1.0 : 0.5, LxInv,
                                std::sqrt((double)n), M->mean, T2, T1w);
             hipLaunchKernelGGL(tail_apply_kernel, dim3((unsigned)nch), dim3(256), 0, ctx->stream, B, npad, Q1, npad, T2, T1w, n, M->npad, q, k, M->W,
-                               M->Wc, M->lam);
+                               M->Wc, M->lam, pub);
             MRBF_HIP(ctx, hipGetLastError());
+            if (pub.hflags) *published = true;
             return 0;
         }
         if (q > 0) {
@@ -780,26 +797,32 @@
         MRBF_HIP(ctx, hipGetLastError());
         return 0;
     };
-    MRBF_TRY(solve_tail(true));
+    int hflags_local[4] = {0, 0, 0, 0};
+    double hscal_local[2] = {0.0, 0.0};
+    int *hflags = ctx->hpin ? reinterpret_cast<int *>(ctx->hpin + HPIN_FIT_FLAGS) : hflags_local;
+    double *hscal = ctx->hpin ? reinterpret_cast<double *>(ctx->hpin + HPIN_FIT_SCAL) : hscal_local;
+    hscal[0] = hscal[1] = 0.0;
+    static const int publish = mrbf_env("MRBF_FIT_PUBLISH") ? atoi(mrbf_env("MRBF_FIT_PUBLISH")) : 1;
+    FitPublish pub;
+    if (ctx->hpin && publish) {
+        pub.dinfo = dinfo;
+        pub.scal = q > 0 ? scal : nullptr;
+        pub.hflags = hflags;
+        pub.hscal = hscal;
+        if (ctx->mega_stat_pending && ctx->mega_stat_dev) {
+            ctx->hpin[HPIN_MEGA_STAT] = ~0ull;
+            pub.hstat = &ctx->hpin[HPIN_MEGA_STAT];
+            pub.dstat = ctx->mega_stat_dev;
+            ctx->mega_stat_pending = 2;
+        }
+    }
+    bool published = false;
+    MRBF_TRY(solve_tail(true, (gaps & 8) ? pub : FitPublish(), &published));
     MRBF_HIP(ctx, hipEventRecord(ctx->ev[4], ctx->stream));
     {
-        int hflags_local[4] = {0, 0, 0, 0};
-        double hscal_local[2] = {0.0, 0.0};
-        int *hflags = ctx->hpin ? reinterpret_cast<int *>(ctx->hpin + HPIN_FIT_FLAGS) : hflags_local;
-        double *hscal = ctx->hpin ? reinterpret_cast<double *>(ctx->hpin + HPIN_FIT_SCAL) : hscal_local;
-        hscal[0] = hscal[1] = 0.0;
-        static const int publish = mrbf_env("MRBF_FIT_PUBLISH") ? atoi(mrbf_env("MRBF_FIT_PUBLISH")) : 1;
-        if (ctx->hpin && publish) {
-            unsigned long long *hstat = nullptr;
-            const unsigned long long *dstat = nullptr;
-            if (ctx->mega_stat_pending && ctx->mega_stat_dev) {
-                ctx->hpin[HPIN_MEGA_STAT] = ~0ull;
-                hstat = &ctx->hpin[HPIN_MEGA_STAT];
-                dstat = ctx->mega_stat_dev;
-                ctx->mega_stat_pending = 2;
-            }
-            hipLaunchKernelGGL(fit_publish_kernel, dim3(1), dim3(64), 0, ctx->stream, (const int *)dinfo, q > 0 ? (const double *)scal : nullptr, dstat,
-                               hflags, hscal, hstat);
+        if (published) {
+        } else if (pub.hflags) {
+            hipLaunchKernelGGL(fit_publish_kernel, dim3(1), dim3(64), 0, ctx->stream, pub);
         } else {
         MRBF_HIP(ctx, hipMemcpyAsync(hflags, dinfo, 4 * sizeof(int), hipMemcpyDeviceToHost, ctx->stream));
         if (q > 0) MRBF_HIP(ctx, hipMemcpyAsync(hscal, scal, 2 * sizeof(double), hipMemcpyDeviceToHost, ctx->stream));
@@ -838,7 +861,7 @@
         if (hflags[3] != 0) {
             info->fallbacks |= MRBF_FB_BACKSOLVE_BLOCKED;
             info->giveup_code = hflags[3];
-            MRBF_TRY(solve_tail(false));
+            MRBF_TRY(solve_tail(false, FitPublish(), &published));
             MRBF_HIP(ctx, hipEventRecord(ctx->ev[4], ctx->stream));
         }
     }
diff --git a/morbit.jl_amd/csrc/update_split.hpp b/morbit.jl_amd/csrc/update_split.hpp
--- /dev/null
+++ b/morbit.jl_amd/csrc/update_split.hpp
@@ -0,0 +1,72 @@
+#pragma once
+#include <cmath>
+#include <cstdint>
+
+#if defined(__HIPCC__) || defined(__CUDACC__)
+#define MRBF_HD __host__ __device__
+#else
+#define MRBF_HD
+#endif
+
+namespace mrbf {
+namespace updsplit {
+
+struct Split {
+    int nfull;
+    int npieces;
+};
+struct Piece {
+    int ti, tj;
+    int r0, rows;
+};
+
+inline Split split(int64_t ntiles, int slots) {
+    Split s;
+    s.nfull = (int)ntiles;
+    s.npieces = (int)ntiles;
+    if (slots > 0 && ntiles > slots) {
+        const int rem = (int)(ntiles % slots);
+        if (rem > 0 && 2 * rem <= slots) {
+            s.nfull = (int)ntiles - rem;
+            s.npieces = s.nfull + 2 * rem;
+        }
+    }
+    return s;
+}
+inline int64_t half_rounds(int slots, const Split &s) {
+    const int64_t full_rounds = (s.nfull + slots - 1) / slots;
+    const int64_t open = full_rounds * slots - s.nfull;
+    int64_t halves = s.npieces - s.nfull - 2 * open;
+    if (halves < 0) halves = 0;
+    return 2 * full_rounds + (halves + slots - 1) / slots;
+}
+
+MRBF_HD inline void tile_of(int t, int mt_sq, int *ti, int *tj) {
+    const int ntri = mt_sq * (mt_sq + 1) / 2;
+    if (t < ntri || mt_sq == 0) {
+        int r = (int)((sqrt(8.0 * (double)t + 1.0) - 1.0) * 0.5);
+        while ((r + 1) * (r + 2) / 2 <= t) ++r;
+        while (r * (r + 1) / 2 > t) --r;
+        *ti = r;
+        *tj = t - r * (r + 1) / 2;
+    } else {
+        *ti = mt_sq + (t - ntri) / mt_sq;
+        *tj = (t - ntri) % mt_sq;
+    }
+}
+MRBF_HD inline Piece piece(int p, int nfull, int mt_sq) {
+    Piece pc;
+    if (p < nfull) {
+        tile_of(p, mt_sq, &pc.ti, &pc.tj);
+        pc.r0 = 0;
+        pc.rows = 128;
+    } else {
+        tile_of(nfull + (p - nfull) / 2, mt_sq, &pc.ti, &pc.tj);
+        pc.r0 = ((p - nfull) & 1) * 64;
+        pc.rows = 64;
+    }
+    return pc;
+}
+
+}
+}
```

After: 174.3 (median of 2 runs). No clear change (-0.0%).
